# jinsungkim96/MPC-SensorlessAO

Measured on AMD Instinct MI355X. Metric: MPC steps/sec (n=27, VAR(2), T=30), higher is better.
Workload: dtype f64

## Files before the change

### mpc-sensorlessao_amd/csrc/fmpc_affine.h

```cpp
#pragma once
#include <hip/hip_runtime.h>
#include "fmpc_host.h"
#include "../../include/fastmpc.h"

#define FA_N 27

struct FaStep {
    const double* x0; const double* x0p; const double* nu0;
    double* zout; double* nuout; double* u0out; int* status; int* iters; double* step;
    int* need;
};

struct FaParams {
    int n, m, T, nb, has_xf, batch, rows, tiles, step_ld;
    int nu_rows, nu_tiles;
    int ldz;
    int tiles_used, wgs_per_group;
    const double* img;
    const double* imgE; const double* imgEp;
    const double* elin; const double* eplin;
    const double* dx0T;
    double e0, ep0, normE, norme, normEp, normep, rd2_0;
    const double* x0; const double* x0p; const double* nu0;
    double* zout; double* nuout; double* u0out; int* status; int* iters; double* step;
    int* need; int* handed;
    int* nflag;
    double* dump;
    int nsteps;
    FaStep steps[FMPC_STRETCH_MAX];
    int nlanes, wgs_per_lane;
    int lane_begin[FMPC_STRETCH_MAX + 1];
    const double* imgG;
    const int* plan;
    int jbase, nu_work;
    int nparts, nitems, swap;
};

#define FMPC_STRETCH_LANES_DEFAULT FMPC_STRETCH_MAX
hipError_t fmpc_launch_affine(FaParams P, int num_cu, hipStream_t stream, const unsigned* supersedes = nullptr);
hipError_t fmpc_launch_affine_nu(FaParams P, int grid, bool nt, hipStream_t stream);
```

### mpc-sensorlessao_amd/csrc/fmpc_affine_dev.h

```cpp
#pragma once
#include <hip/hip_runtime.h>
#include <math.h>
#include "fmpc_device.h"
#include "fmpc_affine.h"
#include "../../include/fastmpc.h"

typedef double d4a __attribute__((ext_vector_type(4)));
typedef double d2a __attribute__((ext_vector_type(2)));
#define FA_MFMA(a, b, c) __builtin_amdgcn_mfma_f64_16x16x4f64((a), (b), (c), 0, 0, 0)
#define FA_THREADS 256
#define FA_CT 4

__device__ __forceinline__ void fa_load_a(double (&A)[FA_KS], const double* img, int tile, int lane) {
    const double* ip = img + (size_t)tile * FA_KS * 64 + lane;
#pragma unroll
    for (int q = 0; q < FA_KS; ++q) A[q] = ip[q * 64];
}

__device__ __forceinline__ void fa_request_a(double (&A)[FA_KS], const double* img, int tile, int lane) {
    const double* ip = img + (size_t)tile * FA_KS * 64 + lane;
    const double* ip2 = ip + 8 * 64;
#define FA_LD(q, base, off) asm volatile("global_load_dwordx2 %0, %1, off offset:" #off : "=v"(A[q]) : "v"(base))
    FA_LD(0, ip, 0); FA_LD(1, ip, 512); FA_LD(2, ip, 1024); FA_LD(3, ip, 1536); FA_LD(4, ip, 2048); FA_LD(5, ip, 2560); FA_LD(6, ip, 3072); FA_LD(7, ip, 3584);
    FA_LD(8, ip2, 0); FA_LD(9, ip2, 512); FA_LD(10, ip2, 1024); FA_LD(11, ip2, 1536); FA_LD(12, ip2, 2048); FA_LD(13, ip2, 2560);
#undef FA_LD
}
template <int BEHIND>
__device__ __forceinline__ void fa_await_a(double (&A)[FA_KS]) {
    asm volatile("s_waitcnt vmcnt(%14)"
                 : "+v"(A[0]), "+v"(A[1]), "+v"(A[2]), "+v"(A[3]), "+v"(A[4]), "+v"(A[5]), "+v"(A[6]), "+v"(A[7]), "+v"(A[8]), "+v"(A[9]),
                   "+v"(A[10]), "+v"(A[11]), "+v"(A[12]), "+v"(A[13])
                 : "n"(BEHIND));
}

__device__ __forceinline__ void fa_request_g(double (&A)[FA_NU_KS], const double* img, int tile, int lane) {
    const double* ip = img + (size_t)tile * FA_NU_KS * 64 + lane;
#define FA_LD(q, base, off) asm volatile("global_load_dwordx2 %0, %1, off offset:" #off : "=v"(A[q]) : "v"(base))
    FA_LD(0, ip, 0); FA_LD(1, ip, 512); FA_LD(2, ip, 1024); FA_LD(3, ip, 1536); FA_LD(4, ip, 2048); FA_LD(5, ip, 2560); FA_LD(6, ip, 3072);
#undef FA_LD
}
template <int BEHIND>
__device__ __forceinline__ void fa_await_g(double (&A)[FA_NU_KS]) {
    asm volatile("s_waitcnt vmcnt(%7)"
                 : "+v"(A[0]), "+v"(A[1]), "+v"(A[2]), "+v"(A[3]), "+v"(A[4]), "+v"(A[5]), "+v"(A[6])
                 : "n"(BEHIND));
}

__device__ __forceinline__ bool fa_decide(const FaParams& P, double qe, double qp, double rdl, double dn2) {
    const double dn = sqrt(dn2);
    double e2 = qe + P.e0, rp2 = qp + P.ep0;
    const double ce = 4096.0 * 2.220446049250313e-16;
    const double de = ce * (dn2 * P.normE + 2.0 * P.norme * dn + fabs(P.e0));
    const double dp = ce * (dn2 * P.normEp + 2.0 * P.normep * dn + fabs(P.ep0));
    e2 += de;
    rp2 = rp2 - dp > 0.0 ? rp2 - dp : 0.0;
    const double rho2 = rp2 + rdl;
    const bool fin = rp2 < 1e300 && rho2 < 1e300 && e2 < 1e300 && e2 >= 0.0;
    return fin && (rp2 > 4e-16 || rho2 > 4e-12) && e2 <= 0.5 * rho2;
}

#define FA_SD(ct, cc, k) sD[((((k) >> 2) * FA_CT + (ct)) * 4 + ((k) & 3)) * 16 + (cc)]
__device__ __forceinline__ void fa_stage(double* sD, const FaParams& P, const double* x0_s, const double* x0p_s, int p0, int tid) {
    constexpr int n = FA_N;
    const int np = P.batch - p0 < FA_CT * 16 ? P.batch - p0 : FA_CT * 16;
    const double* s0 = x0_s + (size_t)p0 * n;
    const double* s1 = x0p_s ? x0p_s + (size_t)p0 * n : s0;
    double v0[7], v1[7];
#pragma unroll
    for (int j = 0; j < 7; ++j) {
        const int idx = tid + FA_THREADS * j, ic = idx < np * n ? idx : 0;
        v0[j] = s0[ic]; v1[j] = s1[ic];
    }
#pragma unroll
    for (int j = 0; j < 7; ++j) {
        const int idx = tid + FA_THREADS * j;
        if (idx < FA_CT * 16 * n) {
            const int pr = idx / n, k = idx - pr * n;
            const bool on = idx < np * n;
            FA_SD(pr >> 4, pr & 15, k) = on ? v0[j] : 0.0;
            FA_SD(pr >> 4, pr & 15, n + k) = (on && x0p_s) ? v1[j] : 0.0;
        }
    }
    double zero = 0.0;
    asm volatile("" : "+v"(zero));
    if (tid < FA_CT * 16) { FA_SD(tid >> 4, tid & 15, 2 * n) = 1.0; FA_SD(tid >> 4, tid & 15, 2 * n + 1) = zero; }
}

__device__ __forceinline__ void fa_forms(const double* sD, double (&sF)[4][3][16], const FaParams& P, int slot, int wv, int lane, int p0,
                                         const double* nu0_s, int* need_s, int* status_s, int* iters_s, double* step_s) {
    constexpr int n = FA_N;
    const int g = lane >> 4, c = lane & 15;
    for (int fct = P.wgs_per_group - 1 - slot; fct < FA_CT; fct += P.wgs_per_group) {
        if (fct < 0 || p0 + fct * 16 >= P.batch) continue;
        const int t = wv;
        double E1[FA_KS], E2[FA_KS], Df[FA_KS];
        fa_load_a(E1, P.imgE, t, lane);
        fa_load_a(E2, P.imgEp, t, lane);
        const int k = 16 * t + c;
        const double le = P.elin[k], lp = P.eplin[k];
        double rdl[4] = {P.rd2_0, P.rd2_0, P.rd2_0, P.rd2_0};
        if (nu0_s && t == 0) {
            double xa[4][2];
#pragma unroll
            for (int r = 0; r < 4; ++r) {
                const int pr = p0 + fct * 16 + 4 * r + g < P.batch ? p0 + fct * 16 + 4 * r + g : P.batch - 1;
                const double* nu = nu0_s + (size_t)pr * P.nb * n;
#pragma unroll
                for (int j = 0; j < 2; ++j) {
                    const int e = c + 16 * j, ec = e < n ? e : 0;
                    xa[r][j] = P.dx0T[ec] + nu[(P.T - 1) * n + ec] + (P.has_xf ? nu[P.T * n + ec] : 0.0);
                }
            }
#pragma unroll
            for (int r = 0; r < 4; ++r) {
                double acc = xa[r][0] * xa[r][0] + (c + 16 < n ? xa[r][1] * xa[r][1] : 0.0);
                acc += __shfl_xor(acc, 1, 64); acc += __shfl_xor(acc, 2, 64); acc += __shfl_xor(acc, 4, 64); acc += __shfl_xor(acc, 8, 64);
                rdl[r] = acc;
            }
        }
#pragma unroll
        for (int q = 0; q < FA_KS; ++q) Df[q] = sD[(q * FA_CT + fct) * 64 + lane];
        d4a ce = {0, 0, 0, 0}, cp = {0, 0, 0, 0};
#pragma unroll
        for (int q = 0; q < FA_KS; ++q) { ce = FA_MFMA(Df[q], E1[q], ce); cp = FA_MFMA(Df[q], E2[q], cp); }
        double qe[4], qp[4], dn2[4];
#pragma unroll
        for (int r = 0; r < 4; ++r) {
            const double dv = k < 2 * n ? FA_SD(fct, 4 * r + g, k < 2 * n ? k : 0) : 0.0;
            qe[r] = dv * (ce[r] + le); qp[r] = dv * (cp[r] + lp); dn2[r] = dv * dv;
#pragma unroll
            for (int o = 1; o < 16; o <<= 1) { qe[r] += __shfl_xor(qe[r], o, 64); qp[r] += __shfl_xor(qp[r], o, 64); dn2[r] += __shfl_xor(dn2[r], o, 64); }
            if (c == 0) { sF[t][0][4 * r + g] = qe[r]; sF[t][1][4 * r + g] = qp[r]; sF[t][2][4 * r + g] = dn2[r]; }
        }
        __syncthreads();
        if (t == 0 && c == 0) {
#pragma unroll
            for (int r = 0; r < 4; ++r) {
                const int i = 4 * r + g, pp = p0 + fct * 16 + i;
                if (pp < P.batch) {
                    const double se = (sF[0][0][i] + sF[1][0][i]) + (sF[2][0][i] + sF[3][0][i]);
                    const double sp = (sF[0][1][i] + sF[1][1][i]) + (sF[2][1][i] + sF[3][1][i]);
                    const double sn = (sF[0][2][i] + sF[1][2][i]) + (sF[2][2][i] + sF[3][2][i]);
                    const bool clear = fa_decide(P, se, sp, rdl[r], sn);
                    need_s[pp] = clear ? 0 : 1;
                    if (!clear && P.nflag) atomicAdd(P.nflag, 1);
                    if (clear) {
                        if (status_s) status_s[pp] = FMPC_OK;
                        if (iters_s) iters_s[pp] = 1;
                        if (step_s) for (int q = 0; q < P.step_ld; ++q) step_s[(size_t)pp * P.step_ld + q] = q == 0 ? 1.0 : -1.0;
                    }
                }
            }
        }
        __syncthreads();
    }
}
```

### mpc-sensorlessao_amd/csrc/fmpc_api.hip

```cpp
#include <hip/hip_runtime.h>
#include <math.h>
#include <stdio.h>
#include <stdlib.h>
#include <string.h>
#include <atomic>
#include <map>
#include <mutex>
#include <new>
#include <vector>

#include "../../include/fastmpc.h"
#include "fmpc_device.h"
#include "fmpc_panel.h"
#include "fmpc_host.h"
#include "fmpc_first.h"
#include "fmpc_affine.h"
#include "fmpc_loopu0.h"
#include "fmpc_tiled.h"
#include "fmpc_rampcold.h"
#include "fmpc_bank.h"
#include "fmpc_records.h"
#include "fmpc_kkt.h"
#include "fmpc_estimator.h"
#include "fmpc_handle.h"
// ... 362 lines not shown
}

static int fmpc_upload_cold(fmpc_handle h, double k, hipStream_t stream) {
    const int n = h->n, m = h->m, mp = h->wave.mp;
    int o[14];
    fmpc_wave_cold_layout(n, mp, o);
    std::vector<double> c((size_t)o[8], 0.0);
    for (int j = 0; j < m; ++j) {
        const double sp = h->hm_umax[j] - h->hm_umid[j], sm = h->hm_umid[j] - h->hm_umin[j];
        const double dp = 1.0 / sp, dm = 1.0 / sm;
        const double hc = k * (dp * dp + dm * dm);
        c[o[0] + j] = h->hm_R2[j] * h->hm_umid[j] + h->hm_rl[j] + k * (dp - dm);
        c[o[1] + j] = hc;
        c[o[2] + j] = 1.0 / (h->hm_R2[j] + hc);
    }
    const double* bt = h->hm_bt.data();
    for (int a = 0; a < n; ++a) {
        double cbu = 0.0, bu = 0.0;
        for (int j = 0; j < m; ++j) {
            cbu += bt[(size_t)j * n + a] * c[o[2] + j] * c[o[0] + j];
            bu += bt[(size_t)j * n + a] * h->hm_umid[j];
        }
        c[o[4] + a] = cbu;
        double a1x = 0.0, a2x = 0.0;
        for (int q = 0; q < n; ++q) { a1x += h->hm_a1[a * n + q] * h->hm_xmid[q]; a2x += h->hm_a2[a * n + q] * h->hm_xmid[q]; }
        c[o[5] + a] = h->hm_xmid[a] - bu;
        c[o[6] + a] = h->hm_xmid[a] - bu - a1x;
        c[o[7] + a] = h->hm_xmid[a] - bu - a1x - a2x;
        double va = 0.0, va2 = 0.0;
        for (int j = 0; j < m; ++j) {
            const double aj = c[o[1] + j] * c[o[2] + j];
            va += bt[(size_t)j * n + a] * aj * c[o[0] + j];
            va2 += bt[(size_t)j * n + a] * aj * aj * c[o[0] + j];
        }
        c[o[11] + a] = va; c[o[12] + a] = va2;
        for (int b = 0; b < n; ++b) {
            double g = 0.0, ma = 0.0, ma2 = 0.0;
            for (int j = 0; j < m; ++j) {
                const double bb = bt[(size_t)j * n + a] * bt[(size_t)j * n + b];
                const double aj = c[o[1] + j] * c[o[2] + j];
                g += bb * c[o[2] + j]; ma += bb * aj; ma2 += bb * aj * aj;
            }
            c[o[3] + a * n + b] = g; c[o[9] + a * n + b] = ma; c[o[10] + a * n + b] = ma2;
        }
    }
    for (int j = 0; j < m; ++j) {
        const double aj = c[o[1] + j] * c[o[2] + j], cu = c[o[0] + j];
        c[o[13]] += aj * cu * cu; c[o[13] + 1] += aj * aj * cu * cu;
    }
    return hipMemcpyAsync(h->cold_d, c.data(), c.size() * sizeof(double), hipMemcpyHostToDevice, stream) == hipSuccess
               ? FMPC_OK : FMPC_E_HIP;
}

static int fmpc_upload_panel(fmpc_handle h, double k, hipStream_t stream) {
    (void)stream;
    h->pn_valid = 0;
    FmpcPanelIn In;
    In.n = h->n; In.m = h->m; In.T = h->T; In.nb = h->nb; In.mp = h->pn_mp; In.var_order = h->var_order;
    In.pool_doubles = h->pn_doubles; In.o_simg = h->pn_o_simg; In.o_limg = h->pn_o_limg; In.o_bt = h->pn_o_bt;
    In.o_aimg = h->pn_o_aimg; In.o_vec = h->pn_o_vec; In.o_ucon = h->pn_o_ucon; In.o_dz = h->pn_o_dz; In.limg_cap = h->pn_limg_cap;
    In.umax = h->hm_umax.data(); In.umin = h->hm_umin.data(); In.umid = h->hm_umid.data(); In.xmid = h->hm_xmid.data();
    In.R2 = h->hm_R2.data(); In.rl = h->hm_rl.data(); In.Q2 = h->hm_Q2.data(); In.Qf2 = h->hm_Qf2.data();
    In.ql = h->hm_ql.data(); In.qfl = h->hm_qfl.data(); In.xf = h->hm_xf.data();
    In.bt = h->hm_bt.data(); In.a1 = h->hm_a1.data(); In.a2 = h->hm_a2.data(); In.blocks = h->hm_blocks.data();
    In.idxD = h->hm_idxD.data(); In.idx1 = h->hm_idx1.data(); In.idx2 = h->hm_idx2.data();
    FmpcPanelOut Out;
    fmpc_host_build_panel(In, k, Out);
    if (!Out.valid) return FMPC_OK;
    h->pn_nsf = Out.nsf; h->pn_nsb = Out.nsb; h->pn_rp2c = Out.rp2c; h->pn_rd2_0 = Out.rd2_0;
    if (hipMemcpy(h->pn_sched, Out.sched.data(), Out.sched.size() * sizeof(int), hipMemcpyHostToDevice) != hipSuccess) return FMPC_E_HIP;
    if (hipMemcpy(h->pn_pool, Out.pool.data(), Out.pool.size() * sizeof(double), hipMemcpyHostToDevice) != hipSuccess) return FMPC_E_HIP;
    h->pn_valid = 1;
    return FMPC_OK;
}

template <typename R>
static int fmpc_tiled_build(fmpc_handle h, int t, hipStream_t stream) {
    fmpc_handle_s::Tiled& X = h->tl[t];
    const int n = h->n, m = h->m, nb = h->nb, nn = n * n;
    int NB = 0, NW = 0;
    if (!fmpc_tiled_supports(n, m, nb, t, &NB, &NW, h->denseR)) return FMPC_E_UNSUPPORTED;
    const int mb = (m + 15) / 16, NQ = NB * NB;
    const int nblk = (int)(h->hm_blocks.size() / nn);
    std::vector<R> img((size_t)(nblk + 1) * NQ * FT_TILE + (size_t)mb * NB * FT_TILE, (R)0);
    for (int k = 0; k < nblk; ++k)
        for (int a = 0; a < n; ++a)
            for (int b = 0; b < n; ++b)
                img[((size_t)k * NQ + (a / 16) * NB + b / 16) * FT_TILE + (a % 16) * 16 + b % 16] = (R)h->hm_blocks[(size_t)k * nn + a * n + b];
    const size_t obt = (size_t)(nblk + 1) * NQ * FT_TILE;
    for (int c = 0; c < m; ++c)
        for (int r = 0; r < n; ++r)
            img[obt + ((size_t)(c / 16) * NB + r / 16) * FT_TILE + (c % 16) * 16 + r % 16] = (R)h->hm_bt[(size_t)c * n + r];
    std::vector<int> ids;
    for (int i = 0; i < nb; ++i) ids.push_back(h->hm_idxD[i]);
    for (int i = 0; i < nb; ++i) ids.push_back(h->hm_idx1[i] >= 0 ? h->hm_idx1[i] : nblk);
    for (int i = 0; i < nb; ++i) ids.push_back(h->hm_idx2[i] >= 0 ? h->hm_idx2[i] : nblk);
    const int NP = 16 * NB, MP = 16 * mb;
    const size_t oBt = 0, oBm = oBt + (size_t)MP * NP, oA1 = oBm + (size_t)NP * MP, oA2 = oA1 + (size_t)NP * NP,
                 oA1t = oA2 + (size_t)NP * NP, oA2t = oA1t + (size_t)NP * NP, oQ2 = oA2t + (size_t)NP * NP,
                 oQf2 = oQ2 + (size_t)NP * NP, oX = oQf2 + (size_t)NP * NP, oXf = oX + (size_t)NP * NP, oR2 = oXf + (size_t)NP * NP,
                 ptot = oR2 + (h->denseR ? (size_t)MP * MP : 0);
    std::vector<double> pad(ptot, 0.0);
    for (int c = 0; c < m; ++c)
        for (int r = 0; r < n; ++r) {
            pad[oBt + (size_t)c * NP + r] = h->hm_bt[(size_t)c * n + r];
            pad[oBm + (size_t)r * MP + c] = h->hm_bt[(size_t)c * n + r];
        }
    for (int a = 0; a < n; ++a)
        for (int b = 0; b < n; ++b) {
            pad[oA1 + (size_t)a * NP + b] = h->hm_a1f[(size_t)a * n + b]; pad[oA1t + (size_t)b * NP + a] = h->hm_a1f[(size_t)a * n + b];
            pad[oA2 + (size_t)a * NP + b] = h->hm_a2f[(size_t)a * n + b]; pad[oA2t + (size_t)b * NP + a] = h->hm_a2f[(size_t)a * n + b];
            pad[oQ2 + (size_t)a * NP + b] = h->hm_q2m[(size_t)a * n + b]; pad[oQf2 + (size_t)a * NP + b] = h->hm_qf2m[(size_t)a * n + b];
            pad[oX + (size_t)a * NP + b] = h->hm_xm[(size_t)a * n + b]; pad[oXf + (size_t)a * NP + b] = h->hm_xfm[(size_t)a * n + b];
        }
    if (h->denseR)
        for (int a = 0; a < m; ++a)
            for (int b = 0; b < m; ++b) pad[oR2 + (size_t)a * MP + b] = h->hm_r2full[(size_t)a * m + b];
    int rc = X.pool.assign((const char*)img.data(), img.size() * sizeof(R), stream);
    if (rc == FMPC_OK) rc = X.ipool.assign(ids.data(), ids.size(), stream);
    if (rc == FMPC_OK) rc = X.bm.assign(pad.data(), pad.size(), stream);
    if (rc != FMPC_OK) return rc;
    X.NB = NB; X.NW = NW;
    X.lds = fmpc_tiled_lds_bytes(NB, mb, NW, t, nb, h->denseR ? ft_pr_doubles(n, m) : 0);
    if (fmpc_tiled_prepare(n, NB, NW, t, X.lds, h->denseR) != hipSuccess) return FMPC_E_HIP;
    X.V.NB = NB; X.V.mb = mb; X.V.cn = n / 16; X.V.nl = n % 16; X.V.nblk = nblk;
    X.V.yimg = X.pool; X.V.btimg = (const R*)X.pool.p + obt;
    X.V.iD = X.ipool; X.V.i1 = X.ipool + nb; X.V.i2 = X.ipool + 2 * nb;
    X.V.BtP = X.bm + oBt; X.V.BmP = X.bm + oBm; X.V.A1P = X.bm + oA1; X.V.A2P = X.bm + oA2; X.V.A1tP = X.bm + oA1t; X.V.A2tP = X.bm + oA2t;
    X.V.denseR = h->denseR; X.V.R2P = h->denseR ? X.bm + oR2 : nullptr;
    X.V.denseQ = h->denseQ; X.V.Q2P = X.bm + oQ2; X.V.Qf2P = X.bm + oQf2; X.V.XP = X.bm + oX; X.V.XfP = X.bm + oXf;
    X.ready = 1;
    return FMPC_OK;
}

int fmpc_tiled_ensure(fmpc_handle h, int t, hipStream_t stream) {
    if (h->tl[t].ready) return FMPC_OK;
    return t ? fmpc_tiled_build<float>(h, 1, stream) : fmpc_tiled_build<double>(h, 0, stream);
}

__global__ void fmpc_zero_ints(int* p, int n) { if ((int)threadIdx.x < n) p[threadIdx.x] = 0; }
int fmpc_tiled_plan(fmpc_handle h, int t, int batch, hipStream_t stream, int nw_override, int grid_hint, FmpcTiledPlan* out) {
    fmpc_handle_s::Tiled& X = h->tl[t];
    { const int rc = fmpc_tiled_ensure(h, t, stream); if (rc != FMPC_OK) return rc; }
    int NWu = X.NW; size_t ldsu = X.lds;
    if (nw_override && nw_override != X.NW && !t && !h->denseR) {
        NWu = nw_override;
        ldsu = fmpc_tiled_lds_bytes(X.NB, X.V.mb, NWu, t, h->nb, 0);
        if (!(h->tl_prepared & (1 << NWu))) {
            if (ldsu > FMPC_LDS_LIMIT || fmpc_tiled_prepare(h->n, X.NB, NWu, t, ldsu, 0) != hipSuccess) { NWu = X.NW; ldsu = X.lds; }
            else h->tl_prepared |= 1 << NWu;
        }
    }
    int wgs = (int)(FMPC_LDS_LIMIT / ldsu);
    if (wgs < 1) wgs = 1;
    if (wgs * NWu > 8) wgs = 8 / NWu > 0 ? 8 / NWu : 1;
    const int cap = h->num_cu * wgs;
    const bool capturing = fmpc_capturing(stream);
    int grid = batch < cap ? batch : cap;
    if (!capturing && grid_hint > 0 && grid_hint < grid) grid = grid_hint;
    const FtWs L = ft_ws_layout(h->n, h->m, h->T, h->nb, X.NB, t ? 4 : 8, h->denseR, (t && h->refine > 0) ? 1 : 0);
    const size_t need = L.total * (size_t)grid, full = L.total * (size_t)cap;
    if (need > h->tl_ws.cap) {
        if (capturing) {
            const size_t have = h->tl_ws.cap / L.total;
            if (have < 1) return FMPC_E_ALLOC;
            grid = (int)have;
        } else {
            size_t want = 2 * h->tl_ws.cap;
            if (want < need) want = need;
            if (want > full) want = full;
            int rc = h->tl_ws.alloc(want, stream);
            if (rc != FMPC_OK && want != need) rc = h->tl_ws.alloc(need, stream);
            if (rc != FMPC_OK) return rc;
        }
    }
    out->NWu = NWu; out->ldsu = ldsu; out->grid = grid; out->slot = L.total;
    return FMPC_OK;
}

static int fmpc_solve_tiled(fmpc_handle h, int t, const FmpcSolve& s, int nw_override = 0, const int* list = nullptr,
                            const int* nlist = nullptr, const double* nuws = nullptr, int grid_hint = 0,
                            const FmpcTiledPlan* planned = nullptr) {
    FmpcTiledPlan plan;
    if (planned) plan = *planned;
    else { const int rc = fmpc_tiled_plan(h, t, s.batch, s.stream, nw_override, grid_hint, &plan); if (rc != FMPC_OK) return rc; }
    fmpc_handle_s::Tiled& X = h->tl[t];
    FtParams P;
    P.M = h->dev; P.V = X.V; P.batch = s.batch;
    P.x0 = s.x0; P.x0p = s.x0_pre; P.w = s.w; P.zinit = s.z_init; P.nu0 = s.nu0;
    P.max_iter = fmpc_max_iter(s); P.kbar = s.k;
    P.zout = s.z_out; P.nuout = s.nu_out; P.status = s.status; P.iters = s.iters; P.step = s.step; P.step_ld = fmpc_step_ld(s.n_newton);
    P.ws = h->tl_ws; P.ws_stride = plan.slot; P.u0out = s.u0_out;
    P.list = list; P.nlist = nlist; P.nuws = nuws;
    P.refine = t ? h->refine : 0;
    h->tl_last_nw = plan.NWu;
    if (t) h->refine_last = P.refine;
    if (!list) { h->last_path = t ? FMPC_PATH_TILED_F32 : FMPC_PATH_TILED; h->bank_first_dispatch = 0; }
    return fmpc_launch_tiled(P, X.NB, plan.NWu, t, plan.grid, plan.ldsu, s.stream) == hipSuccess ? FMPC_OK : FMPC_E_HIP;
}

extern "C" int fmpc_set_precision(fmpc_handle h, int mode) {
    if (!h) return FMPC_E_NULL;
    if (mode != FMPC_PREC_F64 && mode != FMPC_PREC_F32_MIXED) return FMPC_E_DIM;
    if (mode == FMPC_PREC_F32_MIXED && !fmpc_tiled_supports(h->n, h->m, h->nb, 1, nullptr, nullptr, h->denseR)) return FMPC_E_UNSUPPORTED;
    std::lock_guard<std::mutex> lk(h->mu);
    if (mode == FMPC_PREC_F64 && !h->generic_ok && !fmpc_tiled_supports(h->n, h->m, h->nb, 0, nullptr, nullptr, h->denseR)) {
        const size_t lds = fmpc_generic_big_lds_bytes(h->n, h->m);
        if (lds > FMPC_LDS_LIMIT) return FMPC_E_UNSUPPORTED;
        if (fmpc_generic_prepare(lds, 1) != hipSuccess) return FMPC_E_HIP;
        h->generic_ok = 1; h->generic_big = 1; h->lds_bytes = lds; h->wg_per_cu = 2;
    }
    h->prec = mode;
    h->bkf.valid = 0;
    h->bfm.valid = 0;
    return FMPC_OK;
}

extern "C" int fmpc_set_refinement(fmpc_handle h, int sweeps) {
    if (!h) return FMPC_E_NULL;
    if (sweeps < 0 || sweeps > FMPC_MAX_REFINEMENT) return FMPC_E_DIM;
    std::lock_guard<std::mutex> lk(h->mu);
    h->refine = sweeps;
    return FMPC_OK;
}
extern "C" int fmpc_last_refinement(fmpc_handle h) {
    if (!h) return 0;
    std::lock_guard<std::mutex> lk(h->mu);
    return h->last_path == FMPC_PATH_TILED_F32 ? h->refine_last : 0;
}

static int fmpc_grid_for(fmpc_handle h, int batch) {
    int cap = h->num_cu * h->wg_per_cu;
    return batch < cap ? batch : cap;
}

static int fmpc_ensure_ws(fmpc_handle h, int grid, size_t* stride, hipStream_t stream) {
    const FmpcWsLayout L = fmpc_ws_layout(h->n, h->m, h->T, h->nb, h->generic_big != 0, h->denseR != 0);
    *stride = L.total;
    return h->ws.grow(L.total * (size_t)grid, stream);
}

bool fmpc_capturing(hipStream_t stream) {
    hipStreamCaptureStatus st = hipStreamCaptureStatusNone;
    return hipStreamIsCapturing(stream, &st) == hipSuccess && st == hipStreamCaptureStatusActive;
}

struct FmpcChainStep {
    FaStep a;
    FwParams w;
    bool superseded;
    unsigned same_outputs;
};
struct FmpcStretch {
    fmpc_handle h = nullptr;
    int nsteps = 0;
    FaParams A;
    double k = 0.0; int n_newton = 0, zld = 0, g3 = 0; bool z_null = false, z_aligned = false;
    size_t wave_lds = 0, ws_stride = 0; int num_cu = 0;
    FwParams* table = nullptr;
    FmpcChainStep st[FMPC_STRETCH_MAX];
    size_t nodes_seen = 0;
};
static std::mutex fmpc_st_mu;
static std::map<hipStream_t, FmpcStretch> fmpc_st_map;
static std::atomic<int> fmpc_st_open{0};

static bool fmpc_capture_nodes(hipStream_t stream, size_t* count) {
    hipStreamCaptureStatus st = hipStreamCaptureStatusNone;
    unsigned long long id = 0; hipGraph_t graph = nullptr; const hipGraphNode_t* deps = nullptr; size_t ndeps = 0;
    if (hipStreamGetCaptureInfo_v2(stream, &st, &id, &graph, &deps, &ndeps) != hipSuccess || st != hipStreamCaptureStatusActive || !graph)
        return false;
    size_t n = 0;
    if (hipGraphGetNodes(graph, nullptr, &n) != hipSuccess) return false;
    *count = n;
    return true;
}
static void fmpc_stretch_look(FmpcStretch& S, hipStream_t stream) {
    size_t n = 0;
    S.nodes_seen = fmpc_capture_nodes(stream, &n) ? n : 0;
}
static bool fmpc_stretch_foreign(FmpcStretch& S, hipStream_t stream) {
    size_t n = 0;
    if (S.nsteps == 0 || !fmpc_capture_nodes(stream, &n) || n == S.nodes_seen) return false;
    S.nsteps = 0; S.h = nullptr;
    S.nodes_seen = n;
    return true;
}

static int fmpc_stretch_flush(FmpcStretch& S, hipStream_t stream) {
    if (S.nsteps == 0) return FMPC_OK;
    const int n = S.nsteps;
    fmpc_handle h = S.h;
    S.nsteps = 0; S.h = nullptr;
    if (!fmpc_capturing(stream) && h->ev && h->ev_valid && h->last_stream != stream && hipStreamWaitEvent(stream, h->ev, 0) != hipSuccess)
        return FMPC_E_HIP;
    FaParams A = S.A;
    A.nsteps = n;
    for (int i = 0; i < n; ++i) A.steps[i] = S.st[i].a;
    unsigned same[FMPC_STRETCH_MAX];
    for (int j = 0; j < n; ++j) {
        same[j] = S.st[j].same_outputs & ((1u << j) - 1u);
        for (int i = 0; i < j; ++i) if (same[j] >> i & 1u) same[j] |= same[i];
    }
    if (fmpc_launch_affine(A, S.num_cu, stream, same) != hipSuccess) return FMPC_E_HIP;
    int live[FMPC_STRETCH_MAX], nlive = 0;
    for (int i = 0; i < n; ++i) if (!S.st[i].superseded) live[nlive++] = i;
    int launches = 1;
    if (nlive == 1 || S.z_null) {
        for (int j = 0; j < nlive; ++j) {
            FwParams P = S.st[live[j]].w;
            if (j + 1 < nlive) { P.handed = nullptr; P.nflag = nullptr; }
            if (fmpc_launch_wave(P, S.g3, S.wave_lds, stream) != hipSuccess) return FMPC_E_HIP;
            ++launches;
        }
    } else {
        int g = S.num_cu / nlive;
        if (g > S.g3) g = S.g3;
        if (g < 1) return FMPC_E_UNSUPPORTED;
        FwChainStep T[FMPC_STRETCH_MAX];
        for (int j = 0; j < nlive; ++j) {
            const FwParams& P = S.st[live[j]].w;
            T[j] = {P.x0, P.x0p, P.nu0, P.zout, P.nuout, P.u0out, P.status, P.iters, P.step, P.list,
                    j + 1 == nlive ? P.handed : nullptr, P.ws + (size_t)j * g * fmpc_wave_waves_per_wg() * S.ws_stride};
        }
        if (fmpc_launch_wave_chain(S.st[live[0]].w, T, nlive, S.table, g, S.wave_lds, stream) != hipSuccess) return FMPC_E_HIP;
        launches += 2;
    }
    h->st_steps = n; h->st_launches = launches;
    if (!fmpc_capturing(stream) && h->ev && hipEventRecord(h->ev, stream) == hipSuccess) { h->ev_valid = 1; h->last_stream = stream; }
    fmpc_stretch_look(S, stream);
    return FMPC_OK;
}

static void fmpc_stretch_flush_handle_locked(fmpc_handle h, bool keep_one, hipStream_t keep);
static int fmpc_stretch_flush_stream(hipStream_t stream, fmpc_handle h = nullptr) {
    if (fmpc_st_open.load() == 0) return FMPC_OK;
    std::lock_guard<std::mutex> lk(fmpc_st_mu);
    if (h) fmpc_stretch_flush_handle_locked(h, true, stream);
    auto it = fmpc_st_map.find(stream);
    if (it == fmpc_st_map.end()) return FMPC_OK;
    if (fmpc_stretch_foreign(it->second, stream)) return FMPC_E_UNSUPPORTED;
    return fmpc_stretch_flush(it->second, stream);
}
static void fmpc_stretch_flush_handle_locked(fmpc_handle h, bool keep_one, hipStream_t keep) {
    for (auto& kv : fmpc_st_map)
        if (kv.second.nsteps && kv.second.h == h && !(keep_one && kv.first == keep) && !fmpc_stretch_foreign(kv.second, kv.first))
            (void)fmpc_stretch_flush(kv.second, kv.first);
}
static void fmpc_stretch_flush_handle(fmpc_handle h) {
    if (fmpc_st_open.load() == 0) return;
    std::lock_guard<std::mutex> lk(fmpc_st_mu);
    fmpc_stretch_flush_handle_locked(h, false, nullptr);
}

extern "C" int fmpc_stretch_begin(void* stream_) {
    hipStream_t stream = (hipStream_t)stream_;
    std::lock_guard<std::mutex> lk(fmpc_st_mu);
    if (fmpc_st_map.count(stream)) return FMPC_E_UNSUPPORTED;
    FmpcStretch& S = fmpc_st_map[stream];
    fmpc_stretch_look(S, stream);
    fmpc_st_open.fetch_add(1);
    return FMPC_OK;
}
extern "C" int fmpc_stretch_end(void* stream_) {
    hipStream_t stream = (hipStream_t)stream_;
    std::lock_guard<std::mutex> lk(fmpc_st_mu);
    auto it = fmpc_st_map.find(stream);
    if (it == fmpc_st_map.end()) return FMPC_E_UNSUPPORTED;
    int rc = FMPC_OK;
    if (it->second.nsteps) {
        if (it->second.h && hipSetDevice(it->second.h->device) != hipSuccess) rc = FMPC_E_HIP;
        else if (fmpc_stretch_foreign(it->second, stream)) rc = FMPC_E_UNSUPPORTED;
        else rc = fmpc_stretch_flush(it->second, stream);
    }
    fmpc_st_map.erase(it);
    fmpc_st_open.fetch_sub(1);
    return rc;
}
extern "C" int fmpc_last_stretch(fmpc_handle h, int* steps, int* launches) {
    if (!h) return FMPC_E_NULL;
    if (steps) *steps = h->st_steps.load();
    if (launches) *launches = h->st_launches.load();
    return FMPC_OK;
}

static inline bool fmpc_overlap(const void* a, size_t na, const void* b, size_t nb) {
    if (!a || !b || !na || !nb) return false;
    const char* pa = (const char*)a; const char* pb = (const char*)b;
    return pa < pb + nb && pb < pa + na;
}
struct FmpcStepRanges { const void* in[3]; size_t nin[3]; const void* out[6]; size_t nout[6]; };
static FmpcStepRanges fmpc_step_ranges(const FaParams& A, const FaStep& a) {
    FmpcStepRanges R;
    const size_t B = (size_t)A.batch, d = sizeof(double);
    R.in[0] = a.x0; R.nin[0] = B * A.n * d;
    R.in[1] = a.x0p; R.nin[1] = B * A.n * d;
    R.in[2] = a.nu0; R.nin[2] = B * A.nb * A.n * d;
    const size_t ldz = A.ldz > A.rows ? A.ldz : A.rows;
    R.out[0] = a.zout; R.nout[0] = ((B - 1) * ldz + A.rows) * d;
    R.out[1] = a.nuout; R.nout[1] = B * A.nb * A.n * d;
    R.out[2] = a.u0out; R.nout[2] = B * A.m * d;
    R.out[3] = a.status; R.nout[3] = B * sizeof(int);
    R.out[4] = a.iters; R.nout[4] = B * sizeof(int);
    R.out[5] = a.step; R.nout[5] = B * A.step_ld * d;
    return R;
}
static bool fmpc_stretch_accepts(const FmpcStretch& S, fmpc_handle h, const FmpcSolve& s, const FaStep& a, int zld, bool z_null, unsigned* supersedes) {
    *supersedes = 0;
    if (S.h != h || S.nsteps >= FMPC_STRETCH_MAX || memcmp(&S.k, &s.k, sizeof(double)) != 0 || S.A.batch != s.batch) return false;
    if (S.n_newton != s.n_newton || S.zld != zld || S.z_null != z_null || S.z_aligned != (((size_t)a.zout & 127) == 0)) return false;
    const FaStep& f = S.st[0].a;
    if ((f.nuout == nullptr) != (a.nuout == nullptr) || (f.u0out == nullptr) != (a.u0out == nullptr) || (f.status == nullptr) != (a.status == nullptr) ||
        (f.iters == nullptr) != (a.iters == nullptr) || (f.step == nullptr) != (a.step == nullptr)) return false;
    const FmpcStepRanges N = fmpc_step_ranges(S.A, a);
    for (int i = 0; i < S.nsteps; ++i) {
        const FaStep& b = S.st[i].a;
        const FmpcStepRanges O = fmpc_step_ranges(S.A, b);
        for (int x = 0; x < 3; ++x)
            for (int y = 0; y < 6; ++y)
                if (fmpc_overlap(N.in[x], N.nin[x], O.out[y], O.nout[y]) || fmpc_overlap(O.in[x], O.nin[x], N.out[y], N.nout[y])) return false;
        if (a.zout == b.zout && a.nuout == b.nuout && a.u0out == b.u0out && a.status == b.status && a.iters == b.iters && a.step == b.step) {
            *supersedes |= 1u << i;
            continue;
        }
        for (int x = 0; x < 6; ++x)
            for (int y = 0; y < 6; ++y)
                if (fmpc_overlap(N.out[x], N.nout[x], O.out[y], O.nout[y])) return false;
    }
    return true;
}

static int fmpc_stretch_settle(fmpc_handle h, hipStream_t stream) {
    if (!h->st_cur || h->st_cur->nsteps == 0) return FMPC_OK;
    return fmpc_stretch_flush(*h->st_cur, stream);
}
static int fmpc_guard_begin_queued(fmpc_handle h, hipStream_t stream) {
    if (fmpc_capturing(stream)) return FMPC_OK;
    if (!h->ev && hipEventCreateWithFlags(&h->ev, hipEventDisableTiming) != hipSuccess) return FMPC_E_HIP;
    if (h->ev_valid && stream != h->last_stream && hipStreamWaitEvent(stream, h->ev, 0) != hipSuccess) return FMPC_E_HIP;
    return FMPC_OK;
}
int fmpc_guard_begin(fmpc_handle h, hipStream_t stream) {
    const int rcs = fmpc_stretch_flush_stream(stream, h);
    if (rcs != FMPC_OK) return rcs;
    if (fmpc_capturing(stream)) return FMPC_OK;
    if (!h->ev && hipEventCreateWithFlags(&h->ev, hipEventDisableTiming) != hipSuccess) return FMPC_E_HIP;
    if (h->ev_valid && stream != h->last_stream && hipStreamWaitEvent(stream, h->ev, 0) != hipSuccess) return FMPC_E_HIP;
    return FMPC_OK;
}
void fmpc_guard_end(fmpc_handle h, hipStream_t stream) {
    if (fmpc_capturing(stream)) return;
    if (h->ev && hipEventRecord(h->ev, stream) == hipSuccess) { h->ev_valid = 1; h->last_stream = stream; }
}

static void fmpc_panel_params(fmpc_handle h, double k, FpParams& Q) {
    memset(&Q, 0, sizeof(Q));
    Q.m = h->m; Q.mp = h->pn_mp; Q.T = h->T; Q.nb = h->nb; Q.has_xf = h->has_xf; Q.var2 = h->var_order == 2 ? 1 : 0;
    Q.simg = h->pn_pool + h->pn_o_simg; Q.limg = h->pn_pool + h->pn_o_limg;
    Q.sched_f = h->pn_sched; Q.sched_b = h->pn_sched + (size_t)FP_MAX_STEPS(h->nb) * FP_STEP_INTS; Q.nsf = h->pn_nsf; Q.nsb = h->pn_nsb;
    Q.btimg = h->pn_pool + h->pn_o_bt; Q.aimg = h->pn_pool + h->pn_o_aimg;
    Q.vec = h->pn_pool + h->pn_o_vec; Q.ucon = h->pn_pool + h->pn_o_ucon;
    Q.rd2_0 = h->pn_rd2_0; Q.rp2c = h->pn_rp2c; Q.dump = h->pn_pool + h->pn_o_dump;
    Q.dzimg = h->pn_pool + h->pn_o_dz; Q.dzimg_len = h->pn_dz_len;
    Q.kbar = k;
    Q.jimg = h->inv_jimg; Q.nuc = h->inv_nuc; Q.jks = h->inv_jks; Q.jksp = 16 * ((h->inv_jks + 15) / 16 + 3); Q.eimg = h->inv_eimg;
    Q.jst = h->inv_jst; Q.nucst = h->inv_nucst; Q.gate_only = 0;
    Q.gw = nullptr; Q.gwn = h->T * h->n;
}

static int fmpc_build_inverse(fmpc_handle h, double k, hipStream_t stream) {
    const int n = h->n, T = h->T, nb = h->nb, TN = T * n, nrow = nb * n;
    const int ncol = 2 * n + TN, np = 1 + ncol + 2 * n, npanels = (np + FP_NP - 1) / FP_NP;
    const double scale = FMPC_INV_SCALE;
    h->inv_valid = 0;
    std::vector<double> hx0((size_t)np * n, 0.0), hx0p((size_t)np * n, 0.0), hw((size_t)np * TN, 0.0);
    for (int j = 0; j < n; ++j) { hx0[(size_t)(1 + j) * n + j] = scale; hx0p[(size_t)(1 + n + j) * n + j] = scale; }
    for (int j = 0; j < TN; ++j) hw[(size_t)(1 + 2 * n + j) * TN + j] = scale;
    for (int j = 0; j < n; ++j)
        for (int e = 0; e < TN; ++e) {
            hw[(size_t)(1 + ncol + j) * TN + e] = -scale * h->hm_m1[(size_t)e * n + j];
            hw[(size_t)(1 + ncol + n + j) * TN + e] = -scale * h->hm_m2[(size_t)e * n + j];
        }
    DevBuf<double> d;
    const size_t o_x0 = 0, o_x0p = o_x0 + hx0.size(), o_w = o_x0p + hx0p.size(), o_gate = o_w + hw.size(),
                 o_nu = o_gate + 2 * (size_t)np, total = o_nu + (size_t)npanels * nrow * FP_NP;
    int rc = d.alloc(total, stream);
    if (rc != FMPC_OK) return rc;
    std::vector<double> nu((size_t)npanels * nrow * FP_NP);
    if (hipMemcpyAsync(d + o_x0, hx0.data(), hx0.size() * sizeof(double), hipMemcpyHostToDevice, stream) != hipSuccess ||
        hipMemcpyAsync(d + o_x0p, hx0p.data(), hx0p.size() * sizeof(double), hipMemcpyHostToDevice, stream) != hipSuccess ||
        hipMemcpyAsync(d + o_w, hw.data(), hw.size() * sizeof(double), hipMemcpyHostToDevice, stream) != hipSuccess) rc = FMPC_E_HIP;
    if (rc == FMPC_OK) {
        FpParams Q;
        fmpc_panel_params(h, k, Q);
        Q.batch = np; Q.npanels = npanels; Q.step_ld = 1;
        Q.x0 = d + o_x0; Q.x0p = d + o_x0p; Q.w = d + o_w; Q.nu0 = nullptr;
        Q.nuws = d + o_nu; Q.gate = d + o_gate; Q.handed = nullptr;
        const int pgrid = npanels < h->num_cu ? npanels : h->num_cu;
        if (fmpc_launch_panel(Q, pgrid, fmpc_panel_lds_used(h->nb, h->pn_mp, h->pn_nsf + h->pn_nsb), stream) != hipSuccess ||
            hipMemcpyAsync(nu.data(), d + o_nu, nu.size() * sizeof(double), hipMemcpyDeviceToHost, stream) != hipSuccess ||
            hipStreamSynchronize(stream) != hipSuccess) rc = FMPC_E_HIP;
    }
    d.release();
    if (rc != FMPC_OK) return rc;
    std::vector<double> img, nuc, jst, ncs, img2, eimg, J4, nuc4;
    const bool finite = fmpc_host_inverse_images(n, T, nb, h->var_order == 2, h->inv_jks, h->inv_jks2, h->hm_a1.data(), h->hm_a2.data(), nu,
                                                 img, nuc, jst, ncs, img2, eimg, J4, nuc4);
    if (!jst.empty() &&
        (hipMemcpy(h->inv_jst, jst.data(), jst.size() * sizeof(double), hipMemcpyHostToDevice) != hipSuccess ||
         hipMemcpy(h->inv_nucst, ncs.data(), ncs.size() * sizeof(double), hipMemcpyHostToDevice) != hipSuccess)) return FMPC_E_HIP;
    if (!finite) return FMPC_OK;
    if (hipMemcpy(h->inv_jimg2, img2.data(), img2.size() * sizeof(double), hipMemcpyHostToDevice) != hipSuccess) return FMPC_E_HIP;
    if (hipMemcpy(h->inv_eimg, eimg.data(), eimg.size() * sizeof(double), hipMemcpyHostToDevice) != hipSuccess ||
        hipMemcpy(h->inv_jimg, img.data(), img.size() * sizeof(double), hipMemcpyHostToDevice) != hipSuccess ||
        hipMemcpy(h->inv_nuc, nuc.data(), nuc.size() * sizeof(double), hipMemcpyHostToDevice) != hipSuccess) return FMPC_E_HIP;
    h->hm_J4.swap(J4); h->hm_nuc.swap(nuc4);
    h->hm_J4_valid = 1; h->hm_J4_k = k; h->fm_valid = 0;
    h->inv_valid = 1; h->inv_k = k;
    return FMPC_OK;
}

static int fmpc_build_first_move(fmpc_handle h, double k, hipStream_t stream) {
    h->fm_valid = 0;
    if (!h->hm_J4_valid || h->hm_J4_k != k) return FMPC_E_UNSUPPORTED;
    const int n = h->n, m = h->m, T = h->T, TN = T * n;
    FmpcFirstIn In;
    In.n = n; In.m = m; In.T = T; In.nb = h->nb; In.var2 = h->var_order == 2 ? 1 : 0; In.has_xf = h->has_xf;
    In.bt = h->hm_bt.data(); In.umax = h->hm_umax.data(); In.umin = h->hm_umin.data(); In.umid = h->hm_umid.data();
    In.xmid = h->hm_xmid.data(); In.R2 = h->hm_R2.data(); In.rl = h->hm_rl.data(); In.a1 = h->hm_a1.data(); In.a2 = h->hm_a2.data();
    In.m1 = h->hm_m1.data(); In.m2 = h->hm_m2.data(); In.xf = h->hm_xf.empty() ? h->hm_xmid.data() : h->hm_xf.data();
    In.J = h->hm_J4.data(); In.nuc = h->hm_nuc.data(); In.k = k;
    FmpcFirstOut O;
    fmpc_host_build_first_move(In, O);
    for (double v : O.K0t) if (!std::isfinite(v)) return FMPC_E_UNSUPPORTED;
    for (double v : O.E) if (!std::isfinite(v)) return FMPC_E_UNSUPPORTED;
    std::vector<double> pool;
    auto push = [&](const std::vector<double>& v) { const size_t o = pool.size(); pool.insert(pool.end(), v.begin(), v.end()); while (pool.size() % 2) pool.push_back(0.0); return o; };
    std::vector<double> m12t((size_t)2 * n * TN), dx0T(n);
    for (int e = 0; e < TN; ++e)
        for (int q = 0; q < n; ++q) { m12t[(size_t)q * TN + e] = h->hm_m1[(size_t)e * n + q]; m12t[(size_t)(n + q) * TN + e] = h->hm_m2[(size_t)e * n + q]; }
    for (int r = 0; r < n; ++r) dx0T[r] = h->hm_Qf2[r] * h->hm_xmid[r] + h->hm_qfl[r];
    const size_t oK = push(O.K0t), ou = push(O.u0c), oE = push(O.Ec), oe = push(O.e), oEp = push(O.Epc), oep = push(O.ep), om = push(m12t), od = push(dx0T);
    h->fa_valid = 0;
    FmpcAffineOut AO;
    size_t oA = 0, oAE = 0, oAEp = 0, oAl = 0, oAlp = 0, oAd = 0, oAG = 0, oAP = 0;
    bool fa_ok = !h->fa_disabled && 2 * n + 2 <= FA_KC;
    if (fa_ok) {
        FmpcAffineIn AI;
        AI.n = n; AI.m = m; AI.T = T; AI.nb = h->nb; AI.has_xf = h->has_xf; AI.ncJ = 4 * n;
        AI.bt = In.bt; AI.umax = In.umax; AI.umin = In.umin; AI.umid = In.umid; AI.xmid = In.xmid; AI.R2 = In.R2; AI.rl = In.rl;
        AI.Q2 = h->hm_Q2.data(); AI.Qf2 = h->hm_Qf2.data(); AI.ql = h->hm_ql.data(); AI.qfl = h->hm_qfl.data(); AI.a1 = In.a1; AI.a2 = In.a2;
        AI.J = In.J; AI.nuc = In.nuc; AI.k = k;
        fmpc_host_build_affine(AI, AO);
        for (double v : AO.img) if (!std::isfinite(v)) { fa_ok = false; break; }
    }
    if (fa_ok) {
        const int nc = 4 * n, nd = 2 * n;
        std::vector<double> E64((size_t)64 * FA_KC, 0.0), Ep64((size_t)64 * FA_KC, 0.0), el(64, 0.0), epl(64, 0.0), imgE, imgEp;
        for (int r = 0; r < nd; ++r) {
            for (int c = 0; c < nd; ++c) { E64[(size_t)r * FA_KC + c] = O.E[(size_t)r * nc + c]; Ep64[(size_t)r * FA_KC + c] = O.Ep[(size_t)r * nc + c]; }
            el[r] = 2.0 * O.e[r]; epl[r] = -2.0 * O.ep[r];
        }
        fmpc_host_mfma_a_images(E64.data(), 64, imgE);
        fmpc_host_mfma_a_images(Ep64.data(), 64, imgEp);
        oA = push(AO.img); oAE = push(imgE); oAEp = push(imgEp); oAl = push(el); oAlp = push(epl);
        oAd = push(std::vector<double>(4096, 0.0));
        if (!AO.imgG.empty()) {
            std::vector<double> planw((AO.plan.size() * sizeof(FmpcNuStage) + sizeof(double) - 1) / sizeof(double), 0.0);
            memcpy(planw.data(), AO.plan.data(), AO.plan.size() * sizeof(FmpcNuStage));
            oAG = push(AO.imgG); oAP = push(planw);
        }
    }
    h->fl_valid = 0; h->fs_valid = 0;
    size_t oLU = 0, oLE = 0, oLEp = 0, oSU = 0, oSE = 0, oSEp = 0, oSB = 0;
    const bool fl_ok = !h->fl_disabled && 4 * n + 1 <= 4 * FL_KS;
    const bool fs_ok = fl_ok && !h->fs_disabled && n == 27 && m <= 144;
    if (fl_ok) {
        FmpcLoopImages LI;
        fmpc_host_build_loop_images(O, n, m, FL_KS, false, nullptr, LI);
        oLU = push(LI.imgU); oLE = push(LI.imgE); oLEp = push(LI.imgEp);
    }
    if (fs_ok) {
        FmpcLoopImages LI;
        fmpc_host_build_loop_images(O, n, m, FL_KS, true, In.bt, LI);
        oSU = push(LI.imgU); oSE = push(LI.imgE); oSEp = push(LI.imgEp); oSB = push(LI.imgB);
    }
    const int rc = h->fm_pool.assign(pool.data(), pool.size(), stream);
    if (rc != FMPC_OK) return rc;
    FmParams& P = h->fm_P;
    memset(&P, 0, sizeof(P));
    P.n = n; P.m = m; P.T = T; P.nb = h->nb; P.var2 = In.var2; P.has_xf = h->has_xf;
    P.bt = h->dev.Bt; P.K0t = h->fm_pool + oK; P.u0c = h->fm_pool + ou; P.E = h->fm_pool + oE; P.e = h->fm_pool + oe;
    P.Ep = h->fm_pool + oEp; P.ep = h->fm_pool + oep; P.m12t = h->fm_pool + om; P.dx0T = h->fm_pool + od;
    P.e0 = O.e0; P.ep0 = O.ep0; P.normE = O.normE; P.norme = O.norme; P.normEp = O.normEp; P.normep = O.normep; P.rd2_0 = h->pn_rd2_0;
    h->fm_valid = 1; h->fm_k = k;
    if (fa_ok) {
        FaParams& A = h->fa_P;
        memset(&A, 0, sizeof(A));
        A.n = n; A.m = m; A.T = T; A.nb = h->nb; A.has_xf = h->has_xf; A.rows = AO.rows; A.tiles = AO.tiles; A.nu_rows = AO.nu_rows; A.nu_tiles = AO.nu_tiles;
        A.img = h->fm_pool + oA; A.imgE = h->fm_pool + oAE; A.imgEp = h->fm_pool + oAEp; A.elin = h->fm_pool + oAl; A.eplin = h->fm_pool + oAlp; A.dump = h->fm_pool + oAd;
        if (!AO.imgG.empty()) {
            A.imgG = h->fm_pool + oAG; A.plan = (const int*)(h->fm_pool + oAP); A.jbase = AO.jbase; A.nu_work = fmpc_host_nu_work(AO.plan);
        }
        A.dx0T = P.dx0T; A.e0 = O.e0; A.ep0 = O.ep0; A.normE = O.normE; A.norme = O.norme; A.normEp = O.normEp; A.normep = O.normep; A.rd2_0 = h->pn_rd2_0;
        h->fa_valid = 1;
    }
    if (fl_ok) {
        FlParams& L = h->fl_P;
        memset(&L, 0, sizeof(L));
        L.n = n; L.m = m; L.T = T; L.nb = h->nb; L.has_xf = h->has_xf; L.var2 = In.var2;
        L.imgU = h->fm_pool + oLU; L.imgE = h->fm_pool + oLE; L.imgEp = h->fm_pool + oLEp;
        L.dx0T = P.dx0T; L.e0 = O.e0; L.ep0 = O.ep0; L.normE = O.normE; L.norme = O.norme; L.normEp = O.normEp; L.normep = O.normep; L.rd2_0 = h->pn_rd2_0;
        h->fl_valid = 1;
        if (fs_ok) {
            h->fs_P = L;
            h->fs_P.imgU = h->fm_pool + oSU; h->fs_P.imgE = h->fm_pool + oSE; h->fs_P.imgEp = h->fm_pool + oSEp;
            memset(&h->fs_I, 0, sizeof(h->fs_I));
            const int Tn = T * n;
            h->fs_I.rs = (Tn + 63) / 64; h->fs_I.rows = (Tn + h->fs_I.rs - 1) / h->fs_I.rs;
            h->fs_I.imgB = h->fm_pool + oSB; h->fs_I.M1 = h->loop_M1; h->fs_I.M2 = h->loop_M2;
            h->fs_valid = 1;
        }
    }
    return FMPC_OK;
}

static int fmpc_ensure_wave_ws(fmpc_handle h, size_t* stride_out, hipStream_t stream) {
    const int wpw = fmpc_wave_waves_per_wg();
    const size_t stride = fmpc_wave_ws_doubles(h->n, h->m, h->wave.mp, h->T, h->nb);
    const int rc = h->ws.grow(stride * (size_t)h->num_cu * wpw, stream);
    if (rc != FMPC_OK) return rc;
    *stride_out = stride;
    return FMPC_OK;
}

static FwParams fmpc_wave_params(fmpc_handle h, const FmpcSolve& s, size_t stride, int zld = 0) {
    FwParams P;
    memset(&P, 0, sizeof(P));
    P.M = h->dev; P.V = h->wave;
    P.batch = s.batch; P.max_iter = fmpc_max_iter(s); P.step_ld = fmpc_step_ld(s.n_newton); P.kbar = s.k;
    P.x0 = s.x0; P.x0p = s.x0_pre; P.w = s.w; P.zinit = s.z_init; P.nu0 = s.nu0;
    P.zout = s.z_out; P.nuout = s.nu_out; P.status = s.status; P.iters = s.iters; P.step = s.step; P.u0out = s.u0_out;
    P.zld = zld > 0 ? zld : h->T * (h->n + h->m);
    P.ws = h->ws; P.ws_stride = stride;
    P.sh_fac = h->sh_fac; P.sh_rs = h->sh_rs; P.sh_ok = h->sh_ok; P.cold = h->cold_d;
    return P;
}

static int fmpc_wave_grid(fmpc_handle h, int batch) {
    const int wpw = fmpc_wave_waves_per_wg();
    const int grid = (batch + wpw - 1) / wpw;
    return grid < h->num_cu ? grid : h->num_cu;
}

static int fmpc_launch_flagged(fmpc_handle h, const FmpcSolve& s, int grid, size_t stride, int* need, int* nflag = nullptr, int zld = 0) {
    FwParams P = fmpc_wave_params(h, s, stride, zld);
    P.mode = FW_MODE_SHARED; P.handed = h->pn_cnt; P.pphase = 3; P.list = need; P.nflag = nflag;
    return fmpc_launch_wave(P, grid, h->wave_lds, s.stream) == hipSuccess ? FMPC_OK : FMPC_E_HIP;
}

static int fmpc_ensure_cold(fmpc_handle h, double k, size_t stride, hipStream_t stream) {
    if (h->sh_valid && h->sh_k == k) return FMPC_OK;
    if (h->sh_valid && hipStreamSynchronize(stream) != hipSuccess) return FMPC_E_HIP;
    double* scr = h->sh_scratch;
    const FmpcSolve one = {1, scr, scr, nullptr, nullptr, nullptr, 1, k, scr + ((h->n + 15) & ~15), nullptr, nullptr, nullptr, nullptr,
                           nullptr, stream, 0};
    FwParams P = fmpc_wave_params(h, one, stride);
    P.mode = FW_MODE_EXPORT;
    if (fmpc_launch_wave(P, 1, h->wave_lds, stream) != hipSuccess) return FMPC_E_HIP;
    if (fmpc_upload_cold(h, k, stream) != FMPC_OK) return FMPC_E_HIP;
    if (h->pn_enabled && fmpc_upload_panel(h, k, stream) != FMPC_OK) return FMPC_E_HIP;
    h->sh_valid = 1; h->sh_k = k;
    return FMPC_OK;
}

int fmpc_scratch_z(fmpc_handle h, int batch, hipStream_t stream) {
    return h->zs.grow((size_t)batch * h->T * (h->n + h->m), stream);
}


static int fmpc_path_tiled(fmpc_handle h, const FmpcSolve& s) {
    const int t_ = h->prec == FMPC_PREC_F32_MIXED ? 1 : 0;
    const int few = (!t_ && !h->denseR && h->n <= 31 && h->n != FP_N && s.batch <= 512 && !h->force_tiled) ? 4 : 0;
    return fmpc_solve_tiled(h, t_, s, few);
}

static int fmpc_path_generic(fmpc_handle h, const FmpcSolve& s) {
    h->last_path = FMPC_PATH_GENERIC;
    const int grid = fmpc_grid_for(h, s.batch);
    size_t stride = 0;
    const int rc = fmpc_ensure_ws(h, h->generic_big ? grid : h->num_cu * h->wg_per_cu, &stride, s.stream);
    if (rc != FMPC_OK) return rc;
    hipError_t e = fmpc_launch_generic(h->dev, s.batch, grid, s.x0, s.x0_pre, s.w, s.z_init, s.nu0, fmpc_max_iter(s), s.k,
                                       s.z_out, s.nu_out, s.status, s.iters, s.step, fmpc_step_ld(s.n_newton),
                                       h->ws, stride, s.stream, h->generic_big);
    if (e == hipSuccess && s.u0_out)
        e = fmpc_launch_unpack(h->n, h->m, h->T, s.batch, s.z_out, nullptr, nullptr, s.u0_out, s.stream);
    return e == hipSuccess ? FMPC_OK : FMPC_E_HIP;
}

static int fmpc_path_affine(fmpc_handle h, const FmpcSolve& s, size_t stride, int zld, bool z_null) {
    if (!h->fm_valid || h->fm_k != s.k) {
        { const int rcq = fmpc_stretch_settle(h, s.stream); if (rcq != FMPC_OK) return rcq; }
        if (hipStreamSynchronize(s.stream) != hipSuccess) return FMPC_E_HIP;
        const int rcf = fmpc_build_first_move(h, s.k, s.stream);
        if (rcf != FMPC_OK && rcf != FMPC_E_UNSUPPORTED) return rcf;
    }
    if (!(h->fm_valid && h->fm_k == s.k && h->fa_valid)) return FMPC_E_UNSUPPORTED;
    if ((size_t)s.batch > h->fa_need_cap) {
        { const int rcq = fmpc_stretch_settle(h, s.stream); if (rcq != FMPC_OK) return rcq; }
        size_t cap = 256;
        while (cap < (size_t)s.batch) cap *= 2;
        h->fa_need_cap = 0;
        const int rc = h->fa_need.alloc((size_t)FMPC_STRETCH_MAX * cap, s.stream);
        if (rc != FMPC_OK) return rc;
        h->fa_need_cap = cap;
    }
    FaParams A = h->fa_P;
    A.batch = s.batch; A.step_ld = fmpc_step_ld(s.n_newton);
    A.x0 = s.x0; A.x0p = s.x0_pre; A.nu0 = s.nu0; A.zout = z_null ? nullptr : s.z_out; A.nuout = s.nu_out; A.u0out = s.u0_out;
    A.status = s.status; A.iters = s.iters; A.step = s.step; A.need = h->fa_need; A.handed = h->pn_cnt;
    int* const nf = h->fa_nflag;
    static const bool no_nflag = [] { const char* e = getenv("FMPC_NO_NFLAG"); return e && e[0] == '1'; }();
    A.nflag = no_nflag ? nullptr : nf;
    A.ldz = zld;
    A.nsteps = 0;
    const int grid = fmpc_wave_grid(h, s.batch);
    const int g3 = grid < 64 ? grid : 64;
    if (h->st_cur) {
        FmpcStretch& S = *h->st_cur;
        FaStep a = {A.x0, A.x0p, A.nu0, A.zout, A.nuout, A.u0out, A.status, A.iters, A.step, nullptr};
        unsigned sup = 0;
        if (S.nsteps > 0 && !fmpc_stretch_accepts(S, h, s, a, zld, z_null, &sup)) { const int rcq = fmpc_stretch_settle(h, s.stream); if (rcq != FMPC_OK) return rcq; }
        const int i = S.nsteps;
        a.need = h->fa_need + (size_t)i * h->fa_need_cap;
        if (i == 0) {
            S.h = h; S.A = A; S.k = s.k; S.n_newton = s.n_newton; S.zld = zld; S.z_null = z_null; S.z_aligned = ((size_t)A.zout & 127) == 0;
            S.g3 = g3; S.wave_lds = h->wave_lds; S.ws_stride = stride; S.num_cu = h->num_cu; S.table = (FwParams*)h->fw_chain.p;
            fmpc_stretch_look(S, s.stream);
            sup = 0;
        }
        for (int j = 0; j < i; ++j) if (sup & (1u << j)) S.st[j].superseded = true;
        S.st[i].a = a;
        S.st[i].superseded = false;
        S.st[i].same_outputs = sup;
        FwParams W = fmpc_wave_params(h, s, stride, zld);
        W.mode = FW_MODE_SHARED; W.handed = h->pn_cnt; W.pphase = 3; W.list = a.need; W.nflag = no_nflag ? nullptr : nf;
        S.st[i].w = W;
        S.nsteps = i + 1;
        h->last_path = FMPC_PATH_PANEL; h->pn_split_last = 0; h->inv_last = 2;
        return FMPC_OK;
    }
    if (fmpc_launch_affine(A, h->num_cu, s.stream) != hipSuccess) return FMPC_E_HIP;
    const int rc = fmpc_launch_flagged(h, s, g3, stride, h->fa_need, no_nflag ? nullptr : nf, zld);
    h->last_path = FMPC_PATH_PANEL; h->pn_split_last = 0; h->inv_last = 2;
    return rc;
}

static int fmpc_path_panel(fmpc_handle h, const FmpcSolve& s, size_t stride, int zld, bool z_null) {
    const int batch = s.batch, max_iter = fmpc_max_iter(s);
    const int npanels = (batch + FP_NP - 1) / FP_NP;
    if ((size_t)batch > h->pn_cap) {
        { const int rcq = fmpc_stretch_settle(h, s.stream); if (rcq != FMPC_OK) return rcq; }
        h->pn_cap = 0;
        if (h->pn_gate.alloc((size_t)batch * 2, s.stream) != FMPC_OK ||
            h->pn_epsp.alloc((size_t)npanels * h->T * FP_NP, s.stream) != FMPC_OK ||
            h->pn_rnp.alloc((size_t)npanels * h->T * FP_NP, s.stream) != FMPC_OK ||
            h->pn_list.alloc((size_t)batch, s.stream) != FMPC_OK ||
            h->pn_nuws.alloc((size_t)npanels * FP_NP * h->nb * h->n, s.stream) != FMPC_OK) return FMPC_E_ALLOC;
        h->pn_cap = batch;
    }
    const bool lowrank = h->lp_hint && s.w != nullptr && h->lp_v != nullptr;
    const bool dense_form = h->inv_enabled && (s.w == nullptr || lowrank || batch <= h->inv_max_batch);
    if (dense_form && (!h->inv_valid || h->inv_k != s.k) && !(h->inv_failed && h->inv_failed_k == s.k)) {
        { const int rcq = fmpc_stretch_settle(h, s.stream); if (rcq != FMPC_OK) return rcq; }
        if (hipStreamSynchronize(s.stream) != hipSuccess) return FMPC_E_HIP;
        const int rcb = fmpc_build_inverse(h, s.k, s.stream);
        if (rcb != FMPC_OK) return rcb;
        h->inv_failed = h->inv_valid ? 0 : 1; h->inv_failed_k = s.k;
    }
    if (dense_form && h->inv_valid && s.w == nullptr && max_iter == 1 && (s.nu_out == nullptr || !z_null) && !h->fa_disabled && h->n == FP_N) {
        const int rca = fmpc_path_affine(h, s, stride, zld, z_null);
        if (rca != FMPC_E_UNSUPPORTED) return rca;
    }
    if (zld) return FMPC_E_UNSUPPORTED;
    { const int rcq = fmpc_stretch_settle(h, s.stream); if (rcq != FMPC_OK) return rcq; }
    FpParams Q;
    fmpc_panel_params(h, s.k, Q);
    Q.batch = batch; Q.npanels = npanels; Q.step_ld = fmpc_step_ld(s.n_newton);
    Q.x0 = s.x0; Q.x0p = s.x0_pre; Q.w = s.w; Q.nu0 = s.nu0;
    Q.zout = s.z_out; Q.status = s.status; Q.iters = s.iters; Q.step = s.step;
    Q.nuws = h->pn_nuws; Q.nuout = s.nu_out;
    Q.gate = h->pn_gate; Q.epsp = h->pn_epsp; Q.handed = h->pn_cnt;
    Q.rnp = h->pn_rnp;
    const int split = max_iter > 1;
    const int pgrid = npanels < h->num_cu ? npanels : h->num_cu;
    h->inv_last = dense_form && h->inv_valid;
    const bool fuse = h->inv_last && h->inv_fuse && s.w == nullptr && !h->has_xf && max_iter == 1;
    Q.gate_only = fuse ? 1 : 0;
    const bool u0only = z_null && max_iter == 1 && s.nu_out == nullptr;
    Q.u0out = s.u0_out;
    if (h->inv_last) {
        if (lowrank) { Q.gw = h->lp_v; Q.gwn = 2 * h->n; Q.jimg = h->inv_jimg2; Q.jks = h->inv_jks2; Q.jksp = 16 * ((h->inv_jks2 + 15) / 16 + 3); }
        else { Q.gw = s.w; Q.gwn = h->T * h->n; }
    }
    hipError_t e;
    if (h->inv_last) e = fmpc_launch_inv(Q, s.stream);
    else e = fmpc_launch_panel(Q, pgrid, fmpc_panel_lds_used(h->nb, h->pn_mp, h->pn_nsf + h->pn_nsb), s.stream);
    if (e != hipSuccess) return FMPC_E_HIP;
    const int ppx = (npanels + 7) / 8;
    const int dgrid = 8 * ((ppx * h->T + FD_WAVES - 1) / FD_WAVES);
    e = fmpc_launch_dz(Q, dgrid, split, s.stream, fuse ? 1 : 0, u0only ? 1 : 0);
    if (e != hipSuccess) return FMPC_E_HIP;
    const int grid = fmpc_wave_grid(h, batch);
    for (int ph = split ? 1 : 0; ph <= (split ? 2 : 0); ++ph) {
        int g2 = grid;
        if (ph == 2) {
            const int last = ((volatile int*)h->pn_cnt_host.p)[1];
            if (last >= 0) {
                const int wpw2 = fmpc_wave_waves_per_wg();
                int want = (last + last / 2 + wpw2 - 1) / wpw2 + 4;
                if (want < 8) want = 8;
                if (want < g2) g2 = want;
            }
        }
        if (ph == 2 && h->small_tiled) {
            const int last = ((volatile int*)h->pn_cnt_host.p)[1];
            const int hint = last >= 0 ? last + last / 2 + 16 : 0;
            const int rc_t = fmpc_solve_tiled(h, 0, s, h->small_nw, h->pn_list, h->pn_cnt + 1, h->pn_nuws, hint);
            if (rc_t == FMPC_OK) continue;
            if (rc_t != FMPC_E_UNSUPPORTED && rc_t != FMPC_E_ALLOC) return rc_t;
        }
        FwParams P = fmpc_wave_params(h, s, stride);
        P.mode = FW_MODE_SHARED; P.gate = h->pn_gate; P.epsp = h->pn_epsp; P.handed = h->pn_cnt; P.nuws = h->pn_nuws;
        P.pphase = ph; P.rnp = h->pn_rnp; P.list = h->pn_list; P.u0_done = u0only ? 1 : 0;
        e = fmpc_launch_wave(P, g2, h->wave_lds, s.stream);
        if (e != hipSuccess) return FMPC_E_HIP;
    }
    if (split && hipMemcpyAsync(h->pn_cnt_host, h->pn_cnt, 2 * sizeof(int), hipMemcpyDeviceToHost, s.stream) != hipSuccess)
        return FMPC_E_HIP;
    h->last_path = FMPC_PATH_PANEL; h->pn_split_last = split;
    return e == hipSuccess ? FMPC_OK : FMPC_E_HIP;
}

static int fmpc_path_small_tiled(fmpc_handle h, const FmpcSolve& s) {
    return fmpc_solve_tiled(h, 0, s, s.batch <= 512 ? h->small_nw : 2);
}

static int fmpc_path_split(fmpc_handle h, const FmpcSolve& s, size_t stride) {
    const int last = h->gn_cnt_host ? ((volatile int*)h->gn_cnt_host.p)[1] : -1;
    const int gn_hint = last >= 0 ? last + last / 2 + 16 : 0;
    FmpcTiledPlan gplan;
    if (fmpc_tiled_plan(h, 0, s.batch, s.stream, h->small_nw, gn_hint, &gplan) != FMPC_OK) return FMPC_E_UNSUPPORTED;
    const size_t nbn = (size_t)h->nb * h->n;
    if ((size_t)s.batch > h->gn_cap) {
        h->gn_cap = 0;
        if (h->gn_list.alloc((size_t)s.batch, s.stream) != FMPC_OK || h->gn_cnt.alloc(2, s.stream) != FMPC_OK ||
            h->gn_nu.alloc((size_t)s.batch * nbn, s.stream) != FMPC_OK) return FMPC_E_ALLOC;
        h->gn_cap = s.batch;
    }
    if (!h->gn_cnt_host) {
        if (h->gn_cnt_host.alloc(2, s.stream) != FMPC_OK) return FMPC_E_ALLOC;
        h->gn_cnt_host[0] = -1; h->gn_cnt_host[1] = -1;
    }
    double* nu_arr = s.nu_out ? s.nu_out : h->gn_nu;
    hipLaunchKernelGGL(fmpc_zero_ints, dim3(1), dim3(64), 0, s.stream, h->gn_cnt, 2);
    if (hipGetLastError() != hipSuccess) return FMPC_E_HIP;
    FwParams P = fmpc_wave_params(h, s, stride);
    P.nuout = nu_arr; P.handed = h->gn_cnt; P.pphase = 4; P.list = h->gn_list;
    if (fmpc_launch_wave(P, fmpc_wave_grid(h, s.batch), h->wave_lds, s.stream) != hipSuccess) return FMPC_E_HIP;
    h->last_path = FMPC_PATH_WAVE;
    FmpcSolve c = s;
    c.z_init = nullptr; c.nu_out = nu_arr;
    const int rc_t = fmpc_solve_tiled(h, 0, c, h->small_nw, h->gn_list, h->gn_cnt + 1, nullptr, gn_hint, &gplan);
    if (rc_t != FMPC_OK) return rc_t;
    if (hipMemcpyAsync(h->gn_cnt_host, h->gn_cnt, 2 * sizeof(int), hipMemcpyDeviceToHost, s.stream) != hipSuccess) return FMPC_E_HIP;
    return FMPC_OK;
}

static int fmpc_path_wave(fmpc_handle h, const FmpcSolve& s, int mode, size_t stride) {
    FwParams P = fmpc_wave_params(h, s, stride);
    P.mode = mode;
    const hipError_t e = fmpc_launch_wave(P, fmpc_wave_grid(h, s.batch), h->wave_lds, s.stream);
    h->last_path = mode == FW_MODE_SHARED ? FMPC_PATH_SHARED : FMPC_PATH_WAVE;
    return e == hipSuccess ? FMPC_OK : FMPC_E_HIP;
}

static int fmpc_solve_device_inner(fmpc_handle h, FmpcSolve s) {
    if (!h || !s.x0 || (!s.z_out && !s.u0_out)) return FMPC_E_NULL;
    if (s.batch < 0) return FMPC_E_DIM;
    if (s.batch == 0) return FMPC_OK;
    const int max_iter = fmpc_max_iter(s);
    const bool z_null = s.z_out == nullptr;
    if (z_null) {
        if ((size_t)s.batch * h->T * (h->n + h->m) > h->zs.cap) { const int rcq = fmpc_stretch_settle(h, s.stream); if (rcq != FMPC_OK) return rcq; }
        const int rcz = fmpc_scratch_z(h, s.batch, s.stream);
        if (rcz != FMPC_OK) return rcz;
        s.z_out = h->zs;
    }
    const int zld = (!z_null && s.ldz > h->T * (h->n + h->m)) ? s.ldz : 0;
    if (zld && (s.w != nullptr || s.z_init != nullptr || max_iter != 1 || h->prec == FMPC_PREC_F32_MIXED || h->force_tiled || h->denseQ ||
                h->denseR || !h->use_wave || !h->sh_enabled || !h->pn_enabled)) return FMPC_E_UNSUPPORTED;
    if (h->prec == FMPC_PREC_F32_MIXED || h->force_tiled || ((h->denseQ || h->denseR) && !h->generic_big) ||
        (!h->use_wave && (!h->generic_ok || h->prefer_tiled))) {
        { const int rcq = fmpc_stretch_settle(h, s.stream); if (rcq != FMPC_OK) return rcq; }
        return fmpc_path_tiled(h, s);
    }
    if (!h->use_wave) {
        { const int rcq = fmpc_stretch_settle(h, s.stream); if (rcq != FMPC_OK) return rcq; }
        return fmpc_path_generic(h, s);
    }
    size_t stride = 0;
    if (fmpc_wave_ws_doubles(h->n, h->m, h->wave.mp, h->T, h->nb) * (size_t)h->num_cu * fmpc_wave_waves_per_wg() > h->ws.cap) { const int rcq = fmpc_stretch_settle(h, s.stream); if (rcq != FMPC_OK) return rcq; }
    int rc = fmpc_ensure_wave_ws(h, &stride, s.stream);
    if (rc != FMPC_OK) return rc;
    int mode = FW_MODE_NORMAL;
    if (h->sh_enabled && s.z_init == nullptr) {
        if (!(h->sh_valid && h->sh_k == s.k)) { const int rcq = fmpc_stretch_settle(h, s.stream); if (rcq != FMPC_OK) return rcq; }
        rc = fmpc_ensure_cold(h, s.k, stride, s.stream);
        if (rc != FMPC_OK) return rc;
        mode = FW_MODE_SHARED;
    }
    if (mode == FW_MODE_SHARED && h->pn_enabled && h->pn_valid) return fmpc_path_panel(h, s, stride, zld, z_null);
    if (zld) return FMPC_E_UNSUPPORTED;
    { const int rcq = fmpc_stretch_settle(h, s.stream); if (rcq != FMPC_OK) return rcq; }
    if (mode == FW_MODE_NORMAL && h->small_tiled && s.batch <= 1024) {
        rc = fmpc_path_small_tiled(h, s);
        if (rc != FMPC_E_UNSUPPORTED) return rc;
    }
    if (mode == FW_MODE_NORMAL && max_iter > 1 && h->small_tiled && h->gn_split) {
        rc = fmpc_path_split(h, s, stride);
        if (rc != FMPC_E_UNSUPPORTED) return rc;
    }
    return fmpc_path_wave(h, s, mode, stride);
}

static bool fmpc_affine_ready(fmpc_handle h, const FmpcSolve& s) {
    if (s.w || s.z_init || fmpc_max_iter(s) != 1 || s.batch <= 0) return false;
    const bool z_null = s.z_out == nullptr;
    const size_t nz = (size_t)h->T * (h->n + h->m);
    if (z_null && (size_t)s.batch * nz > h->zs.cap) return false;
    if (h->prec == FMPC_PREC_F32_MIXED || h->force_tiled || h->denseQ || h->denseR || !h->use_wave || !h->sh_enabled || !h->pn_enabled ||
        !h->pn_valid || h->n != FP_N) return false;
    if (fmpc_wave_ws_doubles(h->n, h->m, h->wave.mp, h->T, h->nb) * (size_t)h->num_cu * fmpc_wave_waves_per_wg() > h->ws.cap) return false;
    if (!h->sh_valid || h->sh_k != s.k || (size_t)s.batch > h->pn_cap) return false;
    if (!h->inv_enabled || !h->inv_valid || h->inv_k != s.k || h->fa_disabled || (s.nu_out != nullptr && z_null)) return false;
    return h->fm_valid && h->fm_k == s.k && h->fa_valid && (size_t)s.batch <= h->fa_need_cap;
}

static int fmpc_solve_device_impl(fmpc_handle h, FmpcSolve s) {
    if (!h || !s.x0 || (!s.z_out && !s.u0_out)) return FMPC_E_NULL;
    if (s.batch < 0) return FMPC_E_DIM;
    if (s.batch == 0) return FMPC_OK;
    if (hipSetDevice(h->device) != hipSuccess) return FMPC_E_HIP;
    std::lock_guard<std::mutex> lk(h->mu);
    if (s.ldz < 0) s.ldz = h->z_ld;
    std::unique_lock<std::mutex> sl(fmpc_st_mu, std::defer_lock);
    FmpcStretch* S = nullptr;
    if (fmpc_st_open.load() > 0) {
        sl.lock();
        fmpc_stretch_flush_handle_locked(h, true, s.stream);
        auto it = fmpc_st_map.find(s.stream);
        if (it != fmpc_st_map.end()) S = &it->second;
        else sl.unlock();
    }
    if (S && S->nsteps) {
        if (fmpc_stretch_foreign(*S, s.stream)) return FMPC_E_UNSUPPORTED;
        const bool z_null = s.z_out == nullptr;
        const int zld = (!z_null && s.ldz > h->T * (h->n + h->m)) ? s.ldz : 0;
        const FaStep a = {s.x0, s.x0_pre, s.nu0, s.z_out, s.nu_out, s.u0_out, s.status, s.iters, s.step, nullptr};
        unsigned sup = 0;
        if (!(fmpc_affine_ready(h, s) && fmpc_stretch_accepts(*S, h, s, a, zld, z_null, &sup))) {
            const int rcf = fmpc_stretch_flush(*S, s.stream);
            if (rcf != FMPC_OK) return rcf;
        }
    }
    int rc = fmpc_guard_begin_queued(h, s.stream);
    if (rc != FMPC_OK) return rc;
    h->st_cur = S;
    rc = fmpc_solve_device_inner(h, s);
    h->st_cur = nullptr;
    if (!(S && S->nsteps && S->h == h)) fmpc_guard_end(h, s.stream);
    else if (!fmpc_capturing(s.stream)) h->last_stream = s.stream;
    return rc;
}

extern "C" int fmpc_solve_device(fmpc_handle h, int batch,
                                 const double* x0, const double* x0_pre, const double* w,
                                 const double* z_init, const double* nu0,
                                 int n_newton, double k,
                                 double* z_out, double* nu_out, int* status, int* iters, double* step,
                                 void* stream) {
    return fmpc_solve_device_impl(h, {batch, x0, x0_pre, w, z_init, nu0, n_newton, k, z_out, nu_out, status, iters, step,
                                      nullptr, (hipStream_t)stream, -1});
}

extern "C" int fmpc_solve_u0_device(fmpc_handle h, int batch,
                                    const double* x0, const double* x0_pre, const double* w,
                                    const double* z_init, const double* nu0,
                                    int n_newton, double k,
                                    double* z_out, double* nu_out, int* status, int* iters, double* step,
                                    double* u0_out, void* stream) {
    if (!u0_out) return FMPC_E_NULL;
    return fmpc_solve_device_impl(h, {batch, x0, x0_pre, w, z_init, nu0, n_newton, k, z_out, nu_out, status, iters, step,
                                      u0_out, (hipStream_t)stream, -1});
}

extern "C" int fmpc_solve_u0_device_ld(fmpc_handle h, int batch,
                                       const double* x0, const double* x0_pre, const double* w,
                                       const double* z_init, const double* nu0,
                                       int n_newton, double k,
                                       double* z_out, double* nu_out, int* status, int* iters, double* step,
                                       double* u0_out, int ldz, void* stream) {
    if (!h) return FMPC_E_NULL;
    if (ldz < 0 || (ldz != 0 && ldz < h->T * (h->n + h->m))) return FMPC_E_DIM;
    return fmpc_solve_device_impl(h, {batch, x0, x0_pre, w, z_init, nu0, n_newton, k, z_out, nu_out, status, iters, step,
                                      u0_out, (hipStream_t)stream, ldz});
}

#define FMPC_FIRST_MOVE_MAX_BATCH 64
#define FMPC_WALK_MAX_BATCH 4096
static int fmpc_first_move_ensure(fmpc_handle h, int batch, double k, hipStream_t stream, size_t* stride_out, int max_batch = FMPC_FIRST_MOVE_MAX_BATCH) {
    if (h->fm_disabled || !h->use_wave || !h->sh_enabled || !h->pn_enabled || !h->inv_enabled || h->n != FP_N || batch > max_batch)
        return FMPC_E_UNSUPPORTED;
    size_t stride = 0;
    int rc = fmpc_ensure_wave_ws(h, &stride, stream);
    if (rc != FMPC_OK) return rc;
    rc = fmpc_ensure_cold(h, k, stride, stream);
    if (rc != FMPC_OK) return rc;
    if (!h->pn_valid) return FMPC_E_UNSUPPORTED;
    if (!h->inv_valid || h->inv_k != k) {
        if (h->inv_failed && h->inv_failed_k == k) return FMPC_E_UNSUPPORTED;
        if (hipStreamSynchronize(stream) != hipSuccess) return FMPC_E_HIP;
        rc = fmpc_build_inverse(h, k, stream);
        if (rc != FMPC_OK) return rc;
        h->inv_failed = h->inv_valid ? 0 : 1; h->inv_failed_k = k;
        if (!h->inv_valid) return FMPC_E_UNSUPPORTED;
    }
    if (!h->fm_valid || h->fm_k != k) {
        if (hipStreamSynchronize(stream) != hipSuccess) return FMPC_E_HIP;
        rc = fmpc_build_first_move(h, k, stream);
        if (rc != FMPC_OK) return rc;
    }
    rc = fmpc_scratch_z(h, batch, stream);
    if (rc != FMPC_OK) return rc;
    rc = h->fm_need.grow(batch > FMPC_FIRST_MOVE_MAX_BATCH ? (size_t)batch : (size_t)FMPC_FIRST_MOVE_MAX_BATCH, stream);
    if (rc != FMPC_OK) return rc;
    *stride_out = stride;
    return FMPC_OK;
}

static int fmpc_first_move_step(fmpc_handle h, int batch, const double* a_k, const double* x0_last, const double* u1, const double* u2,
                                double* x0, double* x0_pre, double* w, const double* nu0, double k,
                                int* status, int* iters, double* step, double* u0_out, hipStream_t stream, int given = 0) {
    size_t stride = 0;
    int rc = fmpc_first_move_ensure(h, batch, k, stream, &stride);
// ... 801 lines not shown
```

### mpc-sensorlessao_amd/csrc/fmpc_handle.h

```cpp
#pragma once
#include <hip/hip_runtime.h>
#include <atomic>
#include <mutex>
#include <vector>

#include "../../include/fastmpc.h"
#include "fmpc_device.h"
#include "fmpc_first.h"
#include "fmpc_affine.h"
#include "fmpc_loopu0.h"
#include "fmpc_tiled.h"
#include "fmpc_rampcold.h"
#include "fmpc_alloc.h"

#define FMPC_PRODUCT_MIN_BATCH_DEFAULT 65
#define FMPC_LDS_LIMIT (160 * 1024)

struct fmpc_handle_s {
    int n, m, T, nb, var_order, has_xf, device;
    int num_cu;
    FmpcDevModel dev;
    const double* loop_M1; const double* loop_M2;
    DevBuf<double> pool_d;
    DevBuf<int> pool_i;
    size_t lds_bytes;
    int wg_per_cu;
    int use_wave = 0;
    double* fm_forms = nullptr;
    DevBuf<double> fm_compact;
    DevBuf<int> fm_walk_i; size_t fm_walk_cap = 0;
    FaParams fa_P; int fa_valid = 0, fa_disabled = 0;
    DevBuf<int> fa_need; size_t fa_need_cap = 0;
    DevBuf<char> fw_chain;
    struct FmpcStretch* st_cur = nullptr;
    std::atomic<int> st_steps{0}, st_launches{0};
    DevBuf<double> ao_scr;
    FlParams fs_P; FlStepIn fs_I; int fs_valid = 0, fs_disabled = 0, fs_min_batch = FMPC_PRODUCT_MIN_BATCH_DEFAULT;
    FlParams fl_P; int fl_valid = 0, fl_disabled = 0;
    FwModel wave;
    DevBuf<double> wave_pool_d;
    DevBuf<int> wave_pool_i;
    size_t wave_lds = 0;
    DevBuf<double> sh_fac, sh_rs; DevBuf<int> sh_ok; DevBuf<double> sh_scratch;
    double sh_k = 0.0; int sh_valid = 0, sh_enabled = 0;
    DevBuf<double> cold_d;
    int pn_enabled = 0, pn_valid = 0, pn_mp = 0;
    int last_path = 0;
    size_t pn_lds = 0;
    DevBuf<double> pn_pool;
    size_t pn_o_simg, pn_o_limg, pn_o_bt, pn_o_aimg, pn_o_vec, pn_o_ucon, pn_o_dump, pn_doubles;
    DevBuf<int> pn_cnt;
    int pn_split_last = 0;
    DevBuf<int> gn_list; DevBuf<double> gn_nu; DevBuf<int> gn_cnt; PinnedBuf<int> gn_cnt_host; size_t gn_cap = 0;
    int gn_split = 1;
    DevBuf<int> fa_nflag;
    size_t pn_cap = 0;
    DevBuf<double> pn_gate, pn_epsp, pn_nuws;
    DevBuf<double> pn_rnp; DevBuf<int> pn_list;
    PinnedBuf<int> pn_cnt_host;
    size_t pn_o_dz; int pn_dz_len;
    size_t pn_dz_lds = 0;
    double pn_rd2_0 = 0.0, pn_rp2c = 0.0;
    int inv_enabled = 0, inv_valid = 0, inv_jks = 0, inv_max_batch = 768, inv_last = 0; double inv_k = 0.0;
    int inv_failed = 0; double inv_failed_k = 0.0;
    DevBuf<double> inv_jimg, inv_nuc, inv_eimg;
    DevBuf<double> inv_jst, inv_nucst; int inv_fuse = 0;
    DevBuf<double> inv_jimg2; int inv_jks2 = 0;
    DevBuf<double> lp_v; int lp_hint = 0;
    std::vector<double> hm_J4, hm_nuc; double hm_J4_k = 0.0; int hm_J4_valid = 0;
    DevBuf<double> fm_pool; int fm_valid = 0, fm_disabled = 0; double fm_k = 0.0; FmParams fm_P; DevBuf<int> fm_need;
    std::vector<double> hm_m1, hm_m2;
    std::vector<double> hm_Q2, hm_Qf2, hm_ql, hm_qfl, hm_xf, hm_blocks;
    std::vector<int> hm_idxD, hm_idx1, hm_idx2;
    DevBuf<int> pn_sched; int pn_nsf = 0, pn_nsb = 0, pn_limg_cap = 0;
    std::vector<double> hm_R2, hm_rl, hm_umin, hm_umax, hm_umid, hm_xmid, hm_bt, hm_a1, hm_a2;
    int generic_ok;
    int prefer_tiled;
    int generic_big;
    int prec = FMPC_PREC_F64;
    int refine = 0;
    int refine_last = 0;
    int force_tiled = 0;
    struct Tiled { int ready = 0, NB = 0, NW = 0; size_t lds = 0; DevBuf<char> pool; DevBuf<int> ipool; DevBuf<double> bm; FtModel V; } tl[2];
    struct Bank {
        int count = 0, t = 0, nblk = 0, table_ready = 0, prepared[2] = {0, 0};
        size_t plain_stride = 0, pad_stride = 0, yimg_stride = 0;
        DevBuf<double> plain, pad; DevBuf<char> yimg; DevBuf<int> ipool;
    } bank;
    struct BankFactor {
        int valid = 0, count = 0, t = 0, prepared[2] = {0, 0};
        double k = 0.0; size_t stride = 0;
        DevBuf<char> fac; DevBuf<int> flag;
    } bkf;
    int bank_last_stored = 0;
    struct BankFirst {
        int valid = 0, count = 0, disabled = 0, prepared = 0;
        double k = 0.0, cst_k = 0.0; int cst_valid = 0; size_t stride = 0, oK = 0, ou = 0, oE = 0, oe = 0, oEp = 0, oep = 0, od = 0, osc = 0;
        DevBuf<double> ops, scratch, cst; DevBuf<int> flag, need, list, cnt;
    } bfm;
    int bank_last_first = 0;
    int bank_first_dispatch = 0;
    DevBuf<double> tl_ws; int tl_prepared = 0;
    int tl_last_nw = 0;
    int z_ld = 0;
    int small_tiled = 1;
    int small_nw = 4;
    std::vector<double> hm_b;
    std::vector<double> hm_a1f, hm_a2f;
    int denseQ;
    int denseR;
    std::vector<double> hm_r2full;
    std::vector<double> hm_q2m, hm_qf2m, hm_xm, hm_xfm;
    DevBuf<double> ramp_du;
    DevBuf<double> ramp_ws;
    int ramp_lds_ok = 0, ramp_force_ws = 0;
    std::vector<double> hm_dumin, hm_dumax;
    int rc_disabled = 0, rc_valid = 0, rc_failed = 0, rc_last = 0; double rc_k = 0.0, rc_failed_k = 0.0;
    DevBuf<double> rc_pool; FrColdParams rc_P;
    DevBuf<double> rc_ws;
    DevBuf<double> rc_nu; DevBuf<int> rc_si; size_t rc_cap = 0;
    hipEvent_t ev = nullptr; std::atomic<int> ev_valid{0}; std::atomic<hipStream_t> last_stream{nullptr};
    std::mutex mu;
    std::mutex host_mu;
    DevBuf<double> ws;
    DevBuf<double> zs;
    DevBuf<double> rec_w; int rec_ready = 0, rec_panel = 0; size_t rec_oQf = 0, rec_oR = 0;
    DevBuf<double> rec_j;
    DevBuf<double> rec_f;
    DevBuf<double> kkt_part;
    DevBuf<char> stage;
    PinnedBuf<char> pin; void* pin_dev = nullptr;

    ~fmpc_handle_s() { if (ev) (void)hipEventDestroy(ev); }
};

static inline int fmpc_prec_t(const fmpc_handle_s* h) { return h->prec == FMPC_PREC_F32_MIXED ? 1 : 0; }

struct FmpcSolve {
    int batch;
    const double* x0; const double* x0_pre; const double* w; const double* z_init; const double* nu0;
    int n_newton; double k;
    double* z_out; double* nu_out; int* status; int* iters; double* step;
    double* u0_out;
    hipStream_t stream;
    int ldz;
};
static inline int fmpc_max_iter(const FmpcSolve& s) { return s.n_newton > 0 ? s.n_newton : 1000; }

struct FmpcTiledPlan { int NWu; size_t ldsu; int grid; size_t slot; };

int fmpc_guard_begin(fmpc_handle h, hipStream_t stream);
void fmpc_guard_end(fmpc_handle h, hipStream_t stream);
bool fmpc_capturing(hipStream_t stream);
int fmpc_scratch_z(fmpc_handle h, int batch, hipStream_t stream);
int fmpc_tiled_ensure(fmpc_handle h, int t, hipStream_t stream);
int fmpc_tiled_plan(fmpc_handle h, int t, int batch, hipStream_t stream, int nw_override, int grid_hint, FmpcTiledPlan* out);
```

### mpc-sensorlessao_amd/csrc/fmpc_host.cpp

```cpp
#include "fmpc_host.h"
#include "fmpc_bank.h"
#include "../../include/fastmpc.h"
#include "fmpc_noise.h"
#include "fmpc_atm.h"

#include <algorithm>
#include <cmath>
#include <math.h>
#include <stdio.h>
#include <stdlib.h>

bool fmpc_host_is_diag(const double* M, int n) {
    for (int c = 0; c < n; ++c)
        for (int r = 0; r < n; ++r)
            if (r != c && fmpc_host_cm(M, n, r, c) != 0.0) return false;
    return true;
}

bool fmpc_host_spd_inverse(const std::vector<double>& A, int n, std::vector<double>& inv) {
    typedef long double ld;
    std::vector<ld> L((size_t)n * n, 0.0L), Li((size_t)n * n, 0.0L);
    for (int c = 0; c < n; ++c) {
        ld d = A[c * n + c];
        for (int k = 0; k < c; ++k) d -= L[c * n + k] * L[c * n + k];
// ... 1166 lines not shown
    if (ngroups < 1) ngroups = 1;
    const int wpg_max = (tiles_used + 3) / 4 > 0 ? (tiles_used + 3) / 4 : 1;
    auto wpg_of = [&](int L) { const int w = slots / (ngroups * L); return w < 1 ? 1 : (w > wpg_max ? wpg_max : w); };
    for (int i = 0; i < nsteps; ++i) lane_of_step[i] = 0;
    *wpg_out = wpg_of(1);
    if (nsteps <= 1) return 1;
    std::vector<int> cls(nsteps), first, len;
    for (int j = 0; j < nsteps; ++j) {
        int rep = j;
        for (int i = 0; i < j; ++i) if (supersedes[j] >> i & 1u) { rep = first[cls[i]]; break; }
        if (rep == j) { cls[j] = (int)first.size(); first.push_back(j); len.push_back(1); }
        else { cls[j] = cls[rep]; ++len[cls[j]]; }
    }
    const int nc = (int)first.size();
    std::vector<int> order(nc);
    for (int c = 0; c < nc; ++c) order[c] = c;
    for (int a = 1; a < nc; ++a)
        for (int b = a; b > 0 && len[order[b]] > len[order[b - 1]]; --b) { const int t = order[b]; order[b] = order[b - 1]; order[b - 1] = t; }
    int Lmax = slots / ngroups < 1 ? 1 : slots / ngroups;
    if (Lmax > nc) Lmax = nc;
    if (cap >= 1 && Lmax > cap) Lmax = cap;
    if (cap < 1) Lmax = 1;
    int bestL = 1; long best = -1;
    std::vector<int> lane_of_cls(nc), best_lanes(nc, 0), load;
    for (int L = 1; L <= Lmax; ++L) {
        load.assign(L, 0);
        for (int o = 0; o < nc; ++o) {
            int to = 0;
            for (int l = 1; l < L; ++l) if (load[l] < load[to]) to = l;
            lane_of_cls[order[o]] = to; load[to] += len[order[o]];
        }
        int H = 0;
        for (int l = 0; l < L; ++l) if (load[l] > H) H = load[l];
        const int w = wpg_of(L), R = (tiles_used + 4 * w - 1) / (4 * w);
        const long cost = (long)H * (R + FMPC_LANE_START_ROUNDS);
        if (best < 0 || cost < best) { best = cost; bestL = L; best_lanes = lane_of_cls; }
    }
    for (int j = 0; j < nsteps; ++j) lane_of_step[j] = best_lanes[cls[j]];
    *wpg_out = wpg_of(bestL);
    return bestL;
}

extern "C" int fmpc_debug_plan_lanes(int nsteps, const unsigned* supersedes, int ngroups, int slots, int tiles_used, int cap, int* lane_of_step,
                                     int* lanes, int* wpg) {
    if (nsteps < 0 || nsteps > 32 || (nsteps && (!supersedes || !lane_of_step)) || !lanes || !wpg) return -1;
    int dummy = 0;
    *lanes = fmpc_host_plan_lanes(nsteps, supersedes, ngroups, slots, tiles_used, cap, nsteps ? lane_of_step : &dummy, wpg);
    return 0;
}

void fmpc_host_estimator_qranges(int len, int ndiv, const double* D_re, const double* D_im, std::vector<int>& qr) {
    const int nblk = len / 16, nks = len / 4;
    const size_t npx = (size_t)len * len;
    qr.assign((size_t)2 * nblk, 0);
    for (int b = 0; b < nblk; ++b) {
        int lo = nks, hi = 0;
        for (int Q = 0; Q < nks; ++Q) {
            bool any = false;
            for (int k = 0; k < ndiv && !any; ++k)
                for (int x = 4 * Q; x < 4 * Q + 4 && !any; ++x)
                    for (int y = 16 * b; y < 16 * b + 16; ++y) {
                        const size_t o = (size_t)k * npx + (size_t)x * len + y;
                        if (D_re[o] != 0.0 || D_im[o] != 0.0) { any = true; break; }
                    }
            if (any) { if (Q < lo) lo = Q; hi = Q + 1; }
        }
        if (hi <= lo) { lo = 0; hi = 0; }
        qr[2 * b] = lo; qr[2 * b + 1] = hi;
    }
}

int fmpc_host_zernike_modes(int N, int* n_out, int* m_out) {
    if (N < 0) return 0;
    int j = 0;
    for (int n = 0; n <= N; ++n)
        for (int m = -n; m <= n; m += 2, ++j) {
            if (n_out) n_out[j] = n;
            if (m_out) m_out[j] = m;
        }
    return j;
}

void fmpc_host_zernike_coefficients(double coef[FMPC_ZERNIKE_NCOEF], unsigned short off[FMPC_ZERNIKE_MAXN + 1][8]) {
    double fact[FMPC_ZERNIKE_MAXN + 1];
    fact[0] = 1.0;
    for (int i = 1; i <= FMPC_ZERNIKE_MAXN; ++i) fact[i] = fact[i - 1] * i;
    int o = 0;
    for (int n = 0; n <= FMPC_ZERNIKE_MAXN; ++n) {
        for (int h = 0; h < 8; ++h) off[n][h] = 0;
        for (int ma = n & 1; ma <= n; ma += 2) {
            off[n][ma / 2] = (unsigned short)o;
            for (int s = 0; s <= (n - ma) / 2; ++s)
                coef[o++] = (1 - 2 * (s & 1)) * fact[n - s] / fact[s] / fact[(n - ma) / 2 - s] / fact[(n + ma) / 2 - s];
        }
    }
}

double fmpc_host_mean_square(const double* v, int cnt) {
    double s = 0.0;
    for (int i = 0; i < cnt; ++i) s += v[i] * v[i];
    return cnt > 0 ? s / cnt : 0.0;
}

int fmpc_host_noise_check(const fmpc_noise* nz, int batch, int sigma_only) {
    if (!nz) return FMPC_E_NULL;
    if (nz->mode != FMPC_NOISE_SIGMA && nz->mode != FMPC_NOISE_SNR_MEASURED) return FMPC_E_DIM;
    if (sigma_only && nz->mode != FMPC_NOISE_SIGMA) return FMPC_E_DIM;
    if (batch < 0 || nz->first < 0 || nz->first > (1ll << 32) || nz->first + (long long)batch > (1ll << 32)) return FMPC_E_DIM;
    if (!std::isfinite(nz->value)) return FMPC_E_DIM;
    if (nz->mode == FMPC_NOISE_SIGMA && nz->value < 0.0) return FMPC_E_DIM;
    if (nz->mode == FMPC_NOISE_SNR_MEASURED && nz->sigma_dev) return FMPC_E_DIM;
    return FMPC_OK;
}

extern "C" int fmpc_philox4x32_10(const unsigned int counter[4], const unsigned int key[2], unsigned int out[4]) {
    if (!counter || !key || !out) return FMPC_E_NULL;
    uint32_t c[4] = {counter[0], counter[1], counter[2], counter[3]}, k[2] = {key[0], key[1]}, x[4];
    fmpc_philox4x32_10_block(c, k, x);
    for (int i = 0; i < 4; ++i) out[i] = x[i];
    return FMPC_OK;
}

extern "C" int fmpc_noise_normal_host(double* out, int batch, int p, long long ld, const fmpc_noise* nz) {
    if (!out || !nz) return FMPC_E_NULL;
    const int rc = fmpc_host_noise_check(nz, batch, 1);
    if (rc != FMPC_OK) return rc;
    if (p < 1 || (ld != 0 && ld < p)) return FMPC_E_DIM;
    if (nz->sigma_dev || nz->step_dev) return FMPC_E_DIM;
    if (ld == 0) ld = p;
    for (int r = 0; r < batch; ++r)
        for (int i = 0; i < p; ++i)
            out[(size_t)r * ld + i] = fmpc_noise_scaled(nz->value, fmpc_noise_normal(nz->seed, nz->step, (uint32_t)(nz->first + r), (uint32_t)i));
    return FMPC_OK;
}

extern "C" int fmpc_atm_covariance_host(int n, const double* rho, double r0, double L0, double* out) {
    if (!rho || !out) return FMPC_E_NULL;
    if (n < 0 || !(r0 > 0.0) || !(L0 > 0.0) || !std::isfinite(r0) || !std::isfinite(L0)) return FMPC_E_DIM;
    const double pi = 3.14159265358979323846;
    const double ratio = pow(L0 / r0, 5.0 / 3.0), lead = pow(24.0 * tgamma(6.0 / 5.0) / 5.0, 5.0 / 6.0);
    const double cst = lead * (tgamma(11.0 / 6.0) / (pow(2.0, 5.0 / 6.0) * pow(pi, 8.0 / 3.0))) * ratio;
    const double var = lead * (tgamma(11.0 / 6.0) * tgamma(5.0 / 6.0) / (2.0 * pow(pi, 8.0 / 3.0))) * ratio;
    for (int i = 0; i < n; ++i) {
        if (!(rho[i] >= 0.0) || !std::isfinite(rho[i])) return FMPC_E_DIM;
        const double u = 2.0 * pi * rho[i] / L0;
        out[i] = u != 0.0 ? cst * pow(u, 5.0 / 6.0) * std::cyl_bessel_k(5.0 / 6.0, u) : var;
    }
    return FMPC_OK;
}

int fmpc_host_atm_check(int W, double pitch, double r0, double L0, int q, const int* stencil) {
    if (W < 3 || !(pitch > 0.0) || !(r0 > 0.0) || !(L0 > 0.0) || !std::isfinite(pitch) || !std::isfinite(r0) || !std::isfinite(L0)) return FMPC_E_DIM;
    if (q < 1) return FMPC_E_DIM;
    for (int j = 0; j < q && j <= FMPC_ATM_MAXQ; ++j)
        if (stencil[j] < 1 || stencil[j] > W || (j > 0 && stencil[j] <= stencil[j - 1])) return FMPC_E_DIM;
    if (q > FMPC_ATM_MAXQ || (long long)q * W > FMPC_ATM_MAXK) return FMPC_E_UNSUPPORTED;
    return FMPC_OK;
}

int fmpc_host_atm_default_stencil(int W, int* stencil) {
    int q = 0;
    for (int s = 1; s <= W - 1 && q < FMPC_ATM_MAXQ; s *= 2) stencil[q++] = s;
    return q;
}

static bool atm_chol_packed(std::vector<long double>& L, int N) {
    for (int r = 0; r < N; ++r) {
        long double* lr = L.data() + (size_t)r * (r + 1) / 2;
        for (int c = 0; c <= r; ++c) {
            const long double* lc = L.data() + (size_t)c * (c + 1) / 2;
            long double s = lr[c];
            for (int k = 0; k < c; ++k) s -= lr[k] * lc[k];
            if (c == r) {
                if (!(s > 0.0L) || !std::isfinite((double)s)) return false;
                lr[c] = sqrtl(s);
            } else {
                lr[c] = s / lc[c];
            }
        }
    }
    return true;
}

int fmpc_host_atm_extruders(int W, double pitch, double r0, double L0, int q, const int* stencil, bool all, FmpcAtmExtruders& out) {
    const int N = q * W;
    out.A.assign(q + 1, std::vector<double>());
    out.B.assign(q + 1, std::vector<double>());
    std::vector<int> dss(1, 0);
    for (int a = 0; a < q; ++a) {
        dss.push_back(stencil[a]);
        for (int b = a + 1; b < q; ++b) dss.push_back(stencil[b] - stencil[a]);
    }
    std::sort(dss.begin(), dss.end());
    dss.erase(std::unique(dss.begin(), dss.end()), dss.end());
    std::vector<std::vector<long double>> cov(dss.size(), std::vector<long double>(W));
    {
        std::vector<double> rho(W), c(W);
        for (size_t d = 0; d < dss.size(); ++d) {
            for (int i = 0; i < W; ++i) rho[i] = pitch * hypot((double)dss[d], (double)i);
            if (fmpc_atm_covariance_host(W, rho.data(), r0, L0, c.data()) != FMPC_OK) return FMPC_E_UNSUPPORTED;
            for (int i = 0; i < W; ++i) {
                if (!std::isfinite(c[i])) return FMPC_E_UNSUPPORTED;
                cov[d][i] = c[i];
            }
        }
    }
    auto C = [&](int ds, int di) -> long double {
        ds = ds < 0 ? -ds : ds; di = di < 0 ? -di : di;
        return cov[std::lower_bound(dss.begin(), dss.end(), ds) - dss.begin()][di];
    };
    std::vector<long double> L((size_t)N * (N + 1) / 2);
    for (int a = 0; a < q; ++a)
        for (int i = 0; i < W; ++i) {
            long double* lr = L.data() + (size_t)(a * W + i) * (a * W + i + 1) / 2;
            for (int b = 0; b <= a; ++b)
                for (int k = 0; k < W && b * W + k <= a * W + i; ++k) lr[b * W + k] = C(stencil[a] - stencil[b], i - k);
        }
    if (!atm_chol_packed(L, N)) return FMPC_E_UNSUPPORTED;
    std::vector<long double> Y((size_t)W * N);
    for (int w = 0; w < W; ++w) {
        long double* y = Y.data() + (size_t)w * N;
        for (int r = 0; r < N; ++r) {
            const long double* lr = L.data() + (size_t)r * (r + 1) / 2;
            long double s = C(stencil[r / W], r % W - w);
            for (int k = 0; k < r; ++k) s -= lr[k] * y[k];
            y[r] = s / lr[r];
        }
    }
    std::vector<long double> a(N), S((size_t)W * (W + 1) / 2);
    for (int j = all ? 0 : q; j <= q; ++j) {
        const int Nj = j * W;
        out.A[j].assign((size_t)W * Nj, 0.0);
        for (int w = 0; w < W; ++w) {
            for (int r = 0; r < Nj; ++r) a[r] = Y[(size_t)w * N + r];
            for (int r = Nj - 1; r >= 0; --r) {
                const long double* lr = L.data() + (size_t)r * (r + 1) / 2;
                a[r] /= lr[r];
                for (int k = 0; k < r; ++k) a[k] -= lr[k] * a[r];
            }
            for (int r = 0; r < Nj; ++r) out.A[j][(size_t)w * Nj + r] = (double)a[r];
        }
        for (int w = 0; w < W; ++w)
            for (int v = 0; v <= w; ++v) {
                long double s = C(0, w - v);
                const long double *yw = Y.data() + (size_t)w * N, *yv = Y.data() + (size_t)v * N;
                for (int r = 0; r < Nj; ++r) s -= yw[r] * yv[r];
                S[(size_t)w * (w + 1) / 2 + v] = s;
            }
        if (!atm_chol_packed(S, W)) return FMPC_E_UNSUPPORTED;
        out.B[j].assign((size_t)W * W, 0.0);
        for (int w = 0; w < W; ++w)
            for (int v = 0; v <= w; ++v) out.B[j][(size_t)w * W + v] = (double)S[(size_t)w * (w + 1) / 2 + v];
    }
    return FMPC_OK;
}

void fmpc_host_atm_images(int W, int q, const FmpcAtmExtruders& X, std::vector<double>& img, unsigned long long* off) {
    const int Wp4 = fmpc_atm_wp4(W), NT = fmpc_atm_tiles(W);
    size_t total = 0;
    for (int j = 0; j <= q; ++j) { off[j] = total; total += fmpc_atm_img_doubles(W, j); }
    img.assign(total, 0.0);
    for (int j = 0; j <= q; ++j) {
        const int KS = (j + 1) * (Wp4 / 4);
        for (int tile = 0; tile < NT; ++tile)
            for (int ks = 0; ks < KS; ++ks)
                for (int lane = 0; lane < 64; ++lane) {
                    const int row = 16 * tile + (lane & 15), kk = 4 * ks + (lane >> 4), part = kk / Wp4, i = kk % Wp4;
                    if (row >= W || i >= W) continue;
                    img[off[j] + ((size_t)tile * KS + ks) * 64 + lane] =
                        part < j ? X.A[j][(size_t)row * (j * W) + (size_t)part * W + i] : X.B[j][(size_t)row * W + i];
                }
    }
}

extern "C" int fmpc_atm_extruder_host(int W, double pitch, double r0, double L0, int q, const int* stencil, double* A, double* B) {
    const bool first_line = stencil && q == 0;
    if (!B || (!A && !first_line)) return FMPC_E_NULL;
    int def[FMPC_ATM_MAXQ], one = 1;
    if (!stencil) {
        if (W < 3) return FMPC_E_DIM;
        q = fmpc_host_atm_default_stencil(W, def);
        stencil = def;
    }
    const int rc = first_line ? fmpc_host_atm_check(W, pitch, r0, L0, 1, &one) : fmpc_host_atm_check(W, pitch, r0, L0, q, stencil);
    if (rc != FMPC_OK) return rc;
    FmpcAtmExtruders X;
    const int rb = fmpc_host_atm_extruders(W, pitch, r0, L0, q, stencil, false, X);
    if (rb != FMPC_OK) return rb;
    if (!first_line) memcpy(A, X.A[q].data(), X.A[q].size() * sizeof(double));
    memcpy(B, X.B[q].data(), X.B[q].size() * sizeof(double));
    return FMPC_OK;
}

extern "C" int fmpc_atm_displacement_host(long long k, double px_per_step, long long* lines, double* frac) {
    if (!lines || !frac) return FMPC_E_NULL;
    if (k < 0 || !std::isfinite(px_per_step)) return FMPC_E_DIM;
    const double d = fabs((double)k * px_per_step);
    if (!(d < 4503599627370496.0)) return FMPC_E_UNSUPPORTED;
    const double n = floor(d);
    *lines = (long long)n;
    *frac = d - n;
    return FMPC_OK;
}
```

### mpc-sensorlessao_amd/csrc/fmpc_host.h

```cpp
#pragma once
#include <stddef.h>
#include <string.h>
#include <vector>

#include "fmpc_panel_layout.h"

inline double fmpc_host_cm(const double* M, int rows, int r, int c) { return M[(size_t)r + (size_t)c * rows]; }
bool fmpc_host_is_diag(const double* M, int n);
bool fmpc_host_spd_inverse(const std::vector<double>& A, int n, std::vector<double>& inv);

void fmpc_host_add_AXBt(std::vector<double>& out, const std::vector<double>& A, const std::vector<double>& X,
                        const std::vector<double>& B, int n, double sign);

void fmpc_host_y_blocks(int n, int T, bool var2, bool has_xf, const std::vector<double>& a1, const std::vector<double>& a2,
                        const std::vector<double>& X, const std::vector<double>& Xf,
                        std::vector<std::vector<double>>& blocks, std::vector<int>& idxD, std::vector<int>& idx1, std::vector<int>& idx2);

struct FmpcPanelIn {
    int n, m, T, nb, mp, var_order;
    size_t pool_doubles, o_simg, o_limg, o_bt, o_aimg, o_vec, o_ucon, o_dz;
    int limg_cap;
    const double *umax, *umin, *umid, *xmid, *R2, *rl, *Q2, *Qf2, *ql, *qfl, *xf;
    const double *bt;
    const double *a1, *a2;
    const double *blocks;
    const int *idxD, *idx1, *idx2;
};
struct FmpcPanelOut {
    std::vector<double> pool;
    std::vector<int> sched;
    int nsf, nsb, nimg, valid;
    double rp2c, rd2_0;
};
void fmpc_host_panel_layout(int n, int m, int T, int nb, int mp, FmpcPanelIn& L, size_t* o_dump, size_t* total, int* dz_len);
int fmpc_host_build_panel(const FmpcPanelIn& In, double k, FmpcPanelOut& Out);

inline void fmpc_host_key_push(std::vector<double>& key, const double* p, size_t cnt) {
    key.push_back(p ? (double)cnt : -1.0);
    if (p) key.insert(key.end(), p, p + cnt);
}

template <class H>
struct FmpcLru {
    struct Entry { std::vector<double> key; H h; std::vector<double> ramp; unsigned long long stamp; };
    std::vector<Entry> items;
    unsigned long long clock = 0;
    size_t capacity;
    explicit FmpcLru(size_t cap) : capacity(cap) {}
    Entry* find(const std::vector<double>& key) {
        for (Entry& e : items)
            if (e.key.size() == key.size() && memcmp(e.key.data(), key.data(), key.size() * sizeof(double)) == 0) return &e;
        return nullptr;
    }
    template <class D>
    Entry* insert(std::vector<double>&& key, H h, D destroy) {
        if (items.size() >= capacity) {
            size_t old = 0;
            for (size_t i = 1; i < items.size(); ++i) if (items[i].stamp < items[old].stamp) old = i;
            destroy(items[old].h);
            items.erase(items.begin() + old);
        }
        items.push_back(Entry{std::move(key), h, {}, 0});
        return &items.back();
    }
    void touch(Entry* e) { e->stamp = ++clock; }
    template <class D>
    void clear(D destroy) { for (Entry& e : items) destroy(e.h); items.clear(); }
};

#define FMPC_INV_SCALE 1048576.0
bool fmpc_host_inverse_images(int n, int T, int nb, bool var2, int jks, int jks2, const double* a1, const double* a2,
                              const std::vector<double>& nu, std::vector<double>& img, std::vector<double>& nuc,
                              std::vector<double>& jst, std::vector<double>& ncs, std::vector<double>& img2,
                              std::vector<double>& eimg, std::vector<double>& J4, std::vector<double>& nuc4);

#define FM_NC_MAX 108
struct FmpcFirstIn {
    int n, m, T, nb, var2, has_xf;
    const double *bt, *umax, *umin, *umid, *xmid, *R2, *rl, *a1, *a2, *m1, *m2, *xf;
    const double *J;
    const double *nuc;
    double k;
};
struct FmpcFirstOut {
    int nc;
    std::vector<double> K0t, u0c, E, e, Ep, ep;
    std::vector<double> Ec, Epc;
    double e0, ep0, normE, norme, normEp, normep;
};
void fmpc_host_build_first_move(const FmpcFirstIn& In, FmpcFirstOut& Out);

#define FA_KS 14
#define FA_KC (4 * FA_KS)
struct FmpcAffineIn {
    int n, m, T, nb, has_xf, ncJ;
    const double *bt, *umax, *umin, *umid, *xmid, *R2, *rl, *Q2, *Qf2, *ql, *qfl, *a1, *a2;
    const double *J, *nuc;
    double k;
};
#define FA_NU_KS 7
struct FmpcNuStage { int tb, nu, nd, ub; };
#define FMPC_NU_CUT(cnt, p, parts) ((cnt) * (p) / (parts))
struct FmpcAffineOut {
    int rows, tiles;
    int nu_rows, nu_tiles;
    std::vector<double> Kz;
    std::vector<double> img;
    int jbase;
    std::vector<FmpcNuStage> plan;
    std::vector<double> imgG;
};
void fmpc_host_build_affine(const FmpcAffineIn& In, FmpcAffineOut& Out);
void fmpc_host_plan_nu(int m, int n, int T, std::vector<FmpcNuStage>& plan);
int fmpc_host_nu_work(const std::vector<FmpcNuStage>& plan);
int fmpc_host_nu_parts(int T, int work, int W);
int fmpc_host_nu_swap(int T, int parts, int W);
#define FMPC_LANE_START_ROUNDS 3
int fmpc_host_plan_lanes(int nsteps, const unsigned* supersedes, int ngroups, int slots, int tiles_used, int cap, int* lane_of_step, int* wpg);
void fmpc_host_mfma_images(const double* M, int rows, int cols, int ks, std::vector<double>& img);
struct FmpcLoopImages { std::vector<double> imgU, imgE, imgEp, imgB; };
void fmpc_host_build_loop_images(const FmpcFirstOut& O, int n, int m, int ks, bool fused, const double* bt, FmpcLoopImages& out);
void fmpc_host_mfma_a_images(const double* M, int rows, std::vector<double>& img);

struct FmpcRampColdIn {
    int n, m, T, nb, var2, has_xf;
    const double *bt, *a1, *a2;
    const double *umax, *umin, *umid, *xmid, *R2, *rl, *Q2, *Qf2, *ql, *qfl, *xf, *dumin, *dumax;
    double k;
};
struct FmpcRampColdOut {
    int valid;
    std::vector<double> g0;
    std::vector<double> Gf;
    std::vector<double> phib_u, phib_x;
    std::vector<double> gbar_u, gbar_x;
    std::vector<double> hd;
    std::vector<double> erb;
    std::vector<double> cpb;
    std::vector<double> betab;
    std::vector<double> Yinv;
    std::vector<double> G;
    std::vector<double> Xiu0t;
    std::vector<double> y0c;
};
void fmpc_host_build_ramp_cold(const FmpcRampColdIn& In, FmpcRampColdOut& Out);

int fmpc_host_estimator_gain(const double* A_s, int p, int nx, std::vector<double>& G);
void fmpc_host_estimator_dft_images(int len, int d, int first, std::vector<double>& img);
void fmpc_host_estimator_qranges(int len, int ndiv, const double* D_re, const double* D_im, std::vector<int>& qr);

double fmpc_host_mean_square(const double* v, int cnt);
struct fmpc_noise_s;
int fmpc_host_noise_check(const struct fmpc_noise_s* nz, int batch, int sigma_only);

#define FMPC_ZERNIKE_MAXN 14
#define FMPC_ZERNIKE_NCOEF 204
int fmpc_host_zernike_modes(int N, int* n_out, int* m_out);
void fmpc_host_zernike_coefficients(double coef[FMPC_ZERNIKE_NCOEF], unsigned short off[FMPC_ZERNIKE_MAXN + 1][8]);

int fmpc_host_atm_check(int W, double pitch, double r0, double L0, int q, const int* stencil);
int fmpc_host_atm_default_stencil(int W, int* stencil);
struct FmpcAtmExtruders { std::vector<std::vector<double>> A, B; };
int fmpc_host_atm_extruders(int W, double pitch, double r0, double L0, int q, const int* stencil, bool all, FmpcAtmExtruders& out);
void fmpc_host_atm_images(int W, int q, const FmpcAtmExtruders& X, std::vector<double>& img, unsigned long long* off);
```

### mpc-sensorlessao_amd/csrc/fmpc_kernel_affine.hip

```cpp
#include <hip/hip_runtime.h>
#include <math.h>
#include <stdlib.h>
#include "fmpc_device.h"
#include "fmpc_affine.h"
#include "../../include/fastmpc.h"

#ifdef FW_TIMING
__device__ unsigned long long fa_trace[1024 * 8];
extern "C" int fmpc_debug_affine_trace(unsigned long long* out) {
    return hipMemcpyFromSymbol(out, HIP_SYMBOL(fa_trace), sizeof(unsigned long long) * 1024 * 8) == hipSuccess ? 0 : -1;
}
#define FA_TICK(k) do { if (tid == 0 && blockIdx.x < 1024) fa_trace[blockIdx.x * 8 + (k)] = (unsigned long long)wall_clock64(); } while (0)
#else
#define FA_TICK(k)
#endif
typedef double d4a __attribute__((ext_vector_type(4)));
typedef double d2a __attribute__((ext_vector_type(2)));
#define FA_MFMA(a, b, c) __builtin_amdgcn_mfma_f64_16x16x4f64((a), (b), (c), 0, 0, 0)
#define FA_THREADS 256
#define FA_CT 4

__device__ __forceinline__ void fa_load_a(double (&A)[FA_KS], const double* img, int tile, int lane) {
    const double* ip = img + (size_t)tile * FA_KS * 64 + lane;
#pragma unroll
    for (int q = 0; q < FA_KS; ++q) A[q] = ip[q * 64];
}

__device__ __forceinline__ void fa_request_a(double (&A)[FA_KS], const double* img, int tile, int lane) {
    const double* ip = img + (size_t)tile * FA_KS * 64 + lane;
    const double* ip2 = ip + 8 * 64;
#define FA_LD(q, base, off) asm volatile("global_load_dwordx2 %0, %1, off offset:" #off : "=v"(A[q]) : "v"(base))
    FA_LD(0, ip, 0); FA_LD(1, ip, 512); FA_LD(2, ip, 1024); FA_LD(3, ip, 1536); FA_LD(4, ip, 2048); FA_LD(5, ip, 2560); FA_LD(6, ip, 3072); FA_LD(7, ip, 3584);
    FA_LD(8, ip2, 0); FA_LD(9, ip2, 512); FA_LD(10, ip2, 1024); FA_LD(11, ip2, 1536); FA_LD(12, ip2, 2048); FA_LD(13, ip2, 2560);
#undef FA_LD
}
template <int BEHIND>
__device__ __forceinline__ void fa_await_a(double (&A)[FA_KS]) {
    asm volatile("s_waitcnt vmcnt(%14)"
                 : "+v"(A[0]), "+v"(A[1]), "+v"(A[2]), "+v"(A[3]), "+v"(A[4]), "+v"(A[5]), "+v"(A[6]), "+v"(A[7]), "+v"(A[8]), "+v"(A[9]),
                   "+v"(A[10]), "+v"(A[11]), "+v"(A[12]), "+v"(A[13])
                 : "n"(BEHIND));
}

__device__ __forceinline__ bool fa_decide(const FaParams& P, double qe, double qp, double rdl, double dn2) {
    const double dn = sqrt(dn2);
    double e2 = qe + P.e0, rp2 = qp + P.ep0;
    const double ce = 4096.0 * 2.220446049250313e-16;
    const double de = ce * (dn2 * P.normE + 2.0 * P.norme * dn + fabs(P.e0));
    const double dp = ce * (dn2 * P.normEp + 2.0 * P.normep * dn + fabs(P.ep0));
    e2 += de;
    rp2 = rp2 - dp > 0.0 ? rp2 - dp : 0.0;
    const double rho2 = rp2 + rdl;
    const bool fin = rp2 < 1e300 && rho2 < 1e300 && e2 < 1e300 && e2 >= 0.0;
    return fin && (rp2 > 4e-16 || rho2 > 4e-12) && e2 <= 0.5 * rho2;
}

template <bool ZOUT, bool NT = false>
__global__ void __launch_bounds__(FA_THREADS, 2) fmpc_cold_affine(FaParams P) {
    __shared__ double sD[FA_KS * FA_CT * 64];
#define FA_SD(ct, cc, k) sD[((((k) >> 2) * FA_CT + (ct)) * 4 + ((k) & 3)) * 16 + (cc)]
    __shared__ double sF[4][3][16];
    const int tid0 = threadIdx.x;
    constexpr int n = FA_N;
    const int wg = (int)blockIdx.x;
    const int ln = wg / P.wgs_per_lane, wl = wg - ln * P.wgs_per_lane;
    const int gi = wl / P.wgs_per_group, slot = wl - gi * P.wgs_per_group;
    const int s_begin = P.lane_begin[ln], s_end = P.lane_begin[ln + 1];
    const int tiles = P.tiles_used, rows = P.rows, m = P.m;
    const int tstep = 4 * P.wgs_per_group;
    { const int tid = tid0; FA_TICK(0); (void)tid; }
    if (wg == 0 && tid0 == 0 && P.handed) *P.handed = 0;
    double A[FA_KS], An[FA_KS];
    const int p0 = gi * FA_CT * 16;
    const int rounds = tiles / tstep;
    const bool forms_wg = P.wgs_per_group >= 8 && rounds >= 2 && slot >= P.wgs_per_group - FA_CT;
    const int nskip = (P.wgs_per_group >= 8 && rounds >= 2) ? 4 * FA_CT : 0;
    const int skip0 = (rounds - 1) * tstep + (P.wgs_per_group - FA_CT) * 4;
    const int tfull = (rounds - (forms_wg ? 1 : 0)) * tstep;
    for (int s = s_begin; s < s_end; ++s) {
    int tid = tid0;
    asm volatile("" : "+v"(tid));
    const int lane = tid & 63, wv = tid >> 6, g = lane >> 4, c = lane & 15;
    double* dump = P.dump + ((blockIdx.x & 15) * FA_THREADS + tid);
    const FaStep& S = P.steps[s];
    const double* const x0_s = S.x0; const double* const x0p_s = S.x0p; const double* const nu0_s = S.nu0;
    double* const zout_s = S.zout; double* const nuout_s = S.nuout; double* const u0out_s = S.u0out;
    int* const status_s = S.status; int* const iters_s = S.iters; double* const step_s = S.step; int* const need_s = S.need;
    int tile = slot * 4 + wv;
    if (s != s_begin) __syncthreads();
    fa_request_a(A, P.img, tile < tiles ? tile : 0, lane);
    {
        const int np = P.batch - p0 < FA_CT * 16 ? P.batch - p0 : FA_CT * 16;
        const double* s0 = x0_s + (size_t)p0 * n;
        const double* s1 = x0p_s ? x0p_s + (size_t)p0 * n : s0;
        double v0[7], v1[7];
#pragma unroll
        for (int j = 0; j < 7; ++j) {
            const int idx = tid + FA_THREADS * j, ic = idx < np * n ? idx : 0;
            v0[j] = s0[ic]; v1[j] = s1[ic];
        }
#pragma unroll
        for (int j = 0; j < 7; ++j) {
            const int idx = tid + FA_THREADS * j;
            if (idx < FA_CT * 16 * n) {
                const int pr = idx / n, k = idx - pr * n;
                const bool on = idx < np * n;
                FA_SD(pr >> 4, pr & 15, k) = on ? v0[j] : 0.0;
                FA_SD(pr >> 4, pr & 15, n + k) = (on && x0p_s) ? v1[j] : 0.0;
            }
        }
        if (tid < FA_CT * 16) { FA_SD(tid >> 4, tid & 15, 2 * n) = 1.0; FA_SD(tid >> 4, tid & 15, 2 * n + 1) = 0.0; }
    }
    __syncthreads();
    FA_TICK(1);
    for (int fct = P.wgs_per_group - 1 - slot; fct < FA_CT; fct += P.wgs_per_group) {
        if (fct < 0 || p0 + fct * 16 >= P.batch) continue;
        const int t = wv;
        double E1[FA_KS], E2[FA_KS], Df[FA_KS];
        fa_load_a(E1, P.imgE, t, lane);
        fa_load_a(E2, P.imgEp, t, lane);
        const int k = 16 * t + c;
        const double le = P.elin[k], lp = P.eplin[k];
        double rdl[4] = {P.rd2_0, P.rd2_0, P.rd2_0, P.rd2_0};
        if (nu0_s && t == 0) {
            double xa[4][2];
#pragma unroll
            for (int r = 0; r < 4; ++r) {
                const int pr = p0 + fct * 16 + 4 * r + g < P.batch ? p0 + fct * 16 + 4 * r + g : P.batch - 1;
                const double* nu = nu0_s + (size_t)pr * P.nb * n;
#pragma unroll
                for (int j = 0; j < 2; ++j) {
                    const int e = c + 16 * j, ec = e < n ? e : 0;
                    xa[r][j] = P.dx0T[ec] + nu[(P.T - 1) * n + ec] + (P.has_xf ? nu[P.T * n + ec] : 0.0);
                }
            }
#pragma unroll
            for (int r = 0; r < 4; ++r) {
                double acc = xa[r][0] * xa[r][0] + (c + 16 < n ? xa[r][1] * xa[r][1] : 0.0);
                acc += __shfl_xor(acc, 1, 64); acc += __shfl_xor(acc, 2, 64); acc += __shfl_xor(acc, 4, 64); acc += __shfl_xor(acc, 8, 64);
                rdl[r] = acc;
            }
        }
#pragma unroll
        for (int q = 0; q < FA_KS; ++q) Df[q] = sD[(q * FA_CT + fct) * 64 + lane];
        d4a ce = {0, 0, 0, 0}, cp = {0, 0, 0, 0};
#pragma unroll
        for (int q = 0; q < FA_KS; ++q) { ce = FA_MFMA(Df[q], E1[q], ce); cp = FA_MFMA(Df[q], E2[q], cp); }
        double qe[4], qp[4], dn2[4];
#pragma unroll
        for (int r = 0; r < 4; ++r) {
            const double dv = k < 2 * n ? FA_SD(fct, 4 * r + g, k < 2 * n ? k : 0) : 0.0;
            qe[r] = dv * (ce[r] + le); qp[r] = dv * (cp[r] + lp); dn2[r] = dv * dv;
#pragma unroll
            for (int o = 1; o < 16; o <<= 1) { qe[r] += __shfl_xor(qe[r], o, 64); qp[r] += __shfl_xor(qp[r], o, 64); dn2[r] += __shfl_xor(dn2[r], o, 64); }
            if (c == 0) { sF[t][0][4 * r + g] = qe[r]; sF[t][1][4 * r + g] = qp[r]; sF[t][2][4 * r + g] = dn2[r]; }
        }
        __syncthreads();
        if (t == 0 && c == 0) {
#pragma unroll
            for (int r = 0; r < 4; ++r) {
                const int i = 4 * r + g, pp = p0 + fct * 16 + i;
                if (pp < P.batch) {
                    const double se = (sF[0][0][i] + sF[1][0][i]) + (sF[2][0][i] + sF[3][0][i]);
                    const double sp = (sF[0][1][i] + sF[1][1][i]) + (sF[2][1][i] + sF[3][1][i]);
                    const double sn = (sF[0][2][i] + sF[1][2][i]) + (sF[2][2][i] + sF[3][2][i]);
                    const bool clear = fa_decide(P, se, sp, rdl[r], sn);
                    need_s[pp] = clear ? 0 : 1;
                    if (!clear && P.nflag) atomicAdd(P.nflag, 1);
                    if (clear) {
                        if (status_s) status_s[pp] = FMPC_OK;
                        if (iters_s) iters_s[pp] = 1;
                        if (step_s) for (int q = 0; q < P.step_ld; ++q) step_s[(size_t)pp * P.step_ld + q] = q == 0 ? 1.0 : -1.0;
                    }
                }
            }
        }
        __syncthreads();
    }
    {
        const int wg_w = slot * 4 + wv;
        const int nleft = nskip + (tiles - rounds * tstep);
        for (int task = wg_w; task < nleft * FA_CT; task += tstep) {
            const int j = task / FA_CT, ct = task % FA_CT;
            const int lt = j < nskip ? skip0 + j : rounds * tstep + (j - nskip);
            double Al[FA_KS], Dl[FA_KS];
            fa_load_a(Al, P.img, lt, lane);
#pragma unroll
            for (int q = 0; q < FA_KS; ++q) Dl[q] = sD[(q * FA_CT + ct) * 64 + lane];
            d4a acc = {0, 0, 0, 0};
#pragma unroll
            for (int q = 0; q < FA_KS; ++q) acc = FA_MFMA(Dl[q], Al[q], acc);
            const int row = 16 * lt + c;
#pragma unroll
            for (int r = 0; r < 4; ++r) {
                const int pp = (gi * FA_CT + ct) * 16 + 4 * r + g;
                if (ZOUT && lt < P.tiles && row < rows && pp < P.batch) zout_s[(size_t)pp * P.ldz + row] = acc[r];
                if (ZOUT && lt >= P.tiles && row - 16 * P.tiles < P.nu_rows && pp < P.batch) nuout_s[(size_t)pp * P.nu_rows + (row - 16 * P.tiles)] = acc[r];
                if (u0out_s != nullptr && row < m && pp < P.batch) u0out_s[(size_t)pp * m + row] = acc[r];
            }
        }
    }
    if (tile >= tfull) { fa_await_a<0>(A); continue; }
    double D[FA_CT][FA_KS];
#pragma unroll
    for (int ct = 0; ct < FA_CT; ++ct)
#pragma unroll
        for (int q = 0; q < FA_KS; ++q) D[ct][q] = sD[(q * FA_CT + ct) * 64 + lane];
    FA_TICK(4);
    fa_await_a<0>(A);
    FA_TICK(5);
    for (; tile < tfull; tile += tstep) {
        const int nxt = tile + tstep < tfull ? tile + tstep : tile;
        fa_request_a(An, P.img, nxt, lane);
        d4a acc[FA_CT];
#pragma unroll
        for (int ct = 0; ct < FA_CT; ++ct) acc[ct] = (d4a){0, 0, 0, 0};
#pragma unroll
        for (int q = 0; q < FA_KS; ++q)
#pragma unroll
            for (int ct = 0; ct < FA_CT; ++ct) acc[ct] = FA_MFMA(D[ct][q], A[q], acc[ct]);
        const int row = 16 * tile + c;
        if (ZOUT) {
            const bool isnu = tile >= P.tiles;
            const int rloc = isnu ? row - 16 * P.tiles : row, rcnt = isnu ? P.nu_rows : rows, ld = isnu ? P.nu_rows : P.ldz;
            double* obase = isnu ? nuout_s : zout_s;
            const unsigned voz = (unsigned)(g * ld + rloc);
            const bool rok = rloc < rcnt;
#pragma unroll
            for (int ct = 0; ct < FA_CT; ++ct)
#pragma unroll
                for (int r = 0; r < 4; ++r) {
                    const int pb = (gi * FA_CT + ct) * 16 + 4 * r;
                    double* zb = obase + (size_t)pb * ld + voz;
                    double* dst = (rok && pb + g < P.batch) ? zb : dump;
                    if (NT) __builtin_nontemporal_store(acc[ct][r], dst);
                    else *dst = acc[ct][r];
                }
        }
        if (!ZOUT || (u0out_s != nullptr && 16 * tile < m)) {
            const unsigned vou = (unsigned)(g * m + row);
            const bool rok = row < m;
#pragma unroll
            for (int ct = 0; ct < FA_CT; ++ct)
#pragma unroll
                for (int r = 0; r < 4; ++r) {
                    const int pb = (gi * FA_CT + ct) * 16 + 4 * r;
                    double* ub = u0out_s + (size_t)pb * m + vou;
                    double* dst = (rok && pb + g < P.batch) ? ub : dump;
                    *dst = acc[ct][r];
                }
        }
#ifdef FW_TIMING
        if (tile == slot * 4 + wv) { asm volatile("s_nop 0" :: "v"(acc[0][0]), "v"(acc[1][0]), "v"(acc[2][0]), "v"(acc[3][0])); FA_TICK(6); }
#endif
        fa_await_a<16>(An);
#pragma unroll
        for (int q = 0; q < FA_KS; ++q) A[q] = An[q];
#ifdef FW_TIMING
        if (tile == slot * 4 + wv) FA_TICK(2);
#endif
    }
    FA_TICK(3);
    }
}

hipError_t fmpc_launch_affine(FaParams P, int num_cu, hipStream_t stream, const unsigned* supersedes) {
    if (P.n != 27 || 2 * P.n + 2 > FA_KC || 7 * FA_THREADS < FA_CT * 16 * P.n) return hipErrorInvalidValue;
    if (P.nsteps < 0 || P.nsteps > FMPC_STRETCH_MAX) return hipErrorInvalidValue;
    if (P.nsteps == 0) {
        P.nsteps = 1;
        P.steps[0] = {P.x0, P.x0p, P.nu0, P.zout, P.nuout, P.u0out, P.status, P.iters, P.step, P.need};
    }
    P.x0 = P.steps[0].x0; P.zout = P.steps[0].zout; P.nuout = P.steps[0].nuout; P.u0out = P.steps[0].u0out;
    bool aligned = true;
    for (int s = 0; s < P.nsteps; ++s) {
        const FaStep& S = P.steps[s];
        if (!S.x0 || !S.need || (S.zout == nullptr) != (P.zout == nullptr) || (S.nuout == nullptr) != (P.nuout == nullptr) ||
            (S.u0out == nullptr) != (P.u0out == nullptr)) return hipErrorInvalidValue;
        aligned = aligned && ((size_t)S.zout & 127) == 0;
    }
    if (!P.zout && !P.u0out) return hipErrorInvalidValue;
    const int ncol = (P.batch + 15) / 16, ngroups = (ncol + FA_CT - 1) / FA_CT;
    P.tiles_used = P.zout ? P.tiles + (P.nuout ? P.nu_tiles : 0) : (P.m + 15) / 16;
    if (P.ldz < P.rows) P.ldz = P.rows;
    static const bool no_nt = [] { const char* e = getenv("FMPC_AFFINE_NO_NT"); return e && e[0] == '1'; }();
    const bool nt = P.zout && !no_nt && P.ldz % 16 == 0 && aligned;
    int cap = FMPC_STRETCH_LANES_DEFAULT;
    if (P.nsteps > 1) { const char* e = getenv("FMPC_STRETCH_LANES"); if (e && e[0]) cap = atoi(e); }
    if (cap < 1 || !supersedes) cap = 1;
    int lane_of[FMPC_STRETCH_MAX], wpg = 1;
    P.nlanes = fmpc_host_plan_lanes(P.nsteps, supersedes, ngroups, 2 * num_cu, P.tiles_used, cap, lane_of, &wpg);
    P.wgs_per_group = wpg;
    P.wgs_per_lane = ngroups * wpg;
    {
        FaStep in_chain_order[FMPC_STRETCH_MAX];
        for (int s = 0; s < P.nsteps; ++s) in_chain_order[s] = P.steps[s];
        int k = 0;
        for (int l = 0; l < P.nlanes; ++l) {
            P.lane_begin[l] = k;
            for (int s = 0; s < P.nsteps; ++s) if (lane_of[s] == l) P.steps[k++] = in_chain_order[s];
        }
        for (int l = P.nlanes; l <= FMPC_STRETCH_MAX; ++l) P.lane_begin[l] = k;
    }
    const int grid = P.nlanes * ngroups * wpg;
    if (P.zout && P.imgG) {
        const char* e = getenv("FMPC_AFFINE_DIRECT");
        if (!(e && e[0] == '1')) return fmpc_launch_affine_nu(P, grid, nt, stream);
    }
    if (P.zout && nt) hipLaunchKernelGGL((fmpc_cold_affine<true, true>), dim3(grid), dim3(FA_THREADS), 0, stream, P);
    else if (P.zout) hipLaunchKernelGGL((fmpc_cold_affine<true, false>), dim3(grid), dim3(FA_THREADS), 0, stream, P);
    else hipLaunchKernelGGL((fmpc_cold_affine<false, false>), dim3(grid), dim3(FA_THREADS), 0, stream, P);
    return hipGetLastError();
}
```

### mpc-sensorlessao_amd/csrc/fmpc_kernel_affine_nu.hip

```cpp
#include <hip/hip_runtime.h>
#include <math.h>
#include <stdlib.h>
#include "fmpc_affine_dev.h"

#ifdef FW_TIMING
__device__ unsigned long long fa_nu_trace[1024 * 8];
extern "C" int fmpc_debug_affine_nu_trace(unsigned long long* out) {
    return hipMemcpyFromSymbol(out, HIP_SYMBOL(fa_nu_trace), sizeof(unsigned long long) * 1024 * 8) == hipSuccess ? 0 : -1;
}
#define FA_TICK(k) do { if (tid == 0 && blockIdx.x < 1024) fa_nu_trace[blockIdx.x * 8 + (k)] = (unsigned long long)wall_clock64(); } while (0)
#else
#define FA_TICK(k)
#endif

typedef __attribute__((address_space(1))) double fa_gdouble;
__device__ __forceinline__ fa_gdouble* fa_pick(bool ok, double* a, double* b) {
    unsigned long long mk = 0ull - (unsigned long long)ok;
    asm volatile("" : "+v"(mk));
    return (fa_gdouble*)(((unsigned long long)a & mk) | ((unsigned long long)b & ~mk));
}

template <bool NT, bool FULL>
__device__ __forceinline__ void fa_nu_store(const FaParams& P, const d4a (&acc)[FA_CT], int tile, int gi, int lane,
                                            double* zout_s, double* nuout_s, double* dump) {
    asm volatile("" : "+v"(lane));
    const int g = lane >> 4, c = lane & 15;
    const bool isnu = !FULL && tile >= P.tiles;
    const int r0 = isnu ? 16 * (tile - P.tiles) : 16 * tile, rcnt = isnu ? P.nu_rows : P.rows, ld = isnu ? P.nu_rows : P.ldz;
    double* obase = (isnu ? nuout_s : zout_s) + (size_t)(gi * FA_CT * 16) * ld + r0;
    const unsigned voz = (unsigned)(g * ld + c);
    const bool rok = r0 + c < rcnt;
#pragma unroll
    for (int ct = 0; ct < FA_CT; ++ct)
#pragma unroll
        for (int r = 0; r < 4; ++r) {
            const int pb = (gi * FA_CT + ct) * 16 + 4 * r;
            double* zb = obase + (size_t)((ct * 16 + 4 * r) * ld) + voz;
            fa_gdouble* dst = FULL ? (fa_gdouble*)zb : fa_pick(rok && pb + g < P.batch, zb, dump);
            if (NT) __builtin_nontemporal_store(acc[ct][r], dst);
            else *dst = acc[ct][r];
            if (!FULL) __builtin_amdgcn_sched_barrier(0);
        }
}

template <bool NT, bool FULL>
__device__ __forceinline__ void fa_nu_utiles(const FaParams& P, double (&A)[FA_NU_KS], const d4a (&n0)[FA_CT], const d4a (&n1)[FA_CT],
                                             int ub, int ue, int ui, int gi, int lane, double* zout_s, double* dump) {
    double An[FA_NU_KS];
    int tile = ub;
    do {
        fa_request_g(An, P.imgG, ui + (tile + 1 < ue ? tile + 1 : tile) - ub, lane);
        d4a acc[FA_CT];
#pragma unroll
        for (int ct = 0; ct < FA_CT; ++ct) acc[ct] = (d4a){0, 0, 0, 0};
#pragma unroll
        for (int q = 0; q < FA_NU_KS; ++q)
#pragma unroll
            for (int ct = 0; ct < FA_CT; ++ct) acc[ct] = FA_MFMA(q < 4 ? n0[ct][q & 3] : n1[ct][q & 3], A[q], acc[ct]);
        fa_nu_store<NT, FULL>(P, acc, tile, gi, lane, zout_s, nullptr, dump);
        fa_await_g<16>(An);
#pragma unroll
        for (int q = 0; q < FA_NU_KS; ++q) A[q] = An[q];
    } while (++tile < ue);
}

template <bool NT, bool U0>
__device__ __forceinline__ void fa_nu_direct(const FaParams& P, double (&A)[FA_KS], double (&An)[FA_KS], const double (&D)[FA_CT][FA_KS],
                                             int db, int de, int after, int gi, int lane, double* zout_s, double* nuout_s, double* u0out_s, double* dump) {
    const int m = P.m;
    int tile = db;
    do {
        if (!U0) fa_request_a(An, P.img, tile + 1 < de ? tile + 1 : after, lane);
        d4a acc[FA_CT];
#pragma unroll
        for (int ct = 0; ct < FA_CT; ++ct) acc[ct] = (d4a){0, 0, 0, 0};
#pragma unroll
        for (int q = 0; q < FA_KS; ++q)
#pragma unroll
            for (int ct = 0; ct < FA_CT; ++ct) acc[ct] = FA_MFMA(D[ct][q], A[q], acc[ct]);
        if (U0) {
            asm volatile("" :: "v"(acc[0][0]), "v"(acc[1][0]), "v"(acc[2][0]), "v"(acc[3][0]));
            fa_request_a(A, P.img, tile + 1 < de ? tile + 1 : after, lane);
        }
        fa_nu_store<NT, false>(P, acc, tile, gi, lane, zout_s, nuout_s, dump);
        if (U0) {
            int lu = lane;
            asm volatile("" : "+v"(lu));
            const int g = lu >> 4, c = lu & 15;
            const int row = 16 * tile + c;
            const unsigned vou = (unsigned)(g * m + row);
            const bool rok = row < m;
#pragma unroll
            for (int ct = 0; ct < FA_CT; ++ct)
#pragma unroll
                for (int r = 0; r < 4; ++r) {
                    const int pb = (gi * FA_CT + ct) * 16 + 4 * r;
                    double* ubp = u0out_s + (size_t)pb * m + vou;
                    fa_gdouble* dst = fa_pick(rok && pb + g < P.batch, ubp, dump);
                    *dst = acc[ct][r];
                    __builtin_amdgcn_sched_barrier(0);
                }
        }
        if (U0) fa_await_a<32>(A);
        else {
            fa_await_a<16>(An);
#pragma unroll
            for (int q = 0; q < FA_KS; ++q) A[q] = An[q];
        }
    } while (++tile < de);
}

struct FaNuItem { int ub, ue, ui, db, de, jt; };
__device__ __forceinline__ FaNuItem fa_nu_item(const FaParams& P, int it) {
    FaNuItem I = {0, 0, 0, 0, 0, -1};
    const int nst = P.T * P.nparts;
    if (it < nst) {
        const int js = it / P.nparts, part = it - js * P.nparts;
        const int j = js == P.swap ? 0 : (js == 0 ? P.swap : js);
        const int tb = P.plan[4 * j], nu = P.plan[4 * j + 1], nd = P.plan[4 * j + 2], u0 = FMPC_NU_CUT(nu, part, P.nparts);
        I.ub = tb + u0; I.ue = tb + FMPC_NU_CUT(nu, part + 1, P.nparts); I.ui = P.plan[4 * j + 3] + u0;
        I.db = tb + nu + FMPC_NU_CUT(nd, part, P.nparts); I.de = tb + nu + FMPC_NU_CUT(nd, part + 1, P.nparts);
        if (I.ue > I.ub) I.jt = P.jbase + 2 * (j - 1);
    } else {
        I.db = P.tiles + 4 * (it - nst);
        I.de = I.db + 4 < P.tiles + P.nu_tiles ? I.db + 4 : P.tiles + P.nu_tiles;
    }
    return I;
}

template <bool NT>
__global__ void __launch_bounds__(FA_THREADS, 2) fmpc_cold_nu(FaParams P) {
    __shared__ double sD[FA_KS * FA_CT * 64];
    __shared__ double sF[4][3][16];
    const int tid0 = threadIdx.x;
    const int wg = (int)blockIdx.x;
    const int ln = wg / P.wgs_per_lane, wl = wg - ln * P.wgs_per_lane;
    const int gi = wl / P.wgs_per_group, slot = wl - gi * P.wgs_per_group;
    const int s_begin = P.lane_begin[ln], s_end = P.lane_begin[ln + 1];
    const int nwav = 4 * P.wgs_per_group;
    { const int tid = tid0; FA_TICK(0); (void)tid; }
    if (wg == 0 && tid0 == 0 && P.handed) *P.handed = 0;
    const int p0 = gi * FA_CT * 16;
    for (int s = s_begin; s < s_end; ++s) {
    int tid = tid0;
    asm volatile("" : "+v"(tid));
    const int wv = __builtin_amdgcn_readfirstlane(tid >> 6);
    const FaStep& S = P.steps[s];
    const double* const x0_s = S.x0; const double* const x0p_s = S.x0p; const double* const nu0_s = S.nu0;
    double* const zout_s = S.zout; double* const nuout_s = S.nuout; double* const u0out_s = S.u0out;
    int* const status_s = S.status; int* const iters_s = S.iters; double* const step_s = S.step; int* const need_s = S.need;
    if (s != s_begin) __syncthreads();
    fa_stage(sD, P, x0_s, x0p_s, p0, tid);
    __syncthreads();
    FA_TICK(1);
    fa_forms(sD, sF, P, slot, wv, tid & 63, p0, nu0_s, need_s, status_s, iters_s, step_s);
    FA_TICK(2);
    for (int it = slot * 4 + wv; it < P.nitems; it += nwav) {
        int lane = tid & 63;
        asm volatile("" : "+v"(lane));
        const FaNuItem I = fa_nu_item(P, it);
        if (I.de <= I.db && I.jt < 0) continue;
        double A[FA_KS], An[FA_KS];
        fa_request_a(A, P.img, I.de > I.db ? I.db : I.jt, lane);
        double* dump = P.dump + ((blockIdx.x & 15) * FA_THREADS + wv * 64 + lane);
        const int ub = I.ub, ue = I.ue, ui = I.ui, db = I.db, de = I.de, jt = I.jt;
        double D[FA_CT][FA_KS];
#pragma unroll
        for (int ct = 0; ct < FA_CT; ++ct)
#pragma unroll
            for (int q = 0; q < FA_KS; ++q) D[ct][q] = sD[(q * FA_CT + ct) * 64 + lane];
        fa_await_a<0>(A);
        if (de > db) {
            const int after = jt >= 0 ? jt : db;
            if (u0out_s != nullptr && 16 * db < P.m) fa_nu_direct<NT, true>(P, A, An, D, db, de, after, gi, lane, zout_s, nuout_s, u0out_s, dump);
            else fa_nu_direct<NT, false>(P, A, An, D, db, de, after, gi, lane, zout_s, nuout_s, u0out_s, dump);
        }
#ifdef FW_TIMING
        if (it == slot * 4 + wv) FA_TICK(4);
#endif
        if (jt < 0) continue;
        d4a n0[FA_CT], n1[FA_CT];
        double G[FA_NU_KS];
        fa_request_a(An, P.img, jt + 1, lane);
        fa_request_g(G, P.imgG, ui, lane);
#pragma unroll
        for (int ct = 0; ct < FA_CT; ++ct) { n0[ct] = (d4a){0, 0, 0, 0}; n1[ct] = (d4a){0, 0, 0, 0}; }
#pragma unroll
        for (int q = 0; q < FA_KS; ++q) n0[0] = FA_MFMA(A[q], D[0][q], n0[0]);
        fa_await_a<FA_NU_KS>(An);
#pragma unroll
        for (int q = 0; q < FA_KS; ++q) n1[0] = FA_MFMA(An[q], D[0][q], n1[0]);
#pragma unroll
        for (int ct = 1; ct < FA_CT; ++ct)
#pragma unroll
            for (int q = 0; q < FA_KS; ++q) { n0[ct] = FA_MFMA(A[q], D[ct][q], n0[ct]); n1[ct] = FA_MFMA(An[q], D[ct][q], n1[ct]); }
        fa_await_g<0>(G);
#ifdef FW_TIMING
        if (it == slot * 4 + wv) { asm volatile("s_nop 0" :: "v"(n1[0][0]), "v"(n1[1][0]), "v"(n1[2][0]), "v"(n1[3][0])); FA_TICK(5); }
#endif
        if ((gi + 1) * FA_CT * 16 <= P.batch) fa_nu_utiles<NT, true>(P, G, n0, n1, ub, ue, ui, gi, lane, zout_s, dump);
        else fa_nu_utiles<NT, false>(P, G, n0, n1, ub, ue, ui, gi, lane, zout_s, dump);
#ifdef FW_TIMING
        if (it == slot * 4 + wv) FA_TICK(6);
#endif
    }
    FA_TICK(3);
    }
}

hipError_t fmpc_launch_affine_nu(FaParams P, int grid, bool nt, hipStream_t stream) {
    if (P.n != FA_N || !P.zout || !P.imgG || !P.plan || P.nu_work <= 0 || grid < 1) return hipErrorInvalidValue;
    P.nparts = fmpc_host_nu_parts(P.T, P.nu_work, 4 * P.wgs_per_group);
    P.swap = fmpc_host_nu_swap(P.T, P.nparts, 4 * P.wgs_per_group);
    P.nitems = P.T * P.nparts + (P.nuout ? (P.nu_tiles + 3) / 4 : 0);
    if (nt) hipLaunchKernelGGL((fmpc_cold_nu<true>), dim3(grid), dim3(FA_THREADS), 0, stream, P);
    else hipLaunchKernelGGL((fmpc_cold_nu<false>), dim3(grid), dim3(FA_THREADS), 0, stream, P);
    return hipGetLastError();
}
```

Before: 96.26 million.

## Deal affine nu work to waves via host-built load-balanced schedule table

Replaces the fixed round-robin item loop in the affine nu kernel with a host-computed, load-levelled per-wave schedule of segments (forms units, direct tile runs, u-tile units). The schedule is cached in a device arena keyed by wave count and output flags. The forms computation is restructured so each wave handles a whole column tile independently, removing the two block barriers and the shared reduction array. Shuffles now use ds_bpermute directly. The cost is host-side planning, an uploaded table, and a device sync when a cache slot is evicted.

Result: no change. 97.06 million, median of 6 (+0.8%).

```diff
diff --git a/mpc-sensorlessao_amd/csrc/fmpc_affine.h b/mpc-sensorlessao_amd/csrc/fmpc_affine.h
--- a/mpc-sensorlessao_amd/csrc/fmpc_affine.h
+++ b/mpc-sensorlessao_amd/csrc/fmpc_affine.h
@@ -1,6 +1,7 @@
 #pragma once
 #include <hip/hip_runtime.h>
 #include "fmpc_host.h"
+#include "fmpc_alloc.h"
 #include "../../include/fastmpc.h"
 
 #define FA_N 27
@@ -33,9 +34,16 @@
     const double* imgG;
     const int* plan;
     int jbase, nu_work;
-    int nparts, nitems, swap;
+    const int* deal; int deal_seg, deal_tl;
+};
+
+#define FA_DEAL_SLOTS 16
+struct FaDealCache {
+    struct Entry { int W = 0, key = -1, seg_off = 0, tl_off = 0; } e[FA_DEAL_SLOTS];
+    DevBuf<int> arena; size_t slot_ints = 0;
+    int next = 0;
 };
 
 #define FMPC_STRETCH_LANES_DEFAULT FMPC_STRETCH_MAX
-hipError_t fmpc_launch_affine(FaParams P, int num_cu, hipStream_t stream, const unsigned* supersedes = nullptr);
-hipError_t fmpc_launch_affine_nu(FaParams P, int grid, bool nt, hipStream_t stream);
+hipError_t fmpc_launch_affine(FaParams P, int num_cu, hipStream_t stream, const unsigned* supersedes = nullptr, FaDealCache* deals = nullptr);
+hipError_t fmpc_launch_affine_nu(FaParams P, int grid, bool nt, hipStream_t stream, FaDealCache* deals);
diff --git a/mpc-sensorlessao_amd/csrc/fmpc_affine_dev.h b/mpc-sensorlessao_amd/csrc/fmpc_affine_dev.h
--- a/mpc-sensorlessao_amd/csrc/fmpc_affine_dev.h
+++ b/mpc-sensorlessao_amd/csrc/fmpc_affine_dev.h
@@ -50,8 +50,10 @@
     const double dn = sqrt(dn2);
     double e2 = qe + P.e0, rp2 = qp + P.ep0;
     const double ce = 4096.0 * 2.220446049250313e-16;
-    const double de = ce * (dn2 * P.normE + 2.0 * P.norme * dn + fabs(P.e0));
-    const double dp = ce * (dn2 * P.normEp + 2.0 * P.normep * dn + fabs(P.ep0));
+    double two = 2.0;
+    asm volatile("" : "+v"(two));
+    const double de = ce * (dn2 * P.normE + two * P.norme * dn + fabs(P.e0));
+    const double dp = ce * (dn2 * P.normEp + two * P.normep * dn + fabs(P.ep0));
     e2 += de;
     rp2 = rp2 - dp > 0.0 ? rp2 - dp : 0.0;
     const double rho2 = rp2 + rdl;
@@ -81,77 +83,94 @@
             FA_SD(pr >> 4, pr & 15, n + k) = (on && x0p_s) ? v1[j] : 0.0;
         }
     }
-    double zero = 0.0;
-    asm volatile("" : "+v"(zero));
-    if (tid < FA_CT * 16) { FA_SD(tid >> 4, tid & 15, 2 * n) = 1.0; FA_SD(tid >> 4, tid & 15, 2 * n + 1) = zero; }
+    double zero = 0.0, one = 1.0;
+    asm volatile("" : "+v"(zero), "+v"(one));
+    if (tid < FA_CT * 16) { FA_SD(tid >> 4, tid & 15, 2 * n) = one; FA_SD(tid >> 4, tid & 15, 2 * n + 1) = zero; }
 }
 
-__device__ __forceinline__ void fa_forms(const double* sD, double (&sF)[4][3][16], const FaParams& P, int slot, int wv, int lane, int p0,
-                                         const double* nu0_s, int* need_s, int* status_s, int* iters_s, double* step_s) {
+__device__ __forceinline__ double fa_shfl_xor(double v, int o, int lane) {
+    const int at = (lane ^ o) << 2;
+    const int lo = __builtin_amdgcn_ds_bpermute(at, __double2loint(v)), hi = __builtin_amdgcn_ds_bpermute(at, __double2hiint(v));
+    return __hiloint2double(hi, lo);
+}
+
+__device__ __forceinline__ void fa_forms_unit(const double* sD, const FaParams& P, int fct, int lane, int p0,
+                                              const double* nu0_s, int* need_s, int* status_s, int* iters_s, double* step_s) {
     constexpr int n = FA_N;
+    if (p0 + fct * 16 >= P.batch) return;
     const int g = lane >> 4, c = lane & 15;
-    for (int fct = P.wgs_per_group - 1 - slot; fct < FA_CT; fct += P.wgs_per_group) {
-        if (fct < 0 || p0 + fct * 16 >= P.batch) continue;
-        const int t = wv;
-        double E1[FA_KS], E2[FA_KS], Df[FA_KS];
-        fa_load_a(E1, P.imgE, t, lane);
-        fa_load_a(E2, P.imgEp, t, lane);
-        const int k = 16 * t + c;
-        const double le = P.elin[k], lp = P.eplin[k];
-        double rdl[4] = {P.rd2_0, P.rd2_0, P.rd2_0, P.rd2_0};
-        if (nu0_s && t == 0) {
-            double xa[4][2];
+    double xa[4][2];
+    if (nu0_s) {
+#pragma unroll
+        for (int r = 0; r < 4; ++r) {
+            const int pr = p0 + fct * 16 + 4 * r + g < P.batch ? p0 + fct * 16 + 4 * r + g : P.batch - 1;
+            const double* nu = nu0_s + (size_t)pr * P.nb * n;
+#pragma unroll
+            for (int j = 0; j < 2; ++j) {
+                const int e = c + 16 * j, ec = e < n ? e : 0;
+                xa[r][j] = P.dx0T[ec] + nu[(P.T - 1) * n + ec] + (P.has_xf ? nu[P.T * n + ec] : 0.0);
+            }
+        }
+    }
+    double Df[FA_KS];
+#pragma unroll
+    for (int q = 0; q < FA_KS; ++q) Df[q] = sD[(q * FA_CT + fct) * 64 + lane];
+    double se[4], sp[4], sn[4];
+#pragma unroll 1
+    for (int tp = 0; tp < 2; ++tp) {
+        double he[4], hp[4], hn[4];
+#pragma unroll
+        for (int h = 0; h < 2; ++h) {
+            const int t = 2 * tp + h;
+            double E1[FA_KS], E2[FA_KS];
+            fa_load_a(E1, P.imgE, t, lane);
+            fa_load_a(E2, P.imgEp, t, lane);
+            const int k = 16 * t + c;
+            const double le = P.elin[k], lp = P.eplin[k];
+            d4a ce = {0, 0, 0, 0}, cp = {0, 0, 0, 0};
+#pragma unroll
+            for (int q = 0; q < FA_KS; ++q) { ce = FA_MFMA(Df[q], E1[q], ce); cp = FA_MFMA(Df[q], E2[q], cp); }
 #pragma unroll
             for (int r = 0; r < 4; ++r) {
-                const int pr = p0 + fct * 16 + 4 * r + g < P.batch ? p0 + fct * 16 + 4 * r + g : P.batch - 1;
-                const double* nu = nu0_s + (size_t)pr * P.nb * n;
+                const double dv = k < 2 * n ? FA_SD(fct, 4 * r + g, k < 2 * n ? k : 0) : 0.0;
+                double qe = dv * (ce[r] + le), qp = dv * (cp[r] + lp), dn2 = dv * dv;
 #pragma unroll
-                for (int j = 0; j < 2; ++j) {
-                    const int e = c + 16 * j, ec = e < n ? e : 0;
-                    xa[r][j] = P.dx0T[ec] + nu[(P.T - 1) * n + ec] + (P.has_xf ? nu[P.T * n + ec] : 0.0);
-                }
-            }
-#pragma unroll
-            for (int r = 0; r < 4; ++r) {
-                double acc = xa[r][0] * xa[r][0] + (c + 16 < n ? xa[r][1] * xa[r][1] : 0.0);
-                acc += __shfl_xor(acc, 1, 64); acc += __shfl_xor(acc, 2, 64); acc += __shfl_xor(acc, 4, 64); acc += __shfl_xor(acc, 8, 64);
-                rdl[r] = acc;
+                for (int o = 1; o < 16; o <<= 1) { qe += fa_shfl_xor(qe, o, lane); qp += fa_shfl_xor(qp, o, lane); dn2 += fa_shfl_xor(dn2, o, lane); }
+                if (h == 0) { he[r] = qe; hp[r] = qp; hn[r] = dn2; }
+                else { he[r] += qe; hp[r] += qp; hn[r] += dn2; }
             }
         }
 #pragma unroll
-        for (int q = 0; q < FA_KS; ++q) Df[q] = sD[(q * FA_CT + fct) * 64 + lane];
-        d4a ce = {0, 0, 0, 0}, cp = {0, 0, 0, 0};
-#pragma unroll
-        for (int q = 0; q < FA_KS; ++q) { ce = FA_MFMA(Df[q], E1[q], ce); cp = FA_MFMA(Df[q], E2[q], cp); }
-        double qe[4], qp[4], dn2[4];
+        for (int r = 0; r < 4; ++r) {
+            if (tp == 0) { se[r] = he[r]; sp[r] = hp[r]; sn[r] = hn[r]; }
+            else { se[r] += he[r]; sp[r] += hp[r]; sn[r] += hn[r]; }
+        }
+    }
+    double rdl[4] = {P.rd2_0, P.rd2_0, P.rd2_0, P.rd2_0};
+    if (nu0_s) {
 #pragma unroll
         for (int r = 0; r < 4; ++r) {
-            const double dv = k < 2 * n ? FA_SD(fct, 4 * r + g, k < 2 * n ? k : 0) : 0.0;
-            qe[r] = dv * (ce[r] + le); qp[r] = dv * (cp[r] + lp); dn2[r] = dv * dv;
+            double acc = xa[r][0] * xa[r][0] + (c + 16 < n ? xa[r][1] * xa[r][1] : 0.0);
+            acc += fa_shfl_xor(acc, 1, lane); acc += fa_shfl_xor(acc, 2, lane); acc += fa_shfl_xor(acc, 4, lane); acc += fa_shfl_xor(acc, 8, lane);
+            rdl[r] = acc;
+        }
+    }
+    if (c == 0) {
+        double one = 1.0;
+        asm volatile("" : "+v"(one));
 #pragma unroll
-            for (int o = 1; o < 16; o <<= 1) { qe[r] += __shfl_xor(qe[r], o, 64); qp[r] += __shfl_xor(qp[r], o, 64); dn2[r] += __shfl_xor(dn2[r], o, 64); }
-            if (c == 0) { sF[t][0][4 * r + g] = qe[r]; sF[t][1][4 * r + g] = qp[r]; sF[t][2][4 * r + g] = dn2[r]; }
-        }
-        __syncthreads();
-        if (t == 0 && c == 0) {
-#pragma unroll
-            for (int r = 0; r < 4; ++r) {
-                const int i = 4 * r + g, pp = p0 + fct * 16 + i;
-                if (pp < P.batch) {
-                    const double se = (sF[0][0][i] + sF[1][0][i]) + (sF[2][0][i] + sF[3][0][i]);
-                    const double sp = (sF[0][1][i] + sF[1][1][i]) + (sF[2][1][i] + sF[3][1][i]);
-                    const double sn = (sF[0][2][i] + sF[1][2][i]) + (sF[2][2][i] + sF[3][2][i]);
-                    const bool clear = fa_decide(P, se, sp, rdl[r], sn);
-                    need_s[pp] = clear ? 0 : 1;
-                    if (!clear && P.nflag) atomicAdd(P.nflag, 1);
-                    if (clear) {
-                        if (status_s) status_s[pp] = FMPC_OK;
-                        if (iters_s) iters_s[pp] = 1;
-                        if (step_s) for (int q = 0; q < P.step_ld; ++q) step_s[(size_t)pp * P.step_ld + q] = q == 0 ? 1.0 : -1.0;
-                    }
+        for (int r = 0; r < 4; ++r) {
+            const int i = 4 * r + g, pp = p0 + fct * 16 + i;
+            if (pp < P.batch) {
+                const bool clear = fa_decide(P, se[r], sp[r], rdl[r], sn[r]);
+                need_s[pp] = clear ? 0 : 1;
+                if (!clear && P.nflag) atomicAdd(P.nflag, 1);
+                if (clear) {
+                    if (status_s) status_s[pp] = FMPC_OK;
+                    if (iters_s) iters_s[pp] = 1;
+                    if (step_s) for (int q = 0; q < P.step_ld; ++q) step_s[(size_t)pp * P.step_ld + q] = q == 0 ? one : -one;
                 }
             }
         }
-        __syncthreads();
     }
 }
diff --git a/mpc-sensorlessao_amd/csrc/fmpc_api.hip b/mpc-sensorlessao_amd/csrc/fmpc_api.hip
--- a/mpc-sensorlessao_amd/csrc/fmpc_api.hip
+++ b/mpc-sensorlessao_amd/csrc/fmpc_api.hip
@@ -688,7 +688,7 @@
         same[j] = S.st[j].same_outputs & ((1u << j) - 1u);
         for (int i = 0; i < j; ++i) if (same[j] >> i & 1u) same[j] |= same[i];
     }
-    if (fmpc_launch_affine(A, S.num_cu, stream, same) != hipSuccess) return FMPC_E_HIP;
+    { const hipError_t e = fmpc_launch_affine(A, S.num_cu, stream, same, &h->fa_deals); if (e != hipSuccess) return e == hipErrorOutOfMemory ? FMPC_E_ALLOC : FMPC_E_HIP; }
     int live[FMPC_STRETCH_MAX], nlive = 0;
     for (int i = 0; i < n; ++i) if (!S.st[i].superseded) live[nlive++] = i;
     int launches = 1;
@@ -1137,7 +1137,7 @@
         h->last_path = FMPC_PATH_PANEL; h->pn_split_last = 0; h->inv_last = 2;
         return FMPC_OK;
     }
-    if (fmpc_launch_affine(A, h->num_cu, s.stream) != hipSuccess) return FMPC_E_HIP;
+    { const hipError_t e = fmpc_launch_affine(A, h->num_cu, s.stream, nullptr, &h->fa_deals); if (e != hipSuccess) return e == hipErrorOutOfMemory ? FMPC_E_ALLOC : FMPC_E_HIP; }
     const int rc = fmpc_launch_flagged(h, s, g3, stride, h->fa_need, no_nflag ? nullptr : nf, zld);
     h->last_path = FMPC_PATH_PANEL; h->pn_split_last = 0; h->inv_last = 2;
     return rc;
diff --git a/mpc-sensorlessao_amd/csrc/fmpc_handle.h b/mpc-sensorlessao_amd/csrc/fmpc_handle.h
--- a/mpc-sensorlessao_amd/csrc/fmpc_handle.h
+++ b/mpc-sensorlessao_amd/csrc/fmpc_handle.h
@@ -30,6 +30,7 @@
     DevBuf<double> fm_compact;
     DevBuf<int> fm_walk_i; size_t fm_walk_cap = 0;
     FaParams fa_P; int fa_valid = 0, fa_disabled = 0;
+    FaDealCache fa_deals;
     DevBuf<int> fa_need; size_t fa_need_cap = 0;
     DevBuf<char> fw_chain;
     struct FmpcStretch* st_cur = nullptr;
diff --git a/mpc-sensorlessao_amd/csrc/fmpc_host.cpp b/mpc-sensorlessao_amd/csrc/fmpc_host.cpp
--- a/mpc-sensorlessao_amd/csrc/fmpc_host.cpp
+++ b/mpc-sensorlessao_amd/csrc/fmpc_host.cpp
@@ -1492,3 +1492,122 @@
     *frac = d - n;
     return FMPC_OK;
 }
+
+namespace {
+struct DealUnit { int kind, a, b, c, d, first, weight; };
+void deal_push(FmpcDealNu& D, std::vector<std::vector<DealUnit>>& per, int w, const DealUnit& u) { per[w].push_back(u); D.load[w] += u.weight; }
+}
+
+void fmpc_host_deal_nu(int m, int n, int T, int W, int parts, bool has_nu_out, bool has_u0, int forms_cts, int nu_tiles, bool levelled,
+                       FmpcDealNu& D) {
+    D = FmpcDealNu();
+    if (W < 1) W = 1;
+    if (parts < 1) parts = 1;
+    D.W = W;
+    D.load.assign(W, 0);
+    std::vector<FmpcNuStage> plan;
+    fmpc_host_plan_nu(m, n, T, plan);
+    const int s = n + m, tiles = (T * s + 15) / 16, jbase = tiles + nu_tiles, nnu = has_nu_out ? nu_tiles : 0;
+    std::vector<std::vector<DealUnit>> per(W);
+    auto uunit = [&](int j, int p) {
+        const int u0 = FMPC_NU_CUT(plan[j].nu, p, parts), u1 = FMPC_NU_CUT(plan[j].nu, p + 1, parts), jt = jbase + 2 * (j - 1);
+        return DealUnit{FMPC_DEAL_UUNIT, plan[j].tb + u0, plan[j].tb + u1, plan[j].ub + u0, jt, jt, u1 > u0 ? FMPC_DEAL_W_NU + FMPC_DEAL_W_UTILE * (u1 - u0) : 0};
+    };
+    auto run = [&](int kind, int cnt) {
+        const int a = (int)D.tl.size() - cnt;
+        return DealUnit{kind, a, cnt, 0, 0, D.tl[a], FMPC_DEAL_W_DIRECT * cnt};
+    };
+    auto first_move = [&](int tile) { return has_u0 && 16 * tile < m; };
+    if (!levelled) {
+        const int wpg = (W + 3) / 4, swap = fmpc_host_nu_swap(T, parts, W);
+        for (int f = 0; f < forms_cts; ++f) {
+            const int w = 4 * (wpg - 1 - f % wpg);
+            deal_push(D, per, w < W ? w : W - 1, DealUnit{FMPC_DEAL_FORMS, f, 0, 0, 0, -1, FMPC_DEAL_W_FORMS});
+        }
+        const int nst = T * parts, nitems = nst + (nnu + 3) / 4;
+        for (int it = 0; it < nitems; ++it) {
+            const int w = it % W;
+            if (it < nst) {
+                const int js = it / parts, p = it - js * parts, j = js == swap ? 0 : (js == 0 ? swap : js);
+                const int d0 = FMPC_NU_CUT(plan[j].nd, p, parts), d1 = FMPC_NU_CUT(plan[j].nd, p + 1, parts), db = plan[j].tb + plan[j].nu + d0;
+                if (d1 > d0) {
+                    for (int t = d0; t < d1; ++t) D.tl.push_back(plan[j].tb + plan[j].nu + t);
+                    deal_push(D, per, w, run(first_move(db) ? FMPC_DEAL_DIRECT_U0 : FMPC_DEAL_DIRECT, d1 - d0));
+                }
+                const DealUnit u = uunit(j, p);
+                if (u.weight > 0) deal_push(D, per, w, u);
+            } else {
+                const int t0 = 4 * (it - nst), t1 = t0 + 4 < nnu ? t0 + 4 : nnu;
+                for (int t = t0; t < t1; ++t) D.tl.push_back(tiles + t);
+                deal_push(D, per, w, run(FMPC_DEAL_NUOUT, t1 - t0));
+            }
+        }
+    } else {
+        std::vector<DealUnit> units;
+        for (int f = 0; f < forms_cts; ++f) units.push_back(DealUnit{FMPC_DEAL_FORMS, f, 0, 0, 0, -1, FMPC_DEAL_W_FORMS});
+        for (int j = 1; j < T; ++j)
+            for (int p = 0; p < parts; ++p) { const DealUnit u = uunit(j, p); if (u.weight > 0) units.push_back(u); }
+        std::stable_sort(units.begin(), units.end(), [](const DealUnit& x, const DealUnit& y) { return x.weight > y.weight; });
+        auto least = [&](const std::vector<int>& L) { int b = 0; for (int w = 1; w < W; ++w) if (L[w] < L[b]) b = w; return b; };
+        std::vector<std::vector<DealUnit>> uf(W);
+        for (const DealUnit& u : units) { const int w = least(D.load); uf[w].push_back(u); D.load[w] += u.weight; }
+        std::vector<int> cls;
+        for (int c = 0; c < 2; ++c)
+            for (int j = 0; j < T; ++j)
+                for (int t = plan[j].tb + plan[j].nu; t < plan[j].tb + plan[j].nu + plan[j].nd; ++t)
+                    if (first_move(t) == (c == 0)) { D.tl.push_back(t); cls.push_back(c == 0 ? FMPC_DEAL_DIRECT_U0 : FMPC_DEAL_DIRECT); }
+        for (int t = 0; t < nnu; ++t) { D.tl.push_back(tiles + t); cls.push_back(FMPC_DEAL_NUOUT); }
+        const int nd = (int)D.tl.size();
+        std::vector<int> cnt(W, 0), L = D.load;
+        for (int i = 0; i < nd; ++i) { const int w = least(L); ++cnt[w]; L[w] += FMPC_DEAL_W_DIRECT; }
+        int at = 0;
+        std::fill(D.load.begin(), D.load.end(), 0);
+        for (int w = 0; w < W; ++w) {
+            for (const DealUnit& u : uf[w]) if (u.kind == FMPC_DEAL_FORMS) deal_push(D, per, w, u);
+            for (int i = at; i < at + cnt[w];) {
+                int e = i + 1;
+                while (e < at + cnt[w] && cls[e] == cls[i]) ++e;
+                deal_push(D, per, w, DealUnit{cls[i], i, e - i, 0, 0, D.tl[i], FMPC_DEAL_W_DIRECT * (e - i)});
+                i = e;
+            }
+            at += cnt[w];
+            for (const DealUnit& u : uf[w]) if (u.kind != FMPC_DEAL_FORMS) deal_push(D, per, w, u);
+        }
+    }
+    D.off.assign(W + 1, 0);
+    for (int w = 0; w < W; ++w) {
+        D.off[w] = (int)D.seg.size() / FMPC_DEAL_SEG;
+        std::stable_partition(per[w].begin(), per[w].end(), [](const DealUnit& u) { return u.kind == FMPC_DEAL_FORMS; });
+        for (size_t i = 0; i < per[w].size(); ++i) {
+            const DealUnit& u = per[w][i];
+            const int after = i + 1 < per[w].size() ? per[w][i + 1].first : u.first;
+            const int rec[FMPC_DEAL_SEG] = {u.kind, u.a, u.b, u.c, u.d, after, u.weight, u.first};
+            D.seg.insert(D.seg.end(), rec, rec + FMPC_DEAL_SEG);
+        }
+    }
+    D.off[W] = (int)D.seg.size() / FMPC_DEAL_SEG;
+}
+
+void fmpc_host_deal_nu_flat(const FmpcDealNu& D, std::vector<int>& flat, int* seg_off, int* tl_off) {
+    const int nseg = (int)D.seg.size() / FMPC_DEAL_SEG;
+    const int so = (4 + D.W + 1 + 7) / 8 * 8, to = so + nseg * FMPC_DEAL_SEG;
+    flat.assign((size_t)to + D.tl.size() + 1, 0);
+    flat[0] = D.W; flat[1] = nseg; flat[2] = (int)D.tl.size(); flat[3] = so;
+    std::copy(D.off.begin(), D.off.end(), flat.begin() + 4);
+    std::copy(D.seg.begin(), D.seg.end(), flat.begin() + so);
+    std::copy(D.tl.begin(), D.tl.end(), flat.begin() + to);
+    if (seg_off) *seg_off = so;
+    if (tl_off) *tl_off = to;
+}
+
+extern "C" int fmpc_debug_deal_nu(int m, int n, int T, int W, int has_nu_out, int has_u0, int nu_tiles, int levelled, int* out, int cap) {
+    if (m < 1 || n < 1 || T < 1 || W < 1 || nu_tiles < 0) return -1;
+    std::vector<FmpcNuStage> plan;
+    fmpc_host_plan_nu(m, n, T, plan);
+    FmpcDealNu D;
+    fmpc_host_deal_nu(m, n, T, W, fmpc_host_nu_parts(T, fmpc_host_nu_work(plan), W), has_nu_out != 0, has_u0 != 0, 4, nu_tiles, levelled != 0, D);
+    std::vector<int> flat;
+    fmpc_host_deal_nu_flat(D, flat, nullptr, nullptr);
+    if (out && cap >= (int)flat.size()) std::copy(flat.begin(), flat.end(), out);
+    return (int)flat.size();
+}
diff --git a/mpc-sensorlessao_amd/csrc/fmpc_host.h b/mpc-sensorlessao_amd/csrc/fmpc_host.h
--- a/mpc-sensorlessao_amd/csrc/fmpc_host.h
+++ b/mpc-sensorlessao_amd/csrc/fmpc_host.h
@@ -115,6 +115,26 @@
 int fmpc_host_nu_work(const std::vector<FmpcNuStage>& plan);
 int fmpc_host_nu_parts(int T, int work, int W);
 int fmpc_host_nu_swap(int T, int parts, int W);
+#define FMPC_DEAL_DIRECT 0
+#define FMPC_DEAL_DIRECT_U0 1
+#define FMPC_DEAL_UUNIT 2
+#define FMPC_DEAL_NUOUT 3
+#define FMPC_DEAL_FORMS 4
+#define FMPC_DEAL_W_DIRECT 56
+#define FMPC_DEAL_W_UTILE 28
+#define FMPC_DEAL_W_NU 112
+#define FMPC_DEAL_W_FORMS 112
+#define FMPC_DEAL_SEG 8
+struct FmpcDealNu {
+    int W = 0;
+    std::vector<int> off;
+    std::vector<int> seg;
+    std::vector<int> tl;
+    std::vector<int> load;
+};
+void fmpc_host_deal_nu(int m, int n, int T, int W, int parts, bool has_nu_out, bool has_u0, int forms_cts, int nu_tiles, bool levelled,
+                       FmpcDealNu& D);
+void fmpc_host_deal_nu_flat(const FmpcDealNu& D, std::vector<int>& flat, int* seg_off, int* tl_off);
 #define FMPC_LANE_START_ROUNDS 3
 int fmpc_host_plan_lanes(int nsteps, const unsigned* supersedes, int ngroups, int slots, int tiles_used, int cap, int* lane_of_step, int* wpg);
 void fmpc_host_mfma_images(const double* M, int rows, int cols, int ks, std::vector<double>& img);
diff --git a/mpc-sensorlessao_amd/csrc/fmpc_kernel_affine.hip b/mpc-sensorlessao_amd/csrc/fmpc_kernel_affine.hip
--- a/mpc-sensorlessao_amd/csrc/fmpc_kernel_affine.hip
+++ b/mpc-sensorlessao_amd/csrc/fmpc_kernel_affine.hip
@@ -264,7 +264,7 @@
     }
 }
 
-hipError_t fmpc_launch_affine(FaParams P, int num_cu, hipStream_t stream, const unsigned* supersedes) {
+hipError_t fmpc_launch_affine(FaParams P, int num_cu, hipStream_t stream, const unsigned* supersedes, FaDealCache* deals) {
     if (P.n != 27 || 2 * P.n + 2 > FA_KC || 7 * FA_THREADS < FA_CT * 16 * P.n) return hipErrorInvalidValue;
     if (P.nsteps < 0 || P.nsteps > FMPC_STRETCH_MAX) return hipErrorInvalidValue;
     if (P.nsteps == 0) {
@@ -305,7 +305,7 @@
     const int grid = P.nlanes * ngroups * wpg;
     if (P.zout && P.imgG) {
         const char* e = getenv("FMPC_AFFINE_DIRECT");
-        if (!(e && e[0] == '1')) return fmpc_launch_affine_nu(P, grid, nt, stream);
+        if (!(e && e[0] == '1')) return fmpc_launch_affine_nu(P, grid, nt, stream, deals);
     }
     if (P.zout && nt) hipLaunchKernelGGL((fmpc_cold_affine<true, true>), dim3(grid), dim3(FA_THREADS), 0, stream, P);
     else if (P.zout) hipLaunchKernelGGL((fmpc_cold_affine<true, false>), dim3(grid), dim3(FA_THREADS), 0, stream, P);
diff --git a/mpc-sensorlessao_amd/csrc/fmpc_kernel_affine_nu.hip b/mpc-sensorlessao_amd/csrc/fmpc_kernel_affine_nu.hip
--- a/mpc-sensorlessao_amd/csrc/fmpc_kernel_affine_nu.hip
+++ b/mpc-sensorlessao_amd/csrc/fmpc_kernel_affine_nu.hip
@@ -1,6 +1,7 @@
 #include <hip/hip_runtime.h>
 #include <math.h>
 #include <stdlib.h>
+#include <vector>
 #include "fmpc_affine_dev.h"
 
 #ifdef FW_TIMING
@@ -44,33 +45,36 @@
 }
 
 template <bool NT, bool FULL>
-__device__ __forceinline__ void fa_nu_utiles(const FaParams& P, double (&A)[FA_NU_KS], const d4a (&n0)[FA_CT], const d4a (&n1)[FA_CT],
-                                             int ub, int ue, int ui, int gi, int lane, double* zout_s, double* dump) {
-    double An[FA_NU_KS];
+__device__ __forceinline__ void fa_nu_utiles(const FaParams& P, double (&G)[FA_NU_KS], double (&A)[FA_KS], const d4a (&n0)[FA_CT], const d4a (&n1)[FA_CT],
+                                             int ub, int ue, int ui, int after, int gi, int lane, double* zout_s, double* dump) {
+    double Gn[FA_NU_KS];
+    fa_request_a(A, P.img, after, lane);
     int tile = ub;
     do {
-        fa_request_g(An, P.imgG, ui + (tile + 1 < ue ? tile + 1 : tile) - ub, lane);
+        fa_request_g(Gn, P.imgG, ui + (tile + 1 < ue ? tile + 1 : tile) - ub, lane);
         d4a acc[FA_CT];
 #pragma unroll
         for (int ct = 0; ct < FA_CT; ++ct) acc[ct] = (d4a){0, 0, 0, 0};
 #pragma unroll
         for (int q = 0; q < FA_NU_KS; ++q)
 #pragma unroll
-            for (int ct = 0; ct < FA_CT; ++ct) acc[ct] = FA_MFMA(q < 4 ? n0[ct][q & 3] : n1[ct][q & 3], A[q], acc[ct]);
+            for (int ct = 0; ct < FA_CT; ++ct) acc[ct] = FA_MFMA(q < 4 ? n0[ct][q & 3] : n1[ct][q & 3], G[q], acc[ct]);
         fa_nu_store<NT, FULL>(P, acc, tile, gi, lane, zout_s, nullptr, dump);
-        fa_await_g<16>(An);
-#pragma unroll
-        for (int q = 0; q < FA_NU_KS; ++q) A[q] = An[q];
+        fa_await_g<16>(Gn);
+#pragma unroll
+        for (int q = 0; q < FA_NU_KS; ++q) G[q] = Gn[q];
     } while (++tile < ue);
+    fa_await_a<16>(A);
 }
 
 template <bool NT, bool U0>
 __device__ __forceinline__ void fa_nu_direct(const FaParams& P, double (&A)[FA_KS], double (&An)[FA_KS], const double (&D)[FA_CT][FA_KS],
-                                             int db, int de, int after, int gi, int lane, double* zout_s, double* nuout_s, double* u0out_s, double* dump) {
+                                             const int* tl, int cnt, int after, int gi, int lane, double* zout_s, double* nuout_s, double* u0out_s, double* dump) {
     const int m = P.m;
-    int tile = db;
+    int i = 0, tile = tl[0];
     do {
-        if (!U0) fa_request_a(An, P.img, tile + 1 < de ? tile + 1 : after, lane);
+        const int nx = tl[i + 1 < cnt ? i + 1 : i], next = i + 1 < cnt ? nx : after;
+        if (!U0) fa_request_a(An, P.img, next, lane);
         d4a acc[FA_CT];
 #pragma unroll
         for (int ct = 0; ct < FA_CT; ++ct) acc[ct] = (d4a){0, 0, 0, 0};
@@ -80,7 +84,7 @@
             for (int ct = 0; ct < FA_CT; ++ct) acc[ct] = FA_MFMA(D[ct][q], A[q], acc[ct]);
         if (U0) {
             asm volatile("" :: "v"(acc[0][0]), "v"(acc[1][0]), "v"(acc[2][0]), "v"(acc[3][0]));
-            fa_request_a(A, P.img, tile + 1 < de ? tile + 1 : after, lane);
+            fa_request_a(A, P.img, next, lane);
         }
         fa_nu_store<NT, false>(P, acc, tile, gi, lane, zout_s, nuout_s, dump);
         if (U0) {
@@ -107,44 +111,26 @@
 #pragma unroll
             for (int q = 0; q < FA_KS; ++q) A[q] = An[q];
         }
-    } while (++tile < de);
-}
-
-struct FaNuItem { int ub, ue, ui, db, de, jt; };
-__device__ __forceinline__ FaNuItem fa_nu_item(const FaParams& P, int it) {
-    FaNuItem I = {0, 0, 0, 0, 0, -1};
-    const int nst = P.T * P.nparts;
-    if (it < nst) {
-        const int js = it / P.nparts, part = it - js * P.nparts;
-        const int j = js == P.swap ? 0 : (js == 0 ? P.swap : js);
-        const int tb = P.plan[4 * j], nu = P.plan[4 * j + 1], nd = P.plan[4 * j + 2], u0 = FMPC_NU_CUT(nu, part, P.nparts);
-        I.ub = tb + u0; I.ue = tb + FMPC_NU_CUT(nu, part + 1, P.nparts); I.ui = P.plan[4 * j + 3] + u0;
-        I.db = tb + nu + FMPC_NU_CUT(nd, part, P.nparts); I.de = tb + nu + FMPC_NU_CUT(nd, part + 1, P.nparts);
-        if (I.ue > I.ub) I.jt = P.jbase + 2 * (j - 1);
-    } else {
-        I.db = P.tiles + 4 * (it - nst);
-        I.de = I.db + 4 < P.tiles + P.nu_tiles ? I.db + 4 : P.tiles + P.nu_tiles;
-    }
-    return I;
+        tile = next;
+    } while (++i < cnt);
 }
 
 template <bool NT>
 __global__ void __launch_bounds__(FA_THREADS, 2) fmpc_cold_nu(FaParams P) {
     __shared__ double sD[FA_KS * FA_CT * 64];
-    __shared__ double sF[4][3][16];
     const int tid0 = threadIdx.x;
     const int wg = (int)blockIdx.x;
     const int ln = wg / P.wgs_per_lane, wl = wg - ln * P.wgs_per_lane;
     const int gi = wl / P.wgs_per_group, slot = wl - gi * P.wgs_per_group;
     const int s_begin = P.lane_begin[ln], s_end = P.lane_begin[ln + 1];
-    const int nwav = 4 * P.wgs_per_group;
     { const int tid = tid0; FA_TICK(0); (void)tid; }
     if (wg == 0 && tid0 == 0 && P.handed) *P.handed = 0;
     const int p0 = gi * FA_CT * 16;
+    const int wv = __builtin_amdgcn_readfirstlane(tid0 >> 6);
     for (int s = s_begin; s < s_end; ++s) {
-    int tid = tid0;
-    asm volatile("" : "+v"(tid));
-    const int wv = __builtin_amdgcn_readfirstlane(tid >> 6);
+    int tid;
+    asm volatile("v_mbcnt_lo_u32_b32 %0, -1, 0\n\tv_mbcnt_hi_u32_b32 %0, -1, %0" : "=&v"(tid));
+    tid += 64 * wv;
     const FaStep& S = P.steps[s];
     const double* const x0_s = S.x0; const double* const x0p_s = S.x0p; const double* const nu0_s = S.nu0;
     double* const zout_s = S.zout; double* const nuout_s = S.nuout; double* const u0out_s = S.u0out;
@@ -153,66 +139,97 @@
     fa_stage(sD, P, x0_s, x0p_s, p0, tid);
     __syncthreads();
     FA_TICK(1);
-    fa_forms(sD, sF, P, slot, wv, tid & 63, p0, nu0_s, need_s, status_s, iters_s, step_s);
+    const int w = slot * 4 + wv;
+    int sg = P.deal[4 + w];
+    const int sge = P.deal[4 + w + 1];
+    const int* seg = P.deal + P.deal_seg + FMPC_DEAL_SEG * sg;
+    while (sg < sge && seg[0] == FMPC_DEAL_FORMS) {
+        fa_forms_unit(sD, P, seg[1], tid & 63, p0, nu0_s, need_s, status_s, iters_s, step_s);
+        ++sg; seg += FMPC_DEAL_SEG;
+    }
     FA_TICK(2);
-    for (int it = slot * 4 + wv; it < P.nitems; it += nwav) {
-        int lane = tid & 63;
-        asm volatile("" : "+v"(lane));
-        const FaNuItem I = fa_nu_item(P, it);
-        if (I.de <= I.db && I.jt < 0) continue;
+    if (sg < sge) {
         double A[FA_KS], An[FA_KS];
-        fa_request_a(A, P.img, I.de > I.db ? I.db : I.jt, lane);
-        double* dump = P.dump + ((blockIdx.x & 15) * FA_THREADS + wv * 64 + lane);
-        const int ub = I.ub, ue = I.ue, ui = I.ui, db = I.db, de = I.de, jt = I.jt;
-        double D[FA_CT][FA_KS];
-#pragma unroll
-        for (int ct = 0; ct < FA_CT; ++ct)
-#pragma unroll
-            for (int q = 0; q < FA_KS; ++q) D[ct][q] = sD[(q * FA_CT + ct) * 64 + lane];
-        fa_await_a<0>(A);
-        if (de > db) {
-            const int after = jt >= 0 ? jt : db;
-            if (u0out_s != nullptr && 16 * db < P.m) fa_nu_direct<NT, true>(P, A, An, D, db, de, after, gi, lane, zout_s, nuout_s, u0out_s, dump);
-            else fa_nu_direct<NT, false>(P, A, An, D, db, de, after, gi, lane, zout_s, nuout_s, u0out_s, dump);
-        }
-#ifdef FW_TIMING
-        if (it == slot * 4 + wv) FA_TICK(4);
-#endif
-        if (jt < 0) continue;
-        d4a n0[FA_CT], n1[FA_CT];
-        double G[FA_NU_KS];
-        fa_request_a(An, P.img, jt + 1, lane);
-        fa_request_g(G, P.imgG, ui, lane);
-#pragma unroll
-        for (int ct = 0; ct < FA_CT; ++ct) { n0[ct] = (d4a){0, 0, 0, 0}; n1[ct] = (d4a){0, 0, 0, 0}; }
-#pragma unroll
-        for (int q = 0; q < FA_KS; ++q) n0[0] = FA_MFMA(A[q], D[0][q], n0[0]);
-        fa_await_a<FA_NU_KS>(An);
-#pragma unroll
-        for (int q = 0; q < FA_KS; ++q) n1[0] = FA_MFMA(An[q], D[0][q], n1[0]);
-#pragma unroll
-        for (int ct = 1; ct < FA_CT; ++ct)
-#pragma unroll
-            for (int q = 0; q < FA_KS; ++q) { n0[ct] = FA_MFMA(A[q], D[ct][q], n0[ct]); n1[ct] = FA_MFMA(An[q], D[ct][q], n1[ct]); }
-        fa_await_g<0>(G);
-#ifdef FW_TIMING
-        if (it == slot * 4 + wv) { asm volatile("s_nop 0" :: "v"(n1[0][0]), "v"(n1[1][0]), "v"(n1[2][0]), "v"(n1[3][0])); FA_TICK(5); }
-#endif
-        if ((gi + 1) * FA_CT * 16 <= P.batch) fa_nu_utiles<NT, true>(P, G, n0, n1, ub, ue, ui, gi, lane, zout_s, dump);
-        else fa_nu_utiles<NT, false>(P, G, n0, n1, ub, ue, ui, gi, lane, zout_s, dump);
-#ifdef FW_TIMING
-        if (it == slot * 4 + wv) FA_TICK(6);
-#endif
+        {
+            int lane = tid & 63;
+            asm volatile("" : "+v"(lane));
+            fa_request_a(A, P.img, seg[7], lane);
+            fa_await_a<0>(A);
+        }
+        do {
+            int lane = tid & 63;
+            asm volatile("" : "+v"(lane));
+            const int kind = seg[0], sa = seg[1], sb = seg[2], sc = seg[3], after = seg[5];
+            double* dump = P.dump + ((blockIdx.x & 15) * FA_THREADS + wv * 64 + lane);
+            double D[FA_CT][FA_KS];
+#pragma unroll
+            for (int ct = 0; ct < FA_CT; ++ct)
+#pragma unroll
+                for (int q = 0; q < FA_KS; ++q) D[ct][q] = sD[(q * FA_CT + ct) * 64 + lane];
+            if (kind != FMPC_DEAL_UUNIT) {
+                const int* tl = P.deal + P.deal_tl + sa;
+                if (kind == FMPC_DEAL_DIRECT_U0) fa_nu_direct<NT, true>(P, A, An, D, tl, sb, after, gi, lane, zout_s, nuout_s, u0out_s, dump);
+                else fa_nu_direct<NT, false>(P, A, An, D, tl, sb, after, gi, lane, zout_s, nuout_s, u0out_s, dump);
+            } else {
+                const int jt = seg[4];
+                d4a n0[FA_CT], n1[FA_CT];
+                double G[FA_NU_KS];
+                fa_request_a(An, P.img, jt + 1, lane);
+                fa_request_g(G, P.imgG, sc, lane);
+#pragma unroll
+                for (int ct = 0; ct < FA_CT; ++ct) { n0[ct] = (d4a){0, 0, 0, 0}; n1[ct] = (d4a){0, 0, 0, 0}; }
+#pragma unroll
+                for (int q = 0; q < FA_KS; ++q) n0[0] = FA_MFMA(A[q], D[0][q], n0[0]);
+                fa_await_a<FA_NU_KS>(An);
+#pragma unroll
+                for (int q = 0; q < FA_KS; ++q) n1[0] = FA_MFMA(An[q], D[0][q], n1[0]);
+#pragma unroll
+                for (int ct = 1; ct < FA_CT; ++ct)
+#pragma unroll
+                    for (int q = 0; q < FA_KS; ++q) { n0[ct] = FA_MFMA(A[q], D[ct][q], n0[ct]); n1[ct] = FA_MFMA(An[q], D[ct][q], n1[ct]); }
+                fa_await_g<0>(G);
+                if ((gi + 1) * FA_CT * 16 <= P.batch) fa_nu_utiles<NT, true>(P, G, A, n0, n1, sa, sb, sc, after, gi, lane, zout_s, dump);
+                else fa_nu_utiles<NT, false>(P, G, A, n0, n1, sa, sb, sc, after, gi, lane, zout_s, dump);
+            }
+            seg += FMPC_DEAL_SEG;
+        } while (++sg < sge);
     }
     FA_TICK(3);
     }
 }
 
-hipError_t fmpc_launch_affine_nu(FaParams P, int grid, bool nt, hipStream_t stream) {
-    if (P.n != FA_N || !P.zout || !P.imgG || !P.plan || P.nu_work <= 0 || grid < 1) return hipErrorInvalidValue;
-    P.nparts = fmpc_host_nu_parts(P.T, P.nu_work, 4 * P.wgs_per_group);
-    P.swap = fmpc_host_nu_swap(P.T, P.nparts, 4 * P.wgs_per_group);
-    P.nitems = P.T * P.nparts + (P.nuout ? (P.nu_tiles + 3) / 4 : 0);
+static const int* fa_deal_table(FaDealCache& C, const FaParams& P, int W, bool levelled, hipStream_t stream, int* seg_off, int* tl_off) {
+    const int key = (levelled ? 1 : 0) | (P.nuout ? 2 : 0) | (P.u0out ? 4 : 0);
+    for (int i = 0; i < FA_DEAL_SLOTS; ++i)
+        if (C.arena.p && C.e[i].W == W && C.e[i].key == key) { *seg_off = C.e[i].seg_off; *tl_off = C.e[i].tl_off; return C.arena.p + (size_t)i * C.slot_ints; }
+    hipStreamCaptureStatus st = hipStreamCaptureStatusNone;
+    if (hipStreamIsCapturing(stream, &st) == hipSuccess && st == hipStreamCaptureStatusActive) return nullptr;
+    FmpcDealNu D;
+    fmpc_host_deal_nu(P.m, P.n, P.T, W, fmpc_host_nu_parts(P.T, P.nu_work, W), P.nuout != nullptr, P.u0out != nullptr, FA_CT, P.nu_tiles, levelled, D);
+    std::vector<int> flat;
+    fmpc_host_deal_nu_flat(D, flat, seg_off, tl_off);
+    if (!C.arena.p) {
+        const size_t nd = (size_t)P.tiles + P.nu_tiles;
+        C.slot_ints = 24 + nd + 8 + FMPC_DEAL_SEG * (FA_CT + 8 * (size_t)P.T + nd) + nd;
+        if (C.arena.alloc(C.slot_ints * FA_DEAL_SLOTS, stream) != FMPC_OK) return nullptr;
+    }
+    if (flat.size() > C.slot_ints) return nullptr;
+    const int slot = C.next;
+    if (C.e[slot].key >= 0) { (void)hipDeviceSynchronize(); fmpc_alloc_gen.fetch_add(1); }
+    C.e[slot] = FaDealCache::Entry();
+    int* dst = C.arena.p + (size_t)slot * C.slot_ints;
+    if (hipMemcpy(dst, flat.data(), flat.size() * sizeof(int), hipMemcpyHostToDevice) != hipSuccess) return nullptr;
+    C.e[slot].W = W; C.e[slot].key = key; C.e[slot].seg_off = *seg_off; C.e[slot].tl_off = *tl_off;
+    C.next = (slot + 1) % FA_DEAL_SLOTS;
+    return dst;
+}
+
+hipError_t fmpc_launch_affine_nu(FaParams P, int grid, bool nt, hipStream_t stream, FaDealCache* deals) {
+    if (P.n != FA_N || !P.zout || !P.imgG || !P.plan || P.nu_work <= 0 || grid < 1 || !deals) return hipErrorInvalidValue;
+    if (P.tiles != (P.T * (P.n + P.m) + 15) / 16 || P.jbase != P.tiles + P.nu_tiles) return hipErrorInvalidValue;
+    const char* e = getenv("FMPC_AFFINE_DEAL");
+    P.deal = fa_deal_table(*deals, P, 4 * P.wgs_per_group, !(e && e[0] == '0'), stream, &P.deal_seg, &P.deal_tl);
+    if (!P.deal) return hipErrorOutOfMemory;
     if (nt) hipLaunchKernelGGL((fmpc_cold_nu<true>), dim3(grid), dim3(FA_THREADS), 0, stream, P);
     else hipLaunchKernelGGL((fmpc_cold_nu<false>), dim3(grid), dim3(FA_THREADS), 0, stream, P);
     return hipGetLastError();
```
